# aligirayhanozbay/poisson_CNN

Hardware: AMD Instinct MI355X
Metric: grids/sec (fwd+bwd) at 1024^2 (higher is better)
Workload: dtype f32; 1 GPU; c4: Homogeneous_Poisson_NN_Legacy(hpnn.json) full train step (fwd+bwd+loss+Adam), 8 x 1024x1024 Dirichlet grids per GPU; global_batch=8, parallelism=dp1, math=fp32, ranks_seen=1

## Files before the change

include/pcnn.h:

```cpp
#ifndef PCNN_H
#define PCNN_H
#include <stddef.h>
#include <stdint.h>
#ifdef __cplusplus
extern "C" {
#endif

typedef struct pcnn_handle_s* pcnn_handle;

enum { PCNN_PAD_CONSTANT = 0, PCNN_PAD_SYMMETRIC = 1, PCNN_PAD_REFLECT = 2 };
enum { PCNN_ACT_LINEAR = 0, PCNN_ACT_LEAKY_RELU = 1, PCNN_ACT_TANH = 2, PCNN_ACT_RELU = 3 };
enum { PCNN_POOL_AVERAGE = 0, PCNN_POOL_MAX = 1 };
enum { PCNN_RESIZE_NEAREST = 0, PCNN_RESIZE_BILINEAR = 1, PCNN_RESIZE_BICUBIC = 2,
       PCNN_RESIZE_BICUBIC_LEGACY_ALIGN_CORNERS = 3  };

int pcnn_create(int device, void* hip_stream, pcnn_handle* out);
int pcnn_destroy(pcnn_handle h);
int pcnn_set_stream(pcnn_handle h, void* hip_stream);
int pcnn_sync(pcnn_handle h);
const char* pcnn_last_error(pcnn_handle h);
int pcnn_version(void);
uint32_t pcnn_crc32c(const void* data, size_t n, uint32_t crc);

#define PCNN_UNIQUE_ID_BYTES 128
int pcnn_collective_available(char* why, size_t why_bytes);
int pcnn_comm_unique_id(pcnn_handle h, void* id_out);
int pcnn_comm_init(pcnn_handle h, const void* id, int rank, int world_size);
int pcnn_comm_destroy(pcnn_handle h);
int pcnn_allreduce(pcnn_handle h, float* buf, size_t count);
int pcnn_broadcast(pcnn_handle h, float* buf, size_t count, int root);

enum { PCNN_MATH_FP32 = 0, PCNN_MATH_SPLIT_F16 = 1 };
int pcnn_set_math_mode(pcnn_handle h, int mode);
int pcnn_get_math_mode(pcnn_handle h);

enum { PCNN_SPECTRAL_AUTO = -1, PCNN_SPECTRAL_OFF = 0, PCNN_SPECTRAL_FORCE = 1 };
int pcnn_set_spectral_mode(pcnn_handle h, int mode);
int pcnn_get_spectral_mode(pcnn_handle h);
int pcnn_set_spectral_tile(pcnn_handle h, int tile);
int pcnn_get_spectral_tile(pcnn_handle h);
enum { PCNN_XFORM_MFMA = 0, PCNN_XFORM_FFT = 1 };
int pcnn_set_spectral_transform(pcnn_handle h, int xform);
int pcnn_get_spectral_transform(pcnn_handle h);
int pcnn_set_filter_version(pcnn_handle h, uint64_t version);
int pcnn_filter_cache_clear(pcnn_handle h);
int pcnn_filter_cache_stats(pcnn_handle h, long long* entries, long long* bytes, long long* hits, long long* fills, long long* refreshes);
int pcnn_set_workspace_limit(pcnn_handle h, size_t bytes);
int pcnn_set_workspace_retain(pcnn_handle h, int retain);

typedef struct {
  int N, H, W, Cin, ldx;
  int Ho, Wo, Cout, ldy;
  int kh, kw, pad_top, pad_left;
  int pad_mode; float pad_value;
  int act; float act_alpha;
  int ld_res;
  int ld_act_out;
} pcnn_conv_desc;

int pcnn_conv2d_fwd(pcnn_handle h, const pcnn_conv_desc* d, const float* x, const float* w, const float* bias,
                    const float* bn_scale, const float* bn_shift, const float* residual, float* y, float* act_out);
int pcnn_conv2d_fwd_absmax(pcnn_handle h, const pcnn_conv_desc* d, const float* x, const float* w, const float* bias,
                           const float* bn_scale, const float* bn_shift, const float* residual, float* y, float* act_out, float* y_absmax);

int pcnn_conv2d_flip_transpose_weights(pcnn_handle h, const float* w, float* wt, int kh, int kw, int Cin, int Cout);
typedef struct pcnn_flip_item { const float* w; float* wt; int kh, kw, Cin, Cout; int64_t start; } pcnn_flip_item;
int pcnn_conv2d_flip_transpose_table(pcnn_handle h, const pcnn_flip_item* table_dev, int n, int64_t total);

size_t pcnn_conv2d_wgrad_workspace(const pcnn_conv_desc* d);
int pcnn_conv2d_wgrad(pcnn_handle h, const pcnn_conv_desc* d, const float* x, const float* dz, float* dw,
                      void* workspace, size_t workspace_bytes);
int pcnn_conv2d_wgrad_hint(pcnn_handle h, const pcnn_conv_desc* d, const float* x, const float* dz, float* dw,
                           void* workspace, size_t workspace_bytes, const float* x_absmax, const float* dz_absmax);

int pcnn_resnet3_fwd_eligible(pcnn_handle h, int C, int act);
int pcnn_resnet3_fwd(pcnn_handle h, int N, int H, int W, int C, int act, float act_alpha, const float* x, const float* w0, const float* b0,
                     const float* w1, const float* b1, const float* w2, const float* b2, float* o0, float* a1, float* o1, float* y);

int pcnn_conv2d_bwd_spectral_eligible(pcnn_handle h, const pcnn_conv_desc* d, const pcnn_conv_desc* dg);
int pcnn_conv2d_bwd_spectral(pcnn_handle h, const pcnn_conv_desc* d, const pcnn_conv_desc* dg, const float* x, const float* dz, const float* w_flipped,
                             const float* residual, float* dx, float* dw);
typedef struct pcnn_post_desc {
  const float* act_out; int ld_act_out; int act; float act_alpha;
  float* dbias; float* raw_out; int ld_raw;
} pcnn_post_desc;
int pcnn_conv2d_bwd_spectral_post_eligible(pcnn_handle h, const pcnn_conv_desc* d, const pcnn_conv_desc* dg);
int pcnn_conv2d_bwd_spectral_post(pcnn_handle h, const pcnn_conv_desc* d, const pcnn_conv_desc* dg, const float* x, const float* dz, const float* w_flipped,
                                  const float* residual, float* dx, float* dw, const pcnn_post_desc* post);

int pcnn_conv2d_dgrad_post_eligible(pcnn_handle h, const pcnn_conv_desc* dg, const float* dz, const float* residual, const float* dx, const pcnn_post_desc* post);
int pcnn_conv2d_dgrad_post(pcnn_handle h, const pcnn_conv_desc* dg, const float* dz, const float* w_flipped, const float* residual, float* dx,
                           const pcnn_post_desc* post);

int pcnn_debug_forward_spectrum32(pcnn_handle h, int H, int W, int C, const float* x, int Vy, int Vx, int oy, int ox, int pad_mode, float pad_value,
                                  int ylim, int xlim, int pack, float* out, size_t out_floats);
int pcnn_debug_tile_spectrum64(pcnn_handle h, int H, int W, int C, const float* x, int ylim, int xlim, float* out);

size_t pcnn_colsum_workspace(int C);
int pcnn_conv2d_epilogue_bwd(pcnn_handle h, int64_t npix, int C, const float* dy, int lddy, const float* a, int lda,
                             const float* bn_scale, int act, float act_alpha, float* dz, int lddz,
                             float* dbias, float* dsum_dy_a, float* dsum_dy, void* workspace, size_t workspace_bytes);
int pcnn_conv2d_epilogue_bwd_absmax(pcnn_handle h, int64_t npix, int C, const float* dy, int lddy, const float* a, int lda,
                                    const float* bn_scale, int act, float act_alpha, float* dz, int lddz, float* dbias,
                                    float* dsum_dy_a, float* dsum_dy, float* dz_absmax, void* workspace, size_t workspace_bytes);

int pcnn_pad_fold_bwd(pcnn_handle h, int N, int H, int W, int C, int pt, int pb, int pl, int pr, int pad_mode,
                      const float* gp, int ldgp, float* gx, int ldgx, int accumulate);
int pcnn_pad_fold_bwd_post_eligible(int C, int ldgp, int ld_add, const void* gp, const void* add_to, const pcnn_post_desc* post, int lddz, const void* dz);
int pcnn_pad_fold_bwd_post(pcnn_handle h, int N, int H, int W, int C, int pt, int pb, int pl, int pr, int pad_mode, const float* gp, int ldgp,
                           const float* add_to, int ld_add, const pcnn_post_desc* post, const float* bn_scale, float* dsum_dy_a, float* dsum_dy,
                           float* dz, int lddz, void* workspace, size_t workspace_bytes);

int pcnn_bn_fold(pcnn_handle h, int n, const float* gamma, const float* beta, const float* mean, const float* var, float eps,
                 float* scale, float* shift);
int pcnn_bn_fold_bwd(pcnn_handle h, int n, const float* s_dy_a, const float* s_dy, const float* mean, const float* var, float eps,
                     float* dgamma, float* dbeta);

int pcnn_channel_affine(pcnn_handle h, int64_t npix, int C, const float* x, int ldx, const float* scale, const float* shift,
                        const float* residual, int ld_res, float* y, int ldy);
int pcnn_bn_train_fwd(pcnn_handle h, int64_t npix, int C, const float* a, int lda, const float* gamma, const float* beta, float eps,
                      float momentum, float* moving_mean, float* moving_var, float* mean, float* inv_std, float* scale, float* scratch_2C,
                      const float* residual, int ld_res, float* y, int ldy, void* workspace, size_t workspace_bytes);
int pcnn_bn_train_bwd(pcnn_handle h, int64_t npix, int C, const float* dy, int lddy, const float* a, int lda, const float* scale,
                      const float* mean, const float* inv_std, float* dgamma, float* dbeta, float* scratch_4C, float* da, int ldda,
                      void* workspace, size_t workspace_bytes);

int pcnn_pool2d_fwd(pcnn_handle h, int kind, int N, int H, int W, int C, int f, const float* x, int ldx, float* y, int ldy);
int pcnn_pool2d_bwd(pcnn_handle h, int kind, int N, int H, int W, int C, int f, const float* x, int ldx,
                    const float* y, int ldy, const float* dy, int lddy, float* dx, int lddx, int accumulate);

int pcnn_deconv_fwd(pcnn_handle h, int N, int hc, int wc, int Cin, int H, int W, int Cout, int f, const float* x, int ldx,
                    const float* k, const float* bias, float alpha, float beta, float* y, int ldy);
int pcnn_deconv_bwd_data(pcnn_handle h, int N, int hc, int wc, int Cin, int H, int W, int Cout, int f, const float* dy, int lddy,
                         const float* k, float alpha, float* dx, int lddx);
size_t pcnn_deconv_wgrad_workspace(int N, int hc, int wc, int Cin, int Cout, int f);
int pcnn_deconv_bwd_filter(pcnn_handle h, int N, int hc, int wc, int Cin, int H, int W, int Cout, int f, const float* x, int ldx,
                           const float* dy, int lddy, float alpha, float* dk, float* dbias, void* workspace, size_t workspace_bytes);

typedef struct {
  int N, H, W, Cin, ldx;
  int Ho, Wo, Cout, ldy;
  int k;
  int act; float act_alpha;
  float dropout_rate; uint32_t dropout_seed; uint32_t dropout_layer;
  int ld_act_out;
  int accumulate;
} pcnn_wide_desc;
int pcnn_wide_conv2d_fwd(pcnn_handle h, const pcnn_wide_desc* d, const float* x, const float* w, const float* bias, float* y);
int pcnn_wide_conv2d_dgrad(pcnn_handle h, const pcnn_wide_desc* d, const float* dz, const float* wf, const float* act_out, float* dx);
size_t pcnn_wide_conv2d_wgrad_workspace(const pcnn_wide_desc* d);
int pcnn_wide_conv2d_wgrad(pcnn_handle h, const pcnn_wide_desc* d, const float* x, const float* dz, float* dw, float* dbias, void* workspace,
                           size_t workspace_bytes);
int pcnn_wide_deconv_fwd(pcnn_handle h, const pcnn_wide_desc* d, const float* x, const float* k, const float* bias, float* y);
int pcnn_wide_deconv_bwd_data(pcnn_handle h, const pcnn_wide_desc* d, const float* dz, const float* k, const float* act_out, float* dx);
size_t pcnn_wide_deconv_bwd_filter_workspace(const pcnn_wide_desc* d);
int pcnn_wide_deconv_bwd_filter(pcnn_handle h, const pcnn_wide_desc* d, const float* x, const float* dz, float* dk, void* workspace,
                                size_t workspace_bytes);

int pcnn_resize_tables(int method, int n_in, int n_out, int32_t* idx , float* wt );
int pcnn_resize_fwd(pcnn_handle h, int N, int hc, int wc, int C, int Ho, int Wo, const float* x, int ldx,
                    const int32_t* idx_y, const float* wt_y, const int32_t* idx_x, const float* wt_x,
                    float alpha, float beta, float* y, int ldy);
typedef struct pcnn_resize_src {
  const float* x; int hc, wc, ldx;
  const int32_t* idx_y; const float* wt_y; const int32_t* idx_x; const float* wt_x;
} pcnn_resize_src;
int pcnn_resize_fwd_multi_eligible(int N, int C, int Ho, int Wo, int nsrc, const pcnn_resize_src* src, const float* y, int ldy);
int pcnn_resize_fwd_multi(pcnn_handle h, int N, int C, int Ho, int Wo, int nsrc, const pcnn_resize_src* src, float alpha, float beta, float* y, int ldy);
int pcnn_resize_bwd(pcnn_handle h, int N, int hc, int wc, int C, int Ho, int Wo, const float* dy, int lddy,
                    const int32_t* idx_y, const float* wt_y, const int32_t* idx_x, const float* wt_x,
                    float alpha, float* tmp, float* dx, int lddx);

size_t pcnn_grouped_conv2d_wgrad_workspace(const pcnn_conv_desc* d);
int pcnn_grouped_conv2d_uses_mfma(const pcnn_conv_desc* d, int what);
int pcnn_grouped_conv2d_fwd(pcnn_handle h, const pcnn_conv_desc* d, const float* x, const float* w, long long w_sample_stride, const float* bias,
                            long long bias_sample_stride, int flip_transpose, float* y);
int pcnn_grouped_conv2d_wgrad(pcnn_handle h, const pcnn_conv_desc* d, const float* x, const float* dz, float* dw, long long dw_sample_stride, void* workspace);
int pcnn_grouped_bias_grad(pcnn_handle h, int N, long long HW, int C, const float* dz, int lddz, float* dbias, long long bias_sample_stride);
int pcnn_grouped_deconv_fwd(pcnn_handle h, int N, int H, int W, int Cin, int Ho, int Wo, int Cout, int f, const float* x, const float* k,
                            long long k_sample_stride, const float* bias, long long bias_sample_stride, float* y);
int pcnn_grouped_deconv_bwd_data(pcnn_handle h, int N, int H, int W, int Cin, int Ho, int Wo, int Cout, int f, const float* dy, const float* k,
                                 long long k_sample_stride, float* dx);
int pcnn_grouped_deconv_bwd_filter(pcnn_handle h, int N, int H, int W, int Cin, int Ho, int Wo, int Cout, int f, const float* x, const float* dy,
                                   float* dk, long long k_sample_stride, float* dbias, long long bias_sample_stride);

int pcnn_dense_fwd(pcnn_handle h, int N, int In, int Out, const float* x, const float* w, const float* b, int act, float alpha, float* y);
int pcnn_dense_bwd(pcnn_handle h, int N, int In, int Out, const float* x, const float* w, const float* y, const float* dy,
                   int act, float alpha, float* dx, float* dw, float* db);

int pcnn_assemble_input(pcnn_handle h, int N, int H, int W, const float* rhs, int use_pos, float* out, int ldo);
int pcnn_subsample(pcnn_handle h, int N, int H, int W, int C, int stride, const float* x, int ldx, float* y, int ldy, int adjoint);
int pcnn_axpby(pcnn_handle h, int64_t npix, int C, float alpha, const float* x, int ldx, float beta, float* y, int ldy);
int pcnn_channel_scale_fwd(pcnn_handle h, int N, int64_t hw, int C, const float* x, int ldx, const float* s, float* y, int ldy);
int pcnn_channel_scale_bwd(pcnn_handle h, int N, int64_t hw, int C, const float* x, int ldx, const float* s, const float* dy, int lddy,
                           float* dx, int lddx, float* ds, void* workspace, size_t workspace_bytes);
size_t pcnn_channel_scale_workspace(int N, int64_t hw, int C);
int pcnn_channel_scale_bwd_post(pcnn_handle h, int N, int64_t hw, int C, const float* x, int ldx, const float* s, const float* dy, int lddy,
                                float* dz, int lddz, float* ds, int act, float act_alpha, float* dbias, void* workspace, size_t workspace_bytes);
int pcnn_sample_scale_fwd(pcnn_handle h, int N, int64_t per, const float* x, const float* g, float* y);
int pcnn_sample_scale_bwd(pcnn_handle h, int N, int64_t per, const float* x, const float* g, const float* dy, float* dx, float* dg);
int pcnn_bc_ring_fwd(pcnn_handle h, int N, int H, int W, int neumann, const float* x, float* y);
int pcnn_bc_ring_bwd(pcnn_handle h, int N, int H, int W, int neumann, const float* dy, float* dx);
int pcnn_bc_ring_edges_fwd(pcnn_handle h, int N, int H, int W, int neumann_mask, const float* x, float* y);
int pcnn_bc_ring_edges_bwd(pcnn_handle h, int N, int H, int W, int neumann_mask, const float* dy, float* dx);
int pcnn_spp_max_fwd(pcnn_handle h, int N, int H, int W, int C, int nb, const int32_t* bins, const float* x, float* out, int32_t* argmax);
int pcnn_spp_max_bwd(pcnn_handle h, int N, int H, int W, int C, int nb, const int32_t* argmax, const float* dout, float* dx);
int pcnn_jacobi_sweep(pcnn_handle h, int N, int H, int W, const float* u, const float* rhs, const float* dx , float* out);
int pcnn_jacobi_sweep_bwd(pcnn_handle h, int N, int H, int W, const float* dout, const float* dx , float* du);
int pcnn_jacobi_fused_fwd(pcnn_handle h, int N, int H, int W, int sy, int sx, const float* coef , const float* u, const float* rhs,
                          int n_sweeps, float* out);
int pcnn_jacobi_fused_bwd(pcnn_handle h, int N, int H, int W, int sy, int sx, const float* coef , const float* dout, int n_sweeps,
                          float* du);
int pcnn_jacobi_fused_tile(void);
int pcnn_jacobi_fused_max_sweeps(int sy, int sx);
int pcnn_jacobi_fused_bc_fwd(pcnn_handle h, int N, int H, int W, int sy, int sx, const float* coef , const float* u, const float* rhs,
                             int n_sweeps, int neumann_mask, float* out);
int pcnn_jacobi_fused_bc_bwd(pcnn_handle h, int N, int H, int W, int sy, int sx, const float* coef , const float* dout, int n_sweeps,
                             int neumann_mask, float* du);

int pcnn_loss_partials(pcnn_handle h, int N, int64_t hw, const float* pred, const float* target, const float* G, float* out );
int pcnn_loss_bwd(pcnn_handle h, int N, int64_t hw, const float* pred, const float* target, const float* G,
                  const float* c_mae, const float* c_mse, const float* c_int, float* dpred);
int pcnn_loss_coefficients(pcnn_handle h, int N, int64_t hw, const float* partials, float w_mae, float w_mse, float w_int,
                           int scale_by_peak, int global_batch_size, const float* extra, float* loss, float* c_mae, float* c_mse,
                           float* c_int, float* mse);
int pcnn_loss_partials_p(pcnn_handle h, int N, int64_t hw, const float* pred, const float* target, const float* G, float lp_power, float* partials);
int pcnn_loss_bwd_p(pcnn_handle h, int N, int64_t hw, const float* pred, const float* target, const float* G, const float* c_mae,
                    const float* c_mse, const float* c_int, float lp_power, float* dpred);
int pcnn_loss_coefficients_p(pcnn_handle h, int N, int64_t hw, const float* partials, float w_mae, float w_mse, float w_int, float lp_power,
                             int scale_by_peak, int global_batch_size, const float* extra, float* loss, float* c_mae, float* c_mse,
                             float* c_int, float* mse);
int pcnn_pi_loss_partials(pcnn_handle h, int N, int H, int W, int s, const float* pred, const float* rhs, const float* kern, float* out );
int pcnn_pi_loss_bwd(pcnn_handle h, int N, int H, int W, int s, const float* pred, const float* rhs, const float* kern,
                     const float* coef , float* dpred);
int pcnn_pi_loss_partials_rect(pcnn_handle h, int N, int H, int W, int sy, int sx, const float* pred, const float* rhs, const float* kern,
                               float* out );
int pcnn_pi_loss_bwd_rect(pcnn_handle h, int N, int H, int W, int sy, int sx, const float* pred, const float* rhs, const float* kern,
                          const float* coef , float* dpred);
int pcnn_error_stats(pcnn_handle h, int N, int H, int W, const float* pred, const float* target ,
                     const float* rhs , const float* dx , float* out );

// ... 83 lines not shown
```

poisson_cnn_amd/csrc/pcnn_internal.h:

```cpp
#pragma once
#include <hip/hip_runtime.h>
#include "pcnn_host.h"

void pcnn_comm_release(pcnn_handle_s* h);
void pcnn_filter_cache_free(pcnn_handle_s* h);

typedef float f32x16 __attribute__((ext_vector_type(16)));
typedef float f32x4 __attribute__((ext_vector_type(4)));

__device__ __forceinline__ float pcnn_act(float v, int act, float alpha) {
  switch (act) {
    case PCNN_ACT_LEAKY_RELU: return v > 0.f ? v : alpha * v;
    case PCNN_ACT_TANH: return tanhf(v);
    case PCNN_ACT_RELU: return v > 0.f ? v : 0.f;
    default: return v;
  }
}
__device__ __forceinline__ float pcnn_act_grad_from_out(float a, int act, float alpha) {
  switch (act) {
    case PCNN_ACT_LEAKY_RELU: return a > 0.f ? 1.f : alpha;
    case PCNN_ACT_TANH: return 1.f - a * a;
    case PCNN_ACT_RELU: return a > 0.f ? 1.f : 0.f;
    default: return 1.f;
  }
}

__device__ __forceinline__ int pcnn_pad_index(int i, int n, int mode) {
  if (i >= 0 && i < n) return i;
  if (mode == PCNN_PAD_CONSTANT) return -1;
  int r;
  if (mode == PCNN_PAD_SYMMETRIC) r = i < 0 ? -i - 1 : 2 * n - 1 - i;
  else r = i < 0 ? -i : 2 * n - 2 - i;
  return r < 0 ? 0 : (r >= n ? n - 1 : r);
}
```

poisson_cnn_amd/csrc/pointwise.hip:

```cpp
#include "pcnn_internal.h"

namespace {

constexpr int CS_BLOCK = 256;
constexpr int CS_MAXBLK = 1024;

static int pow2_ge(int c) { int p = 1; while (p < c) p <<= 1; return p; }

__global__ __launch_bounds__(CS_BLOCK) void epilogue_bwd_kernel(int64_t npix, int C, int CP, const float* __restrict__ dy, int lddy,
                                                                const float* __restrict__ a, int lda, const float* __restrict__ bn_scale,
                                                                int act, float alpha, float* __restrict__ dz, int lddz,
                                                                float* __restrict__ partial , unsigned* __restrict__ absmax) {
  __shared__ float red[3][CS_BLOCK];
  const int tid = threadIdx.x, c = tid % CP, r = tid / CP, R = CS_BLOCK / CP;
  float s0 = 0.f, s1 = 0.f, s2 = 0.f, zmax = 0.f;
  if (c < C) {
    const float sc = bn_scale ? bn_scale[c] : 1.f;
    for (int64_t pix = (int64_t)blockIdx.x * R + r; pix < npix; pix += (int64_t)gridDim.x * R) {
      const float g = dy[pix * lddy + c];
      const float av = a ? a[pix * lda + c] : 0.f;
      const float z = g * sc * pcnn_act_grad_from_out(av, act, alpha);
      if (dz) dz[pix * lddz + c] = z;
      s0 += z; s1 += g * av; s2 += g; zmax = fmaxf(zmax, fabsf(z));
    }
  }
  if (absmax) {
#pragma unroll
    for (int o = 32; o > 0; o >>= 1) zmax = fmaxf(zmax, __shfl_xor(zmax, o));
    if ((tid & 63) == 0) atomicMax(absmax, __float_as_uint(zmax <= 3.0e38f ? zmax : 3.0e38f));
  }
  red[0][tid] = s0; red[1][tid] = s1; red[2][tid] = s2;
  __syncthreads();
  if (r == 0 && c < C) {
    for (int k = 0; k < 3; ++k) {
      float s = 0.f;
      for (int q = 0; q < R; ++q) s += red[k][q * CP + c];
      partial[((int64_t)blockIdx.x * 3 + k) * C + c] = s;
    }
  }
}

__global__ __launch_bounds__(CS_BLOCK) void epilogue_bwd_vec4_kernel(int64_t npix, int C, const float* __restrict__ dy, int lddy,
                                                                     const float* __restrict__ a, int lda, const float* __restrict__ bn_scale,
                                                                     int act, float alpha, float* __restrict__ dz, int lddz,
                                                                     float* __restrict__ partial , unsigned* __restrict__ absmax) {
  __shared__ float red[3][CS_BLOCK * 4];
  float zmax = 0.f;
  const int GQ = C >> 2, R = CS_BLOCK / GQ;
  const int tid = threadIdx.x, r = tid / GQ, q = tid - r * GQ, c = q << 2;
  float s0[4] = {0.f, 0.f, 0.f, 0.f}, s1[4] = {0.f, 0.f, 0.f, 0.f}, s2[4] = {0.f, 0.f, 0.f, 0.f};
  if (r < R) {
    float sc[4];
#pragma unroll
    for (int j = 0; j < 4; ++j) sc[j] = bn_scale ? bn_scale[c + j] : 1.f;
    for (int64_t pix = (int64_t)blockIdx.x * R + r; pix < npix; pix += (int64_t)gridDim.x * R) {
      const float4 g4 = *reinterpret_cast<const float4*>(dy + pix * lddy + c);
      const float4 a4 = a ? *reinterpret_cast<const float4*>(a + pix * lda + c) : make_float4(0.f, 0.f, 0.f, 0.f);
      const float g[4] = {g4.x, g4.y, g4.z, g4.w}, av[4] = {a4.x, a4.y, a4.z, a4.w};
      float z[4];
#pragma unroll
      for (int j = 0; j < 4; ++j) {
        z[j] = g[j] * sc[j] * pcnn_act_grad_from_out(av[j], act, alpha);
        s0[j] += z[j]; s1[j] += g[j] * av[j]; s2[j] += g[j]; zmax = fmaxf(zmax, fabsf(z[j]));
      }
      if (dz) *reinterpret_cast<float4*>(dz + pix * lddz + c) = make_float4(z[0], z[1], z[2], z[3]);
    }
  }
  if (absmax) {
#pragma unroll
    for (int o = 32; o > 0; o >>= 1) zmax = fmaxf(zmax, __shfl_xor(zmax, o));
    if ((tid & 63) == 0) atomicMax(absmax, __float_as_uint(zmax <= 3.0e38f ? zmax : 3.0e38f));
  }
#pragma unroll
  for (int j = 0; j < 4; ++j) { red[0][tid * 4 + j] = s0[j]; red[1][tid * 4 + j] = s1[j]; red[2][tid * 4 + j] = s2[j]; }
  __syncthreads();
  if (tid < C) {
    for (int k = 0; k < 3; ++k) {
      float s = 0.f;
      for (int rr = 0; rr < R; ++rr) s += red[k][rr * C + tid];
      partial[((int64_t)blockIdx.x * 3 + k) * C + tid] = s;
    }
  }
}

__global__ __launch_bounds__(256) void colsum_final_kernel(const float* __restrict__ partial, int nblk, int C, float* o0, float* o1, float* o2) {
  __shared__ float red[3][256];
  const int c = blockIdx.x, t = threadIdx.x;
  float s[3] = {0.f, 0.f, 0.f};
  for (int b = t; b < nblk; b += 256)
    for (int k = 0; k < 3; ++k) s[k] += partial[((int64_t)b * 3 + k) * C + c];
  for (int k = 0; k < 3; ++k) red[k][t] = s[k];
  __syncthreads();
  for (int st = 128; st > 0; st >>= 1) {
    if (t < st)
      for (int k = 0; k < 3; ++k) red[k][t] += red[k][t + st];
    __syncthreads();
  }
  if (t == 0) {
    if (o0) o0[c] = red[0][0];
    if (o1) o1[c] = red[1][0];
    if (o2) o2[c] = red[2][0];
  }
}

static int colsum_blocks(int64_t npix, int CP) {
  const int R = CS_BLOCK / CP;
  int64_t nb = pcnn_cdiv64(npix, (int64_t)R * 16);
  if (nb > CS_MAXBLK) nb = CS_MAXBLK;
  if (nb < 1) nb = 1;
  return (int)nb;
}

__global__ void pad_fold_kernel(int N, int H, int W, int C, int pt, int pb, int pl, int pr, int mode, const float* __restrict__ gp, int ldgp,
                                float* __restrict__ gx, int ldgx, int accumulate) {
  const int Hp = H + pt + pb, Wp = W + pl + pr;
  const int64_t total = (int64_t)N * H * W * C;
  for (int64_t i = (int64_t)blockIdx.x * blockDim.x + threadIdx.x; i < total; i += (int64_t)gridDim.x * blockDim.x) {
    const int c = i % C; int64_t r = i / C; const int x = r % W; r /= W; const int y = r % H; const int n = r / H;
    int ys[3], xs[3], ny = 0, nx = 0;
    ys[ny++] = y + pt;
    xs[nx++] = x + pl;
    if (mode == PCNN_PAD_SYMMETRIC) {
      if (y < pt) ys[ny++] = pt - 1 - y;
      if (H - 1 - y < pb) ys[ny++] = pt + H + (H - 1 - y);
      if (x < pl) xs[nx++] = pl - 1 - x;
      if (W - 1 - x < pr) xs[nx++] = pl + W + (W - 1 - x);
    } else if (mode == PCNN_PAD_REFLECT) {
      if (y >= 1 && y <= pt) ys[ny++] = pt - y;
      if (H - 2 - y >= 0 && H - 2 - y < pb) ys[ny++] = pt + H + (H - 2 - y);
      if (x >= 1 && x <= pl) xs[nx++] = pl - x;
      if (W - 2 - x >= 0 && W - 2 - x < pr) xs[nx++] = pl + W + (W - 2 - x);
    }
    float s = 0.f;
    for (int a = 0; a < ny; ++a)
      for (int b = 0; b < nx; ++b) s += gp[(((int64_t)n * Hp + ys[a]) * Wp + xs[b]) * ldgp + c];
    float* dst = &gx[(((int64_t)n * H + y) * W + x) * ldgx + c];
    *dst = accumulate ? *dst + s : s;
  }
}

__global__ void pad_fold_vec4_kernel(int N, int H, int W, int C, int pt, int pb, int pl, int pr, int mode, const float* __restrict__ gp, int ldgp,
                                     float* __restrict__ gx, int ldgx, int accumulate) {
  const int Hp = H + pt + pb, Wp = W + pl + pr, CV = C >> 2;
  const int64_t total = (int64_t)N * H * W * CV;
  for (int64_t i = (int64_t)blockIdx.x * blockDim.x + threadIdx.x; i < total; i += (int64_t)gridDim.x * blockDim.x) {
    const int c = (int)(i % CV) << 2; int64_t r = i / CV; const int x = r % W; r /= W; const int y = r % H; const int n = r / H;
    int ys[3], xs[3], ny = 0, nx = 0;
    ys[ny++] = y + pt;
    xs[nx++] = x + pl;
    if (mode == PCNN_PAD_SYMMETRIC) {
      if (y < pt) ys[ny++] = pt - 1 - y;
      if (H - 1 - y < pb) ys[ny++] = pt + H + (H - 1 - y);
      if (x < pl) xs[nx++] = pl - 1 - x;
      if (W - 1 - x < pr) xs[nx++] = pl + W + (W - 1 - x);
    } else if (mode == PCNN_PAD_REFLECT) {
      if (y >= 1 && y <= pt) ys[ny++] = pt - y;
      if (H - 2 - y >= 0 && H - 2 - y < pb) ys[ny++] = pt + H + (H - 2 - y);
      if (x >= 1 && x <= pl) xs[nx++] = pl - x;
      if (W - 2 - x >= 0 && W - 2 - x < pr) xs[nx++] = pl + W + (W - 2 - x);
    }
    float4 s = make_float4(0.f, 0.f, 0.f, 0.f);
    for (int a = 0; a < ny; ++a)
      for (int b = 0; b < nx; ++b) {
        const float4 q = *reinterpret_cast<const float4*>(gp + (((int64_t)n * Hp + ys[a]) * Wp + xs[b]) * ldgp + c);
        s.x += q.x; s.y += q.y; s.z += q.z; s.w += q.w;
      }
    float4* dst = reinterpret_cast<float4*>(gx + (((int64_t)n * H + y) * W + x) * ldgx + c);
    if (accumulate) { const float4 o = *dst; s.x += o.x; s.y += o.y; s.z += o.z; s.w += o.w; }
    *dst = s;
  }
}

__global__ __launch_bounds__(CS_BLOCK) void pad_fold_post_vec4_kernel(int N, int H, int W, int C, int pt, int pb, int pl, int pr, int mode,
                                                                      const float* __restrict__ gp, int ldgp, const float* __restrict__ add_to, int ldadd,
                                                                      const float* __restrict__ a, int lda, const float* __restrict__ bn_scale, int act, float alpha,
                                                                      float* __restrict__ raw, int ldraw, float* __restrict__ dz, int lddz,
                                                                      float* __restrict__ partial ) {
  __shared__ float red[3][CS_BLOCK * 4];
  const int Hp = H + pt + pb, Wp = W + pl + pr;
  const int64_t npix = (int64_t)N * H * W;
  const int GQ = C >> 2, R = CS_BLOCK / GQ;
  const int tid = threadIdx.x, r = tid / GQ, q = tid - r * GQ, c = q << 2;
  float s0[4] = {0.f, 0.f, 0.f, 0.f}, s1[4] = {0.f, 0.f, 0.f, 0.f}, s2[4] = {0.f, 0.f, 0.f, 0.f};
  if (r < R) {
    float sc[4];
#pragma unroll
    for (int j = 0; j < 4; ++j) sc[j] = bn_scale ? bn_scale[c + j] : 1.f;
    for (int64_t pix = (int64_t)blockIdx.x * R + r; pix < npix; pix += (int64_t)gridDim.x * R) {
      int64_t t = pix; const int x = t % W; t /= W; const int y = t % H; const int n = t / H;
      int ys[3], xs[3], ny = 0, nx = 0;
      ys[ny++] = y + pt;
      xs[nx++] = x + pl;
      if (mode == PCNN_PAD_SYMMETRIC) {
        if (y < pt) ys[ny++] = pt - 1 - y;
        if (H - 1 - y < pb) ys[ny++] = pt + H + (H - 1 - y);
        if (x < pl) xs[nx++] = pl - 1 - x;
        if (W - 1 - x < pr) xs[nx++] = pl + W + (W - 1 - x);
      } else if (mode == PCNN_PAD_REFLECT) {
        if (y >= 1 && y <= pt) ys[ny++] = pt - y;
        if (H - 2 - y >= 0 && H - 2 - y < pb) ys[ny++] = pt + H + (H - 2 - y);
        if (x >= 1 && x <= pl) xs[nx++] = pl - x;
        if (W - 2 - x >= 0 && W - 2 - x < pr) xs[nx++] = pl + W + (W - 2 - x);
      }
      float4 g = make_float4(0.f, 0.f, 0.f, 0.f);
      for (int ia = 0; ia < ny; ++ia)
        for (int ib = 0; ib < nx; ++ib) {
          const float4 v = *reinterpret_cast<const float4*>(gp + (((int64_t)n * Hp + ys[ia]) * Wp + xs[ib]) * ldgp + c);
          g.x += v.x; g.y += v.y; g.z += v.z; g.w += v.w;
        }
      if (add_to) { const float4 o = *reinterpret_cast<const float4*>(add_to + pix * ldadd + c); g.x += o.x; g.y += o.y; g.z += o.z; g.w += o.w; }
      if (raw) *reinterpret_cast<float4*>(raw + pix * ldraw + c) = g;
      const float4 a4 = *reinterpret_cast<const float4*>(a + pix * lda + c);
      const float gv[4] = {g.x, g.y, g.z, g.w}, av[4] = {a4.x, a4.y, a4.z, a4.w};
      float z[4];
#pragma unroll
      for (int j = 0; j < 4; ++j) {
        z[j] = gv[j] * sc[j] * pcnn_act_grad_from_out(av[j], act, alpha);
        s0[j] += z[j]; s1[j] += gv[j] * av[j]; s2[j] += gv[j];
      }
      *reinterpret_cast<float4*>(dz + pix * lddz + c) = make_float4(z[0], z[1], z[2], z[3]);
    }
  }
#pragma unroll
  for (int j = 0; j < 4; ++j) { red[0][tid * 4 + j] = s0[j]; red[1][tid * 4 + j] = s1[j]; red[2][tid * 4 + j] = s2[j]; }
  __syncthreads();
  if (tid < C) {
    for (int k = 0; k < 3; ++k) {
      float s = 0.f;
      for (int rr = 0; rr < R; ++rr) s += red[k][rr * C + tid];
      partial[((int64_t)blockIdx.x * 3 + k) * C + tid] = s;
    }
  }
}

__global__ void axpby_kernel(int64_t npix, int C, float alpha, const float* __restrict__ x, int ldx, float beta, float* __restrict__ y, int ldy) {
  const int64_t total = npix * C;
  for (int64_t i = (int64_t)blockIdx.x * blockDim.x + threadIdx.x; i < total; i += (int64_t)gridDim.x * blockDim.x) {
    const int c = i % C; const int64_t pix = i / C;
    float* dst = &y[pix * ldy + c];
    const float v = alpha * x[pix * ldx + c];
    *dst = beta == 0.f ? v : v + beta * *dst;
  }
}

__global__ void assemble_input_kernel(int N, int H, int W, const float* __restrict__ rhs, int use_pos, float* __restrict__ out, int ldo) {
  const int64_t total = (int64_t)N * H * W;
  const float pi = 3.14159265358979323846f;
  for (int64_t i = (int64_t)blockIdx.x * blockDim.x + threadIdx.x; i < total; i += (int64_t)gridDim.x * blockDim.x) {
    const int x = i % W; const int y = (i / W) % H;
    out[i * ldo] = rhs[i];
    if (use_pos) {
      const float ly = H > 1 ? (float)y * (1.0f / (float)(H - 1)) : 0.f;
      const float lx = W > 1 ? (float)x * (1.0f / (float)(W - 1)) : 0.f;
      out[i * ldo + 1] = cosf(pi * ly);
      out[i * ldo + 2] = cosf(pi * lx);
    }
  }
}

__global__ void channel_scale_fwd_kernel(int N, int64_t hw, int C, const float* __restrict__ x, int ldx, const float* __restrict__ s,
                                         float* __restrict__ y, int ldy) {
  const int64_t total = (int64_t)N * hw * C;
  for (int64_t i = (int64_t)blockIdx.x * blockDim.x + threadIdx.x; i < total; i += (int64_t)gridDim.x * blockDim.x) {
    const int c = i % C; const int64_t pix = i / C; const int n = pix / hw;
    y[pix * ldy + c] = x[pix * ldx + c] * s[n * C + c];
  }
}

__global__ __launch_bounds__(CS_BLOCK) void channel_scale_bwd_kernel(int64_t hw, int C, int CP, const float* __restrict__ x, int ldx,
                                                                     const float* __restrict__ s, const float* __restrict__ dy, int lddy,
                                                                     float* __restrict__ dx, int lddx, float* __restrict__ partial,
                                                                     int gmode, float galpha, float* __restrict__ bpartial) {
  __shared__ float red[CS_BLOCK];
  const int n = blockIdx.y, tid = threadIdx.x, c = tid % CP, r = tid / CP, R = CS_BLOCK / CP;
  float acc = 0.f, bacc = 0.f;
  if (c < C) {
    const float sv = s[n * C + c];
    for (int64_t q = (int64_t)blockIdx.x * R + r; q < hw; q += (int64_t)gridDim.x * R) {
      const int64_t pix = (int64_t)n * hw + q;
      const float g = dy[pix * lddy + c], xv = x[pix * ldx + c];
      acc += g * xv;
      float v = g * sv;
      if (bpartial) {
        v *= gmode == PCNN_ACT_TANH ? 1.f - xv * xv : (xv > 0.f ? 1.f : galpha);
        bacc += v;
      }
      dx[pix * lddx + c] = v;
    }
  }
  red[tid] = acc;
  __syncthreads();
  if (r == 0 && c < C) {
    float t = 0.f;
    for (int q = 0; q < R; ++q) t += red[q * CP + c];
    partial[((int64_t)n * gridDim.x + blockIdx.x) * C + c] = t;
  }
  if (bpartial) {
    __syncthreads();
    red[tid] = bacc;
    __syncthreads();
    if (r == 0 && c < C) {
      float t = 0.f;
      for (int q = 0; q < R; ++q) t += red[q * CP + c];
      bpartial[((int64_t)n * gridDim.x + blockIdx.x) * C + c] = t;
    }
  }
}

__global__ void channel_scale_bias_final_kernel(const float* __restrict__ bpartial, int N, int nb, int C, float* __restrict__ dbias) {
  const int c = blockIdx.x * blockDim.x + threadIdx.x;
  if (c >= C) return;
  float t = 0.f;
  for (int i = 0; i < N * nb; ++i) t += bpartial[(int64_t)i * C + c];
  dbias[c] = t;
}

__global__ void channel_scale_final_kernel(const float* __restrict__ partial, int N, int nblk, int C, float* __restrict__ ds) {
  const int i = blockIdx.x * blockDim.x + threadIdx.x;
  if (i >= N * C) return;
  const int n = i / C, c = i % C;
  float t = 0.f;
  for (int b = 0; b < nblk; ++b) t += partial[((int64_t)n * nblk + b) * C + c];
  ds[i] = t;
}

__global__ void sample_scale_fwd_kernel(int N, int64_t per, const float* __restrict__ x, const float* __restrict__ g, float* __restrict__ y) {
  const int64_t total = (int64_t)N * per;
  for (int64_t i = (int64_t)blockIdx.x * blockDim.x + threadIdx.x; i < total; i += (int64_t)gridDim.x * blockDim.x)
    y[i] = x[i] * (1.0f + g[i / per]);
}

constexpr int SS_SPLIT = 64;
__global__ __launch_bounds__(256) void sample_scale_bwd_kernel(int64_t per, const float* __restrict__ x, const float* __restrict__ g,
                                                               const float* __restrict__ dy, float* __restrict__ dx, float* __restrict__ part) {
  __shared__ float red[256];
  const int n = blockIdx.y, sp = blockIdx.x;
  const float gv = 1.0f + g[n];
  const int64_t piece = (per + SS_SPLIT - 1) / SS_SPLIT, q0 = (int64_t)sp * piece, q1 = q0 + piece < per ? q0 + piece : per;
  float acc = 0.f;
  for (int64_t q = q0 + threadIdx.x; q < q1; q += blockDim.x) {
    const int64_t i = (int64_t)n * per + q;
    const float d = dy[i];
    acc += d * x[i];
    dx[i] = d * gv;
  }
  red[threadIdx.x] = acc;
  __syncthreads();
  for (int s = blockDim.x / 2; s > 0; s >>= 1) {
    if ((int)threadIdx.x < s) red[threadIdx.x] += red[threadIdx.x + s];
    __syncthreads();
  }
  if (threadIdx.x == 0) part[n * SS_SPLIT + sp] = red[0];
}
__global__ void sample_scale_final_kernel(int N, const float* __restrict__ part, float* __restrict__ dg) {
  const int n = blockIdx.x * blockDim.x + threadIdx.x;
  if (n >= N) return;
// ... 638 lines not shown
```

poisson_cnn_amd/csrc/spectral_common.h:

```cpp
#pragma once
#include "pcnn_internal.h"
#include <type_traits>

namespace pcnn_spec {

constexpr int RS = 32;
constexpr int SP_PAD = 32;
__host__ __device__ __forceinline__ int64_t sp_item(int64_t item, int rows) { return item * ((int64_t)rows * RS + SP_PAD); }
__host__ __device__ __forceinline__ size_t sp_bytes(size_t items, int rows) { return items * ((size_t)rows * RS + SP_PAD) * sizeof(float); }

constexpr int SP_P = 1;
__host__ __device__ constexpr int sp_blk(int P, int k, int part) { return 2 * P * (k / P) + P * part + (k % P); }
__host__ __device__ constexpr int sp_pc(int T, int P) { return P < T ? P : T; }
__host__ __device__ constexpr int sp_pr(int T, int P) { return P < T / 2 ? P : T / 2; }
__host__ __device__ constexpr int sp_row_c(int T, int fy, int part, int P = SP_P) { return sp_blk(sp_pc(T, P), fy, part); }
__host__ __device__ constexpr int sp_row_r(int T, int s, int P = SP_P) {
  return s == T / 2 ? sp_blk(sp_pr(T, P), 0, 1) : (s < T / 2 ? sp_blk(sp_pr(T, P), s, 0) : sp_blk(sp_pr(T, P), s - T / 2, 1));
}
__host__ __device__ constexpr int sp_row_from_canonical(int T, int r, int P = SP_P) {
  return r < 2 * T ? (r / T) * T + sp_row_r(T, r % T, P) : 2 * T + ((r - 2 * T) / (2 * T)) * 2 * T + sp_row_c(T, (r - 2 * T) % T, ((r - 2 * T) % (2 * T)) / T, P);
}
static_assert(sp_row_from_canonical(32, 5, 64) == 5 && sp_row_from_canonical(32, 16, 64) == 16 && sp_row_from_canonical(32, 64 + 37, 64) == 64 + 37 && sp_row_from_canonical(64, 128 + 64 + 9, 64) == 128 + 64 + 9, "P >= T is the canonical order");
static_assert(sp_row_from_canonical(32, 16, 1) == 1 && sp_row_from_canonical(32, 3, 1) == 6 && sp_row_from_canonical(32, 16 + 3, 1) == 7 && sp_row_from_canonical(32, 64 + 32 + 5, 1) == 64 + 11, "P = 1: Re | Im adjacent");
inline void sp_build_slots(int T, int P, int* slots) {
  int n = 0;
  auto put = [&](int rr, int ri, int kind) { slots[4 * n] = rr; slots[4 * n + 1] = ri; slots[4 * n + 2] = kind; slots[4 * n + 3] = 0; ++n; };
  for (int b = 0; b < 2; ++b) {
    put(b * T + sp_row_r(T, 0, P), b * T + sp_row_r(T, T / 2, P), 1);
    for (int fy = 1; fy < T / 2; ++fy) put(b * T + sp_row_r(T, fy, P), b * T + sp_row_r(T, T / 2 + fy, P), 0);
  }
  for (int fx = 1; fx < T / 2; ++fx)
    for (int fy = 0; fy < T; ++fy) put(2 * T + 2 * T * (fx - 1) + sp_row_c(T, fy, 0, P), 2 * T + 2 * T * (fx - 1) + sp_row_c(T, fy, 1, P), 0);
}

__device__ __forceinline__ f32x16 mfma(float a, float b, f32x16 c) { return __builtin_amdgcn_mfma_f32_32x32x2f32(a, b, c, 0, 0, 0); }
__device__ __forceinline__ f32x4 mfma16(float a, float b, f32x4 c) { return __builtin_amdgcn_mfma_f32_16x16x4f32(a, b, c, 0, 0, 0); }
__device__ __forceinline__ f32x16 zero16() {
  f32x16 z;
#pragma unroll
  for (int i = 0; i < 16; ++i) z[i] = 0.f;
  return z;
}
__device__ __forceinline__ f32x4 zero4() { f32x4 z = {0.f, 0.f, 0.f, 0.f}; return z; }
__device__ __forceinline__ void lds_barrier() { asm volatile("s_waitcnt lgkmcnt(0)\n\ts_barrier" ::: "memory"); }
__device__ __forceinline__ int acc_row(int r, int half) { return 8 * (r >> 2) + 4 * half + (r & 3); }

__device__ __forceinline__ float dpp_quad_swap1(float v) { return __int_as_float(__builtin_amdgcn_mov_dpp(__float_as_int(v), 0xB1, 0xf, 0xf, true)); }
__device__ __forceinline__ float dpp_quad_swap2(float v) { return __int_as_float(__builtin_amdgcn_mov_dpp(__float_as_int(v), 0x4E, 0xf, 0xf, true)); }
__device__ __forceinline__ void quad_transpose(float& r0, float& r1, float& r2, float& r3, bool odd, bool upper) {
  { const float t = dpp_quad_swap1(odd ? r0 : r1); if (odd) r0 = t; else r1 = t; }
  { const float t = dpp_quad_swap1(odd ? r2 : r3); if (odd) r2 = t; else r3 = t; }
  { const float t = dpp_quad_swap2(upper ? r0 : r2); if (upper) r0 = t; else r2 = t; }
  { const float t = dpp_quad_swap2(upper ? r1 : r3); if (upper) r1 = t; else r3 = t; }
}

struct FwdParams {
  const float* x = nullptr; float* sp = nullptr; const float* tab = nullptr;
  int H = 0, W = 0, C = 0, ld = 0, groups = 1, cstride = 32, cvalid = 32;
  int tiles_x = 1, tiles_y = 1, tile0 = 0, ntile = 1;
  int Vy = 0, Vx = 0, oy = 0, ox = 0, pad_mode = PCNN_PAD_CONSTANT; float pad_value = 0.f;
  int ylim = 0, xlim = 0;
  int ext_y = 1 << 30, ext_x = 1 << 30;
  int pack = 1, cpt = 32, tgx = 1;
};

struct InvParams {
  const float* sp = nullptr; const float* tab = nullptr;
  float* y = nullptr; const float* bias = nullptr; const float* bn_scale = nullptr; const float* bn_shift = nullptr; const float* res = nullptr;
  float* act_out = nullptr; unsigned* absmax = nullptr;
  int Ho = 0, Wo = 0, C = 0, ldy = 0, ld_res = 0, ld_act = 0, groups = 1, cstride = 32, cvalid = 32, act = PCNN_ACT_LINEAR; float alpha = 0.f;
  int tiles_x = 1, tiles_y = 1, tile0 = 0, ntile = 1, Vy = 0, Vx = 0;
  int flip = 0;
  int pack = 1, cpt = 32, tgx = 1;
  const float* gact = nullptr; float* y2 = nullptr; float* bsum = nullptr;
  int ld_gact = 0, ld_y2 = 0, gmode = 0; float galpha = 1.f;
};

constexpr int TAB32_FLOATS = 7168, TAB64_FLOATS = 32768;
constexpr size_t O_TAB32 = 0, O_SLOTS32 = O_TAB32 + ((TAB32_FLOATS * 4 + 255) & ~255), O_TAB64 = O_SLOTS32 + 512 * 16,
                 O_SLOTS64 = O_TAB64 + TAB64_FLOATS * 4, O_SLOTS32F = O_SLOTS64 + 2048 * 16, O_SLOTS64F = O_SLOTS32F + 512 * 16, O_REST = O_SLOTS64F + 2048 * 16;
static_assert(O_REST % 256 == 0, "workspace header alignment");
void build_tables64(float* tab, int* slots);

constexpr int POST_BLOCKS = 256, POST_SLOTS_MAX = POST_BLOCKS * 8 * 4;

struct Xform {
  int family;
  int T, rows, nslot;
  int P;
  size_t tab_off, slots_off;
  void (*fwd)(pcnn_handle h, FwdParams p, int ntile);
  void (*inv)(pcnn_handle h, InvParams p, int ntile);
  void (*post_bias)(pcnn_handle h, const float* bsum, int pack, int cpt, int C, float* dbias);
  void (*fwd_multi)(pcnn_handle h, const FwdParams* tab, int count, int max_items);
  int post_slots;
  const float* tab; const int4* slots;
};
extern const Xform XFORM_MFMA32, XFORM_MFMA64, XFORM_FFT32, XFORM_FFT64;

template <bool B> using flag = std::integral_constant<bool, B>;
template <typename Launch>
void dispatch_epilogue(InvParams p, Launch launch) {
  auto slope = [](int act, float alpha) { return act == PCNN_ACT_LINEAR ? 1.f : (act == PCNN_ACT_RELU ? 0.f : alpha); };
  if (p.gact) {
    p.alpha = 1.f; p.galpha = slope(p.gmode, p.galpha);
    if (p.res) launch(flag<false>{}, flag<true>{}, flag<true>{}, p); else launch(flag<false>{}, flag<false>{}, flag<true>{}, p);
  } else if (p.act == PCNN_ACT_TANH) {
    if (p.res) launch(flag<true>{}, flag<true>{}, flag<false>{}, p); else launch(flag<true>{}, flag<false>{}, flag<false>{}, p);
  } else {
    p.alpha = slope(p.act, p.alpha);
    if (p.res) launch(flag<false>{}, flag<true>{}, flag<false>{}, p); else launch(flag<false>{}, flag<false>{}, flag<false>{}, p);
  }
}

}
```

poisson_cnn_amd/csrc/spectral_conv.hip:

```cpp
#include "spectral_common.h"
#include <math.h>
#include <stdlib.h>
#include <array>
#include <vector>

int pcnn_spectral_conv_fwd(pcnn_handle h, const pcnn_conv_desc* d, const float* x, const float* w, const float* bias, const float* bn_scale,
                           const float* bn_shift, const float* residual, float* y, float* act_out);
int pcnn_spectral_conv_wgrad(pcnn_handle h, const pcnn_conv_desc* d, const float* x, const float* dz, float* dw);
bool pcnn_spectral_eligible(pcnn_handle h, const pcnn_conv_desc* d, bool wgrad);
bool pcnn_conv_small_fwd_eligible(const pcnn_conv_desc* d);
bool pcnn_conv_fwd_takes_narrow_route(pcnn_handle h, const pcnn_conv_desc* d);

using namespace pcnn_spec;


namespace {

constexpr int T = 32, ROWS = 1024, NSLOT = 512;
constexpr int TAB_G = 0, TAB_GI = 1024, TAB_F2 = 2048, TAB_FI2 = 4096, TAB_GI2 = 6144, TAB_FLOATS = TAB32_FLOATS;
static_assert(TAB_GI2 + 1024 == TAB_FLOATS, "table block");
constexpr size_t LDS_U = (size_t)T * T * 32 * sizeof(float);
constexpr size_t LDS_INV = LDS_U + 1024 * sizeof(float);
__host__ __device__ __forceinline__ int64_t sp_item(int64_t item) { return pcnn_spec::sp_item(item, ROWS); }

// ... 928 lines not shown
  for (FilterEntry& en : fc->e) pcnn_release(h, en.buf);
  for (int ti = 0; ti < 2; ++ti) if (fc->dev[ti]) pcnn_release(h, fc->dev[ti]);
  delete fc;
  h->filter_cache = nullptr;
}

extern "C" int pcnn_set_filter_version(pcnn_handle h, uint64_t version) {
  if (!h) return 1;
  h->filter_version = version;
  return 0;
}

extern "C" int pcnn_filter_cache_clear(pcnn_handle h) {
  if (!h) return 1;
  pcnn_filter_cache_free(h);
  return 0;
}

extern "C" int pcnn_filter_cache_stats(pcnn_handle h, long long* entries, long long* bytes, long long* hits, long long* fills, long long* refreshes) {
  if (!h) return 1;
  const FilterCache* fc = static_cast<const FilterCache*>(h->filter_cache);
  if (entries) *entries = fc ? (long long)fc->e.size() : 0;
  if (bytes) *bytes = fc ? (long long)fc->bytes : 0;
  if (hits) *hits = h->fc_hits;
  if (fills) *fills = h->fc_fills;
  if (refreshes) *refreshes = h->fc_refreshes;
  return 0;
}

int pcnn_spectral_conv_fwd(pcnn_handle h, const pcnn_conv_desc* d, const float* x, const float* w, const float* bias, const float* bn_scale,
                           const float* bn_shift, const float* residual, float* y, float* act_out) {
  TileGrid g;
  if (int rc = tile_grid(h, d, d->kh, d->kw, d->N, d->Ho, d->Wo, d->Cin, d->Cout, &g)) return rc;
  const int gin = pcnn_cdiv(d->Cin, 32), gout = pcnn_cdiv(d->Cout, 32);
  int chunk = std::min(chunk_tiles(g.T) / (gin > gout ? gin : gout), g.ntile);
  float* ws[3];
  if (int rc = carve_workspace(h, &chunk, [&](int ch) {
        return std::array<size_t, 3>{sp_region((size_t)d->Cin * gout, g.rows), sp_region((size_t)ch * gin, g.rows), sp_region((size_t)pad32(ch) * gout, g.rows)};
      }, ws)) return rc;
  float *wsp = ws[0], *xs = ws[1], *ys = ws[2];
  const Xform xf = xform_of(h, g.T);
  const float* fsp = filter_spectrum(h, xf, w, wsp, d->kh, d->kw, d->Cin, d->Cout, gout);
  PCNN_CHECK_LAUNCH(h, "spectral convolution (filter spectrum)");
  FwdParams fx = image_fwd_params(g, x, xs, d->H, d->W, d->Cin, d->ldx, gin, d->pad_top, d->pad_left, d->pad_mode, d->pad_value);
  InvParams iv = image_inv_params(g, ys, y, d->Ho, d->Wo, d->Cout, d->ldy, gout, residual, d->ld_res);
  iv.bias = bias; iv.bn_scale = bn_scale; iv.bn_shift = bn_shift; iv.act_out = act_out; iv.ld_act = d->ld_act_out;
  iv.absmax = reinterpret_cast<unsigned*>(h->y_absmax); iv.act = d->act; iv.alpha = d->act_alpha;
  MixParams mx;
  mx.xs = xs; mx.ys = ys; mx.wsp = fsp; mx.gin = gin; mx.gout = gout; mx.Cin = d->Cin; mx.cpt = g.cpt;
  for (int t0 = 0; t0 < g.ntile; t0 += chunk) {
    const int nt = std::min(chunk, g.ntile - t0);
    fx.tile0 = t0; iv.tile0 = t0;
    launch_fwd(h, xf, fx, nt);
    launch_mix(h, xf, mx, gin, gout, nt);
    launch_inv(h, xf, iv, nt);
  }
  PCNN_CHECK_LAUNCH(h, "spectral convolution");
  return 0;
}

int pcnn_spectral_conv_wgrad(pcnn_handle h, const pcnn_conv_desc* d, const float* x, const float* dz, float* dw) {
  TileGrid g;
  if (int rc = tile_grid(h, d, d->kh, d->kw, d->N, d->Ho, d->Wo, d->Cin, d->Cout, &g)) return rc;
  const int gin = pcnn_cdiv(d->Cin, 32), S = wgrad_splits(g.T);
  int chunk = std::min(chunk_tiles(g.T) / gin, g.ntile);
  float* ws[4];
  if (int rc = carve_workspace(h, &chunk, [&](int ch) {
        return std::array<size_t, 4>{sp_region((size_t)d->Cin, g.rows), sp_region((size_t)ch * gin, g.rows), sp_region((size_t)ch, g.rows), align256((size_t)S * g.nslot * gin * 4 * 1024 * 4)};
      }, ws)) return rc;
  float *csp = ws[0], *xs = ws[1], *zs = ws[2], *part = ws[3];
  const Xform xf = xform_of(h, g.T);
  FwdParams fx = image_fwd_params(g, x, xs, d->H, d->W, d->Cin, d->ldx, gin, d->pad_top, d->pad_left, d->pad_mode, d->pad_value);
  FwdParams fz = image_fwd_params(g, dz, zs, d->Ho, d->Wo, d->Cout, d->ldy, 1, 0, 0, PCNN_PAD_CONSTANT, 0.f);
  fz.ylim = g.Vy; fz.xlim = g.Vx;
  WMixParams wm;
  wm.xs = xs; wm.ds = zs; wm.part = part; wm.slots = xf.slots; wm.gin = gin; wm.S = S / 4; wm.rows = g.rows; wm.nslot = g.nslot;
  for (int t0 = 0; t0 < g.ntile; t0 += chunk) {
    const int nt = std::min(chunk, g.ntile - t0);
    fx.tile0 = t0; fz.tile0 = t0; wm.ntile = nt; wm.accumulate = t0 > 0;
    launch_fwd(h, xf, fx, nt);
    launch_fwd(h, xf, fz, nt);
    hipLaunchKernelGGL(spec_wmix_kernel, dim3(g.nslot, S / 4, gin), dim3(256), 0, h->stream, wm);
  }
  hipLaunchKernelGGL(spec_wcombine_kernel, dim3(g.nslot, gin), dim3(256), 0, h->stream, part, xf.slots, csp, S, gin, d->Cin, 1.0f, g.cpt, g.rows);
  launch_inv(h, xf, taps_params(xf, csp, dw, d->kh, d->kw, d->Cin, d->Cout, 0), 1);
  PCNN_CHECK_LAUNCH(h, "spectral weight gradient");
  return 0;
}

__global__ __launch_bounds__(256) void spec_canonical_rows_kernel(const float* __restrict__ sp, float* __restrict__ out, int T, int rows, int P) {
  const int item = blockIdx.y;
  for (int e = blockIdx.x * 256 + threadIdx.x; e < rows * 32; e += gridDim.x * 256) {
    const int r = e >> 5, c = e & 31;
    out[(size_t)item * rows * 32 + e] = sp[pcnn_spec::sp_item(item, rows) + pcnn_spec::sp_row_from_canonical(T, r, P) * RS + c];
  }
}
static int canonical_copy(pcnn_handle h, const Xform& xf, const float* sp, float* out, int items) {
  hipLaunchKernelGGL(spec_canonical_rows_kernel, dim3(16, items), dim3(256), 0, h->stream, sp, out, xf.T, xf.rows, xf.P);
  return hipGetLastError() == hipSuccess ? 0 : 1;
}

extern "C" int pcnn_debug_tile_spectrum64(pcnn_handle h, int H, int W, int C, const float* x, int ylim, int xlim, float* out) {
  PCNN_REQUIRE(h, h && x && out && H >= 1 && W >= 1 && C >= 1 && C <= 64, "pcnn_debug_tile_spectrum64: bad argument");
  TileGrid g;
  if (int rc = tile_grid_given(h, 64, 64, 64, 1, 1, 64, 64, &g)) return rc;
  const int groups = pcnn_cdiv(C, 32);
  char* r;
  if (int rc = ensure_workspace(h, sp_region((size_t)groups, g.rows), &r)) return rc;
  const Xform xf = xform_of(h, g.T);
  FwdParams f = image_fwd_params(g, x, reinterpret_cast<float*>(r), H, W, C, C, groups, 0, 0, PCNN_PAD_CONSTANT, 0.f);
  f.ylim = ylim; f.xlim = xlim;
  launch_fwd(h, xf, f, 1);
  PCNN_CHECK_LAUNCH(h, "pcnn_debug_tile_spectrum64");
  if (canonical_copy(h, xf, f.sp, out, groups)) PCNN_FAIL(h, "pcnn_debug_tile_spectrum64: copy failed");
  return 0;
}

extern "C" int pcnn_debug_forward_spectrum32(pcnn_handle h, int H, int W, int C, const float* x, int Vy, int Vx, int oy, int ox, int pad_mode, float pad_value,
                                             int ylim, int xlim, int pack, float* out, size_t out_floats) {
  PCNN_REQUIRE(h, h && x && out && H >= 1 && W >= 1 && C >= 1 && C <= 64 && Vy >= 1 && Vy <= 32 && Vx >= 1 && Vx <= 32, "pcnn_debug_forward_spectrum32: bad argument");
  PCNN_REQUIRE(h, pack == 1 || ((pack == 2 || pack == 4 || pack == 8) && C <= 32 / pack), "pcnn_debug_forward_spectrum32: pack = %d with %d channels", pack, C);
  TileGrid g;
  if (int rc = tile_grid_given(h, 32, Vy, Vx, pack, 1, H, W, &g)) return rc;
  const int groups = pack > 1 ? 1 : pcnn_cdiv(C, 32);
  PCNN_REQUIRE(h, out_floats >= (size_t)g.ntile * groups * 1024 * 32, "pcnn_debug_forward_spectrum32: output holds %zu floats, %zu needed", out_floats, (size_t)g.ntile * groups * 1024 * 32);
  char* r;
  if (int rc = ensure_workspace(h, sp_region((size_t)g.ntile * groups, g.rows), &r)) return rc;
  const Xform xf = xform_of(h, g.T);
  FwdParams f = image_fwd_params(g, x, reinterpret_cast<float*>(r), H, W, C, C, groups, oy, ox, pad_mode, pad_value);
  f.ylim = ylim; f.xlim = xlim;
  launch_fwd(h, xf, f, g.ntile);
  PCNN_CHECK_LAUNCH(h, "pcnn_debug_forward_spectrum32");
  if (canonical_copy(h, xf, f.sp, out, g.ntile * groups)) PCNN_FAIL(h, "pcnn_debug_forward_spectrum32: copy failed");
  return 0;
}

extern "C" int pcnn_conv2d_bwd_spectral_eligible(pcnn_handle h, const pcnn_conv_desc* d, const pcnn_conv_desc* dg) {
  if (!h || !d || !dg) return 0;
  if (d->Cout > 32 || d->Cin > 64) return 0;
  if (d->pad_mode == PCNN_PAD_CONSTANT && d->pad_value != 0.f) return 0;
  if (pcnn_conv_fwd_takes_narrow_route(h, dg)) return 0;
  if (pcnn_spectral_eligible(h, dg, false) && pcnn_spectral_eligible(h, d, true)) return 1;
  double ts_g = 0.0, ta_g = 0.0, ts_w = 0.0, ta_w = 0.0;
  if (spectral_costs(h, dg, false, &ts_g, &ta_g) != 2 || spectral_costs(h, d, true, &ts_w, &ta_w) != 2) return 0;
  return 1.75 * std::max(ts_g, ts_w) < 0.9 * (ta_g + ta_w) ? 1 : 0;
}

extern "C" int pcnn_conv2d_bwd_spectral_post_eligible(pcnn_handle h, const pcnn_conv_desc* d, const pcnn_conv_desc* dg) {
  if (!pcnn_conv2d_bwd_spectral_eligible(h, d, dg)) return 0;
  if (d->pad_mode != PCNN_PAD_CONSTANT) return 0;
  return d->Cin <= 32 ? 1 : 0;
}

static int bwd_spectral_impl(pcnn_handle h, const pcnn_conv_desc* d, const pcnn_conv_desc* dg, const float* x, const float* dz, const float* w_flipped,
                             const float* residual, float* dx, float* dw, const pcnn_post_desc* post);

extern "C" int pcnn_conv2d_bwd_spectral(pcnn_handle h, const pcnn_conv_desc* d, const pcnn_conv_desc* dg, const float* x, const float* dz, const float* w_flipped,
                                        const float* residual, float* dx, float* dw) {
  return bwd_spectral_impl(h, d, dg, x, dz, w_flipped, residual, dx, dw, nullptr);
}

extern "C" int pcnn_conv2d_bwd_spectral_post(pcnn_handle h, const pcnn_conv_desc* d, const pcnn_conv_desc* dg, const float* x, const float* dz, const float* w_flipped,
                                             const float* residual, float* dx, float* dw, const pcnn_post_desc* post) {
  PCNN_REQUIRE(h, h && post && post->act_out, "pcnn_conv2d_bwd_spectral_post: null argument");
  PCNN_REQUIRE(h, pcnn_conv2d_bwd_spectral_post_eligible(h, d, dg), "pcnn_conv2d_bwd_spectral_post: layer is not eligible (ask pcnn_conv2d_bwd_spectral_post_eligible first)");
  return bwd_spectral_impl(h, d, dg, x, dz, w_flipped, residual, dx, dw, post);
}

static int bwd_spectral_impl(pcnn_handle h, const pcnn_conv_desc* d, const pcnn_conv_desc* dg, const float* x, const float* dz, const float* w_flipped,
                             const float* residual, float* dx, float* dw, const pcnn_post_desc* post) {
  PCNN_REQUIRE(h, h && d && dg && x && dz && w_flipped && dx && dw, "pcnn_conv2d_bwd_spectral: null argument");
  if (pcnn_check_conv_desc(h, "pcnn_conv2d_bwd_spectral", d, 64, 32, PCNN_ANY) || pcnn_check_conv_desc(h, "pcnn_conv2d_bwd_spectral (dg)", dg, 32, 64, PCNN_ANY)) return 1;
  PCNN_REQUIRE(h, pcnn_conv2d_bwd_spectral_eligible(h, d, dg), "pcnn_conv2d_bwd_spectral: layer is not eligible (ask pcnn_conv2d_bwd_spectral_eligible first)");
  PCNN_REQUIRE(h, dg->Cin == d->Cout && dg->Cout == d->Cin && dg->kh == d->kh && dg->kw == d->kw && dg->N == d->N, "pcnn_conv2d_bwd_spectral: descriptors do not match");
  TileGrid g;
  if (int rc = tile_grid(h, dg, d->kh, d->kw, d->N, dg->Ho, dg->Wo, d->Cin, d->Cout, &g)) return rc;
  const int gz = 1, gx = pcnn_cdiv(d->Cin, 32), S = wgrad_splits(g.T);
  const size_t bs_b = post ? (size_t)POST_SLOTS_MAX * 64 * sizeof(float) : 0;
  int chunk = std::min(chunk_tiles(g.T) / gx, g.ntile);
  float* ws[7];
  if (int rc = carve_workspace(h, &chunk, [&](int ch) {
        const size_t ys_b = sp_region((size_t)pad32(ch) * gx, g.rows);
        return std::array<size_t, 7>{sp_region((size_t)std::max(dg->Cin * gx, d->Cin), g.rows), sp_region((size_t)ch * gz, g.rows), ys_b, ys_b,
                                     align256((size_t)S * g.nslot * gx * 4 * 1024 * 4), bs_b, 4096};
      }, ws)) return rc;
  float *wsp = ws[0], *zs = ws[1], *ys = ws[2], *xs = ws[3], *part = ws[4], *bsum = ws[5];
  const Xform xf = xform_of(h, g.T);
  PCNN_REQUIRE(h, gx == 1 || dg->Cout == 64, "pcnn_conv2d_bwd_spectral: %d input channels unsupported (<= 32 or 64)", d->Cin);
  const float* fsp = filter_spectrum(h, xf, w_flipped, wsp, d->kh, d->kw, dg->Cin, dg->Cout, gx);
  PCNN_CHECK_LAUNCH(h, "pcnn_conv2d_bwd_spectral (filter spectrum)");
  FwdParams fz = image_fwd_params(g, dz, zs, dg->H, dg->W, dg->Cin, dg->ldx, gz, dg->pad_top, dg->pad_left, dg->pad_mode, dg->pad_value);
  const bool padded_domain = d->pad_mode != PCNN_PAD_CONSTANT;
  FwdParams fxm = image_fwd_params(g, x, xs, d->H, d->W, d->Cin, d->ldx, gx, padded_domain ? d->pad_top : 0, padded_domain ? d->pad_left : 0, d->pad_mode, 0.f);
  fxm.ylim = g.Vy; fxm.xlim = g.Vx; fxm.ext_y = dg->Ho; fxm.ext_x = dg->Wo;
  InvParams iv = image_inv_params(g, ys, dx, dg->Ho, dg->Wo, dg->Cout, dg->ldy, gx, residual, dg->ld_res);
  if (post) {
    iv.gact = post->act_out; iv.ld_gact = post->ld_act_out; iv.gmode = post->act; iv.galpha = post->act_alpha;
    iv.y2 = post->raw_out; iv.ld_y2 = post->ld_raw; iv.bsum = post->dbias ? bsum : nullptr;
    if (iv.bsum && hipMemsetAsync(bsum, 0, bs_b, h->stream) != hipSuccess) PCNN_FAIL(h, "pcnn_conv2d_bwd_spectral_post: memset failed");
  }
  MixWParams mw;
  mw.zs = zs; mw.xs = xs; mw.ys = ys; mw.part = part; mw.wsp = fsp; mw.slots = xf.slots; mw.gx = gx; mw.rows = g.rows; mw.nslot = g.nslot;
  mw.Cz = dg->Cin; mw.cpt = g.cpt;
  for (int t0 = 0; t0 < g.ntile; t0 += chunk) {
    const int nt = std::min(chunk, g.ntile - t0);
    fz.tile0 = t0; fxm.tile0 = t0; iv.tile0 = t0; mw.ntile = nt; mw.accumulate = t0 > 0;
    launch_fwd(h, xf, fz, nt);
    launch_fwd(h, xf, fxm, nt);
    hipLaunchKernelGGL(spec_mixw_kernel, dim3(g.nslot, S / 4, gx), dim3(256), 0, h->stream, mw);
    launch_inv(h, xf, iv, nt);
  }
  if (post && post->dbias) xf.post_bias(h, bsum, g.pack, g.cpt, dg->Cout, post->dbias);
  float* csp = wsp;
  hipLaunchKernelGGL(spec_wcombine_kernel, dim3(g.nslot, gx), dim3(256), 0, h->stream, part, xf.slots, csp, S, gx, d->Cin, -1.0f, g.cpt, g.rows);
  launch_inv(h, xf, taps_params(xf, csp, dw, d->kh, d->kw, d->Cin, d->Cout, 1), 1);
  PCNN_CHECK_LAUNCH(h, "pcnn_conv2d_bwd_spectral");
  return 0;
}
```

poisson_cnn_amd/csrc/spectral_fft.hip:

```cpp
#include "spectral_common.h"
#include "fft_regs.h"
#include <algorithm>

namespace pcnn_spec {

namespace {
using namespace pcnn_fft;

constexpr int T = 32, ROWS = 1024;
constexpr int EO = 16 * 32 * 32;
constexpr size_t LDS_BYTES = (size_t)T * T * 32 * sizeof(float);
__host__ __device__ __forceinline__ int64_t sp_item32(int64_t item) { return pcnn_spec::sp_item(item, ROWS); }

__device__ __forceinline__ int pad_sel(int i, int n, int mode) {
  const int refl = mode == PCNN_PAD_SYMMETRIC ? (i < 0 ? -i - 1 : 2 * n - 1 - i) : (i < 0 ? -i : 2 * n - 2 - i);
  const int rc = min(max(refl, 0), n - 1);
  return (unsigned)i < (unsigned)n ? i : (mode == PCNN_PAD_CONSTANT ? 0 : rc);
}

struct FwdRow {
  float fill;
  int cl, cr;
  int xlim;
  bool use_fill;
// ... 5 lines not shown
  int t = p.tile0 + item / p.groups;
  const int txg = t % p.tgx; t /= p.tgx;
  const int ty = t % p.tiles_y;
  const int n = t / p.tiles_y;
  const int sub = p.pack > 1 ? c / p.cpt : 0, cc = c - sub * p.cpt;
  const int tx = txg * p.pack + sub;
  const int chan = g * p.cstride + cc;
  const bool cok = cc < p.cvalid && chan < p.C && tx < p.tiles_x;
  const float* img = p.x + (int64_t)n * p.H * p.W * p.ld;
  const int wy0 = ty * p.Vy - p.oy, wx0 = tx * p.Vx - p.ox;
  const int ylim = min(p.ylim, p.ext_y - ty * p.Vy);
  it.xlim = min(p.xlim, p.ext_x - tx * p.Vx);
  const int gy = wy0 + y;
  const bool rowconst = p.pad_mode == PCNN_PAD_CONSTANT && (unsigned)gy >= (unsigned)p.H;
  const bool rowzero = !cok || y >= ylim;
  it.use_fill = rowzero || rowconst;
  it.fill = rowzero ? 0.f : p.pad_value;
  it.cl = 0; it.cr = T;
  const int wx_first = txg * p.pack * p.Vx - p.ox, wx_last = wx_first + (p.pack - 1) * p.Vx;
  it.fast = wx_first >= 0 && wx_last + T <= p.W;
  if (2 * wave >= ylim) return;
  const int sy = pad_sel(gy, p.H, p.pad_mode);
  const unsigned ch = (unsigned)(cok ? chan : 0);
  if (it.fast) {
    const unsigned lo = (unsigned)((sy * p.W + wx0) * p.ld) + ch;
    const float* rp = img;
#pragma unroll
    for (int x = 0; x < T; ++x) { R[x] = rp[lo]; rp += p.ld; }
  } else {
    const unsigned rowoff = (unsigned)(sy * p.W * p.ld) + ch;
    if (p.pad_mode == PCNN_PAD_CONSTANT) { it.cl = -wx0; it.cr = p.W - wx0; }
#pragma unroll
    for (int x = 0; x < T; ++x) R[x] = img[rowoff + (unsigned)(pad_sel(wx0 + x, p.W, p.pad_mode) * p.ld)];
  }
}

template <bool MASKED>
__device__ __forceinline__ void fwd_consume(const FwdParams& p, const FwdRow& it, float (&R)[32]) {
#pragma unroll
  for (int x = 0; x < T; ++x) {
    float v = R[x];
    if (!it.fast && (x < it.cl || x >= it.cr)) v = p.pad_value;
    if (it.use_fill) v = it.fill;
    if (MASKED && x >= it.xlim) v = 0.f;
    R[x] = v;
  }
}

template <int N> __device__ __forceinline__ void pin(float* a) {
#pragma unroll
  for (int i = 0; i < N; ++i) asm volatile("" : "+v"(a[i]));
}

__device__ __forceinline__ float hc_get(const float (&R)[32], int s) {
  bool neg = false;
  const int pos = s <= 16 ? rfft_pos(32, s, false, neg) : rfft_pos(32, s - 16, true, neg);
  return neg ? -R[pos] : R[pos];
}
__device__ __forceinline__ void hc_put(float (&R)[32], int s, float v) {
  bool neg = false;
  const int pos = s <= 16 ? rfft_pos(32, s, false, neg) : rfft_pos(32, s - 16, true, neg);
  R[pos] = neg ? -v : v;
}

template <bool MASKED>
__device__ __forceinline__ void fft32_fwd_body(const FwdParams& p, float* U, const int bid, const int gdim) {
  const int tid = threadIdx.x, lane = tid & 63, half = lane >> 5, c = lane & 31;
  const int wave = __builtin_amdgcn_readfirstlane(tid >> 6);
  const int total = p.ntile * p.groups;
  int item = bid;
  if (item >= total) return;
  const int y = 2 * wave + half;
  float R[32];
  FwdRow cur;
  fwd_request(p, item, wave, y, c, cur, R);
  auto x_phase = [&]() {
    fwd_consume<MASKED>(p, cur, R);
    rfft_fwd<32>(R);
    float* u = U + (y * 32) * 32 + c;
#pragma unroll
    for (int s = 0; s < T; ++s) u[s * 32] = hc_get(R, s);
  };
  x_phase();
  for (;;) {
    const int next = item + gdim;
    if (next < total) fwd_request(p, next, wave, y, c, cur, R);
    lds_barrier();
    float* out = p.sp + sp_item32(item);
    float V[32];
    if (wave == 0) {
      const float* u = U + (half ? 16 : 0) * 32 + c;
#pragma unroll
      for (int yy = 0; yy < T; ++yy) V[yy] = u[yy * 1024];
      rfft_fwd<32>(V);
      const unsigned lo = (unsigned)((half ? 32 : 0) * RS + c);
#pragma unroll
      for (int s = 0; s < T; ++s) __builtin_nontemporal_store(hc_get(V, s), &(out + (sp_row_r(T, s) * RS))[lo]);
    } else {
      const float* ur = U + wave * 32 + c, *ui = U + (16 + wave) * 32 + c;
      float* vr = V, *vi = V + 16;
      int par = half;
      asm volatile("" : "+v"(par));
      const float osign = par ? -1.f : 1.f;
#pragma unroll
      for (int yy = 0; yy < 16; ++yy) {
        const float lr = ur[yy * 1024], hr = ur[(yy + 16) * 1024], li = ui[yy * 1024], hi = ui[(yy + 16) * 1024];
        const float ar = fma_(osign, hr, lr), ai = fma_(osign, hi, li);
        if (yy == 0) { vr[yy] = ar; vi[yy] = ai; }
        else {
          const float wr = par ? tw_re<32>(yy) : 1.f, wi = par ? tw_im<32>(yy) : 0.f;
          vr[yy] = fma_(ar, wr, -(ai * wi));
          vi[yy] = fma_(ar, wi, ai * wr);
        }
      }
      cfft_dif<16, -1>(vr, vi);
      float* o = out + (64 + 64 * (wave - 1)) * RS;
      const unsigned lo = (unsigned)(half * (sp_row_c(T, 1, 0) - sp_row_c(T, 0, 0)) * RS + c);
#pragma unroll
      for (int m = 0; m < 16; ++m) {
        __builtin_nontemporal_store(vr[bitrev(m, 16)], &(o + (sp_row_c(T, 2 * m, 0) * RS))[lo]);
        __builtin_nontemporal_store(vi[bitrev(m, 16)], &(o + (sp_row_c(T, 2 * m, 1) * RS))[lo]);
      }
    }
    if (next >= total) break;
    item = __builtin_amdgcn_readfirstlane(next);
    lds_barrier();
    x_phase();
  }
}

template <bool MASKED>
__global__ __launch_bounds__(1024) void fft32_fwd_kernel(FwdParams p) {
  extern __shared__ __attribute__((aligned(16))) float U[];
  fft32_fwd_body<MASKED>(p, U, blockIdx.x, gridDim.x);
}

__device__ __forceinline__ FwdParams load_fwd_params(const FwdParams* q) {
  static_assert(sizeof(FwdParams) % 4 == 0, "FwdParams is copied word by word");
  FwdParams p;
  const int* s = reinterpret_cast<const int*>(q);
  int* d = reinterpret_cast<int*>(&p);
#pragma unroll
  for (int i = 0; i < (int)(sizeof(FwdParams) / 4); ++i) d[i] = __builtin_amdgcn_readfirstlane(s[i]);
  return p;
}

__global__ __launch_bounds__(1024) void fft32_fwd_multi_kernel(const FwdParams* __restrict__ tab) {
  extern __shared__ __attribute__((aligned(16))) float U[];
  const FwdParams p = load_fwd_params(tab + blockIdx.y);
  fft32_fwd_body<true>(p, U, blockIdx.x, gridDim.x);
}

struct NoBetween { __device__ __forceinline__ void operator()(int) const {} };
template <bool TANH, bool RES, bool POST, int NPIX, int BURST, bool NT, typename Between = NoBetween>
__device__ __forceinline__ void epilogue_row(const InvParams& p, const float* X, float scale, int vx, unsigned pix0, int sgn, unsigned chv, float bias, float sc, float sh,
                                             float* yimg, float* aimg, const float* rimg, const float* gimg, float* y2img, float& ymax, float& bsum, Between between = Between(),
                                             int vx_uniform = NPIX) {
  auto st = [](float v, float* q) { if (NT) __builtin_nontemporal_store(v, q); else *q = v; };
  float first_y = 0.f, first_a = 0.f, first_y2 = 0.f;
#pragma unroll
  for (int x0b = 0; x0b < NPIX; x0b += BURST) {
    if (x0b >= vx_uniform) { between(x0b / BURST); continue; }
    float rv[BURST], gv[BURST], oy[BURST], oa[BURST], oy2[BURST];
    if (RES) {
#pragma unroll
      for (int r = 0; r < BURST; ++r) rv[r] = rimg[(pix0 + (unsigned)(x0b + r < vx ? sgn * (x0b + r) : 0)) * (unsigned)p.ld_res + chv];
    }
    if (POST) {
#pragma unroll
      for (int r = 0; r < BURST; ++r) gv[r] = gimg[(pix0 + (unsigned)(x0b + r < vx ? sgn * (x0b + r) : 0)) * (unsigned)p.ld_gact + chv];
    }
#pragma unroll
    for (int r = 0; r < BURST; ++r) {
      const bool ok = x0b + r < vx;
      float v = X[x0b + r] * scale;
      if (!POST) {
        v += bias;
        v = TANH ? tanhf(v) : (v > 0.f ? v : v * p.alpha);
        oa[r] = v;
        v = v * sc + sh;
      }
      if (RES) v += rv[r];
      if (POST) {
        oy2[r] = v;
        const float gq = gv[r];
        v *= p.gmode == PCNN_ACT_TANH ? 1.f - gq * gq : (gq > 0.f ? 1.f : p.galpha);
        bsum += ok ? v : 0.f;
      }
      oy[r] = v;
      ymax = fmaxf(ymax, ok ? fabsf(v) : 0.f);
      if (x0b + r == 0) { first_y = v; if (!POST) first_a = oa[0]; if (POST) first_y2 = oy2[0]; }
    }
    __builtin_amdgcn_sched_barrier(0);
    float* const second = POST ? y2img : aimg;
    const unsigned ld2 = (unsigned)(POST ? p.ld_y2 : p.ld_act);
    if (second) {
#pragma unroll
      for (int r = 0; r < BURST; ++r) {
        const bool ok = x0b + r < vx;
        const unsigned pix = pix0 + (unsigned)(ok ? sgn * (x0b + r) : 0);
        st(ok ? (POST ? oy2[r] : oa[r]) : (POST ? first_y2 : first_a), &second[pix * ld2 + chv]);
        st(ok ? oy[r] : first_y, &yimg[pix * (unsigned)p.ldy + chv]);
      }
    } else {
#pragma unroll
      for (int r = 0; r < BURST; ++r) {
        const bool ok = x0b + r < vx;
        const unsigned pix = pix0 + (unsigned)(ok ? sgn * (x0b + r) : 0);
        st(ok ? oy[r] : first_y, &yimg[pix * (unsigned)p.ldy + chv]);
      }
    }
    __builtin_amdgcn_sched_barrier(0);
    between(x0b / BURST);
  }
}

__device__ __forceinline__ void inv_request(const float* in, int wave, int half, int c, float (&B)[32]) {
  const float* sp = in + (wave == 0 ? 0 : (64 + 64 * (wave - 1)) * RS);
  const unsigned lo = (unsigned)((wave == 0 ? 32 : sp_row_c(T, 1, 0) - sp_row_c(T, 0, 0)) * RS * half + c);
  static_assert(sp_row_r(T, 17, 1) == 3 && sp_row_r(T, 16, 1) == 1 && sp_row_c(T, 6, 1, 1) == 13, "row order the stepping form assumes");
  const int step = (wave == 0 ? 2 : 4) * RS;
#pragma unroll
  for (int part = 0; part < 2; ++part) {
    const float* q = sp + part * RS;
#pragma unroll
    for (int m = 0; m < 16; ++m) { B[16 * part + m] = q[lo]; q += step; }
  }
}

template <int J0, int NJ>
__device__ __forceinline__ void inv_request_slice(const float* in, int wave, int half, int c, float (&B)[32]) {
  const float* sp = in + (wave == 0 ? 0 : (64 + 64 * (wave - 1)) * RS);
  const unsigned lo = (unsigned)((wave == 0 ? 32 : 2) * RS * half + c);
  const int step = (wave == 0 ? 2 : 4) * RS;
#pragma unroll
  for (int j = J0; j < J0 + NJ; ++j) B[j] = (sp + (j >> 4) * RS + (j & 15) * step)[lo];
}

template <bool RES, bool POST> constexpr bool inv32_pipe() { return RES == POST; }

template <bool TANH, bool RES, bool POST>
__global__ __launch_bounds__(1024) void fft32_inv_kernel(InvParams p) {
  extern __shared__ __attribute__((aligned(16))) float U[];
  const int tid = threadIdx.x, lane = tid & 63, half = lane >> 5, c = lane & 31;
  const int wave = __builtin_amdgcn_readfirstlane(tid >> 6);
  const int total = p.ntile * p.groups;
  int item = blockIdx.x;
  if (item >= total) return;
  constexpr bool INV32_PIPE = inv32_pipe<RES, POST>();
  float B[32];
  if (INV32_PIPE) inv_request(p.sp + sp_item32(item), wave, half, c, B);
  float ymax = 0.f, bsum = 0.f;
  constexpr int BURST = (RES == POST) ? 4 : 8;
  for (;;) {
    const int next = item + gridDim.x;
    {
      float V[32];
      if (!INV32_PIPE) inv_request(p.sp + sp_item32(item), wave, half, c, B);
#pragma unroll
      for (int i = 0; i < 32; ++i) V[i] = B[i];
      if (wave == 0) {
        float W[32];
#pragma unroll
        for (int s = 0; s < T; ++s) hc_put(W, s, V[s]);
        rfft_inv<32>(W);
        float* e = U + (half ? 16 : 0) * 32 + c;
#pragma unroll
        for (int yy = 0; yy < 16; ++yy) {
          e[yy * 1024] = 0.5f * (W[yy] + W[yy + 16]);
          e[EO + yy * 1024] = 0.5f * (W[yy] - W[yy + 16]);
        }
      } else {
        float* vr = V, *vi = V + 16;
        cfft_dif<16, +1>(vr, vi);
        float* er = U + (half ? EO : 0) + wave * 32 + c, *ei = er + 16 * 32;
        int par = half;
        asm volatile("" : "+v"(par));
#pragma unroll
        for (int yy = 0; yy < 16; ++yy) {
          const float ar = vr[bitrev(yy, 16)], ai = vi[bitrev(yy, 16)];
          if (yy == 0) { er[0] = ar; ei[0] = ai; }
          else {
            const float wr = par ? tw_re<32>(yy) : 1.f, wi = par ? -tw_im<32>(yy) : 0.f;
            er[yy * 1024] = fma_(ar, wr, -(ai * wi));
            ei[yy * 1024] = fma_(ar, wi, ai * wr);
          }
        }
      }
    }
    lds_barrier();
    {
      const int g = item % p.groups;
      int t = p.tile0 + item / p.groups;
      const int txg = t % p.tgx; t /= p.tgx;
      const int ty = t % p.tiles_y;
      const int n = t / p.tiles_y;
      const int sub = p.pack > 1 ? c / p.cpt : 0, cc = c - sub * p.cpt;
      const int subx = sub * p.Vx;
      const int y0 = ty * p.Vy, x0 = txg * p.pack * p.Vx;
      const int vy = min(p.Vy, p.Ho - y0), vx = min(p.Vx, p.Wo - x0 - subx);
      const int chan = g * p.cstride + cc;
      const bool cok = cc < p.cvalid && chan < p.C;
      const float* nin = p.sp + sp_item32(next < total ? next : item);
      bool piped = false;
      if (2 * wave < vy) {
        const int yy = 2 * wave + half;
        const bool rowok = cok && yy < vy && vx > 0;
        float X[32];
        {
          const float* e = U + ((yy & 15) * 32) * 32 + c;
          const float osign = wave < 8 ? 1.f : -1.f;
#pragma unroll
          for (int s0 = 0; s0 < T; s0 += 8) {
#pragma unroll
            for (int s = s0; s < s0 + 8; ++s) hc_put(X, s, fma_(osign, e[EO + s * 32], e[s * 32]));
            __builtin_amdgcn_sched_barrier(0);
          }
        }
        rfft_inv<32>(X);
        const float bias = (p.bias && cok) ? p.bias[chan] : 0.f;
        const float sc = (p.bn_scale && cok) ? p.bn_scale[chan] : 1.f, sh = (p.bn_scale && cok) ? p.bn_shift[chan] : 0.f;
        const int sgn = p.flip ? -1 : 1;
        const int prow = p.flip ? p.Ho - 1 - y0 - yy : y0 + yy, pcol = p.flip ? p.Wo - 1 - x0 - subx : x0 + subx;
        unsigned pix0 = (unsigned)(prow * p.Wo + pcol);
        asm volatile("" : "+v"(pix0));
        const int64_t ipix = (int64_t)n * p.Ho * p.Wo;
        float* yimg = p.y + ipix * p.ldy;
        float* aimg = (!POST && p.act_out) ? p.act_out + ipix * p.ld_act : nullptr;
        const float* rimg = RES ? p.res + ipix * p.ld_res : nullptr;
        const float* gimg = POST ? p.gact + ipix * p.ld_gact : nullptr;
        float* y2img = (POST && p.y2) ? p.y2 + ipix * p.ld_y2 : nullptr;
        const unsigned chv = (unsigned)chan;
        if (INV32_PIPE) {
          auto between = [&](int b) {
            if constexpr (BURST == 8) {
              if (b == 0) inv_request_slice<0, 8>(nin, wave, half, c, B); else if (b == 1) inv_request_slice<8, 8>(nin, wave, half, c, B);
              else if (b == 2) inv_request_slice<16, 8>(nin, wave, half, c, B); else inv_request_slice<24, 8>(nin, wave, half, c, B);
            } else {
              if (b == 0) inv_request_slice<0, 4>(nin, wave, half, c, B); else if (b == 1) inv_request_slice<4, 4>(nin, wave, half, c, B);
              else if (b == 2) inv_request_slice<8, 4>(nin, wave, half, c, B); else if (b == 3) inv_request_slice<12, 4>(nin, wave, half, c, B);
              else if (b == 4) inv_request_slice<16, 4>(nin, wave, half, c, B); else if (b == 5) inv_request_slice<20, 4>(nin, wave, half, c, B);
              else if (b == 6) inv_request_slice<24, 4>(nin, wave, half, c, B); else inv_request_slice<28, 4>(nin, wave, half, c, B);
            }
          };
          if (rowok) {
            epilogue_row<TANH, RES, POST, T, BURST, false>(p, X, 1.f / 1024.f, vx, pix0, sgn, chv, bias, sc, sh, yimg, aimg, rimg, gimg, y2img, ymax, bsum, between,
                                                           p.pack > 1 ? T : __builtin_amdgcn_readfirstlane(min(p.Vx, p.Wo - x0)));
          } else {
            inv_request(nin, wave, half, c, B);
          }
          piped = true;
        } else
        if (rowok)
          epilogue_row<TANH, RES, POST, T, BURST, false>(p, X, 1.f / 1024.f, vx, pix0, sgn, chv, bias, sc, sh, yimg, aimg, rimg, gimg, y2img, ymax, bsum, NoBetween(),
                                                         p.pack > 1 ? T : __builtin_amdgcn_readfirstlane(min(p.Vx, p.Wo - x0)));
      }
      if (INV32_PIPE && !piped) inv_request(nin, wave, half, c, B);
    }
    if (next >= total) break;
    item = __builtin_amdgcn_readfirstlane(next);
    lds_barrier();
  }
  if (POST && p.bsum) p.bsum[(blockIdx.x * 16 + wave) * 64 + lane] += bsum;
  if (p.absmax) {
#pragma unroll
    for (int o = 32; o > 0; o >>= 1) ymax = fmaxf(ymax, __shfl_xor(ymax, o));
    if (lane == 0) {
      const unsigned bits = __float_as_uint(ymax <= 3.0e38f ? ymax : 3.0e38f);
      if (bits > __atomic_load_n(p.absmax, __ATOMIC_RELAXED)) atomicMax(p.absmax, bits);
    }
  }
}


__global__ __launch_bounds__(256) void fft32_post_bias_kernel(const float* __restrict__ bsum, int nslots, int pack, int cpt, float* __restrict__ dbias) {
  __shared__ float red[256];
  const int ch = blockIdx.x, t = threadIdx.x;
  float a = 0.f;
  for (int sl = t; sl < nslots; sl += 256)
    for (int sub = 0; sub < pack; ++sub) {
      const int c = sub * cpt + ch;
      a += bsum[sl * 64 + c];
      a += bsum[sl * 64 + 32 + c];
    }
  red[t] = a;
  __syncthreads();
  for (int st = 128; st > 0; st >>= 1) { if (t < st) red[t] += red[t + st]; __syncthreads(); }
  if (t == 0) dbias[ch] = red[0];
}

constexpr int T64 = 64, ROWS64 = 4096;
__device__ __forceinline__ void item64(int v, int& tg, int& hf) { tg = (v >> 4) * 8 + (v & 7); hf = (v >> 3) & 1; }

__host__ __device__ __forceinline__ int64_t sp_item64(int64_t item) { return pcnn_spec::sp_item(item, ROWS64); }


struct FwdItem64 {
  const float* img;
  int cl, cr;
  int xlim;
  unsigned voff;
};
struct FwdRow64 {
  float fill;
  unsigned lo;
  bool use_fill;
  bool fetch;
};

__device__ __forceinline__ void fwd64_describe(const FwdParams& p, int v, int lane, int c16, FwdItem64& it, FwdRow64 (&row)[2], int unit0) {
  int tg, hf;
  item64(v, tg, hf);
  const int g = tg % p.groups;
  int t = p.tile0 + tg / p.groups;
  const int tx = t % p.tiles_x; t /= p.tiles_x;
  const int ty = t % p.tiles_y;
  const int n = t / p.tiles_y;
  const int cc = 16 * hf + c16, chan = g * p.cstride + cc;
  const bool cok = cc < p.cvalid && chan < p.C;
  it.img = p.x + (int64_t)n * p.H * p.W * p.ld;
  const int wy0 = ty * p.Vy - p.oy, wx0 = tx * p.Vx - p.ox;
  const int ylim = min(p.ylim, p.ext_y - ty * p.Vy);
  it.xlim = min(p.xlim, p.ext_x - tx * p.Vx);
  it.cl = 0; it.cr = T64;
  if (p.pad_mode == PCNN_PAD_CONSTANT) { it.cl = -wx0; it.cr = p.W - wx0; }
  it.voff = (unsigned)(pad_sel(wx0 + lane, p.W, p.pad_mode) * p.ld);
#pragma unroll
  for (int u = 0; u < 2; ++u) {
    const int y = 4 * (unit0 + u) + (lane >> 4);
    const int gy = wy0 + y;
    const bool rowconst = p.pad_mode == PCNN_PAD_CONSTANT && (unsigned)gy >= (unsigned)p.H;
    const bool rowzero = !cok || y >= ylim;
    row[u].use_fill = rowzero || rowconst;
    row[u].fill = rowzero ? 0.f : p.pad_value;
    row[u].fetch = 4 * (unit0 + u) < ylim;
    row[u].lo = (unsigned)(pad_sel(gy, p.H, p.pad_mode) * p.W * p.ld) + (unsigned)(cok ? chan : 0);
  }
}

template <int Un>
__device__ __forceinline__ void fwd64_request(const FwdItem64& it, const FwdRow64 (&row)[2], float (&R)[2][64]) {
#pragma unroll
  for (int x = 0; x < T64; ++x) {
    const float* rp = it.img + (unsigned)__builtin_amdgcn_readlane((int)it.voff, x);
    R[Un][x] = row[Un].fetch ? rp[row[Un].lo] : 0.f;
  }
}

template <bool MASKED>
__device__ __forceinline__ void fwd64_consume(const FwdParams& p, const FwdItem64& it, const FwdRow64& row, float (&R)[64]) {
#pragma unroll
  for (int x = 0; x < T64; ++x) {
    float v = R[x];
    if (x < it.cl || x >= it.cr) v = p.pad_value;
    if (row.use_fill) v = row.fill;
    if (MASKED && x >= it.xlim) v = 0.f;
    R[x] = v;
  }
}

__device__ __forceinline__ void y64_gather(const float* U, int offr, int offi, int cl, float isign, const float* tw, float* vr, float* vi) {
  asm volatile("" : "+v"(offr), "+v"(offi));
  const float* ur = U + offr, *ui = U + offi;
  const bool odd = cl & 1;
  const float sg2 = odd ? -1.f : 1.f;
  const float s = (cl & 2) ? -1.f : 1.f;
#pragma unroll
  for (int y = 0; y < 16; ++y) {
    const float u0r = ur[y * 512], u1r = ur[(y + 16) * 512], u2r = ur[(y + 32) * 512], u3r = ur[(y + 48) * 512];
    const float u0i = isign * ui[y * 512], u1i = isign * ui[(y + 16) * 512], u2i = isign * ui[(y + 32) * 512], u3i = isign * ui[(y + 48) * 512];
    const float ar = fma_(sg2, u2r, u0r), ai = fma_(sg2, u2i, u0i);
    const float wr_ = fma_(sg2, u3r, u1r), wi_ = fma_(sg2, u3i, u1i);
    const float br = odd ? wi_ : wr_, bi = odd ? -wr_ : wi_;
    const float xr = fma_(s, br, ar), xi = fma_(s, bi, ai);
    if (y == 0) { vr[0] = xr; vi[0] = xi; }
    else {
      const float tr = tw[2 * y], ti = tw[2 * y + 1];
      vr[y] = fma_(xr, tr, -(xi * ti));
      vi[y] = fma_(xr, ti, xi * tr);
    }
    if (y & 1) __builtin_amdgcn_sched_barrier(0);
  }
}

template <bool MASKED>
__device__ __forceinline__ void fft64_fwd_body(const FwdParams& p, const int nvirt, float* U, const int bid, const int gdim) {
  const int tid = threadIdx.x, lane = tid & 63, lg = lane >> 4, c16 = lane & 15;
  const int wave = __builtin_amdgcn_readfirstlane(tid >> 6);
  const int ntg = p.ntile * p.groups;
  int v = bid;
  if (v >= nvirt) return;
  float* const TW = U + 64 * 32 * 16;
  if (tid < 64) { TW[2 * tid] = cos64(((tid >> 4) * (tid & 15)) & 63); TW[2 * tid + 1] = -sin64(((tid >> 4) * (tid & 15)) & 63); }
  const float* const tw = TW + lg * 32;
  float R[2][64];
  FwdItem64 cur;
  FwdRow64 row[2];
  auto safe = [&](int vv) { int tg, hf; item64(vv, tg, hf); return tg < ntg ? vv : (vv & 8); };
  fwd64_describe(p, safe(v), lane, c16, cur, row, 2 * wave);
  for (;;) {
    const int next = v + gdim;
    const bool more = next < nvirt;
    fwd64_request<0>(cur, row, R);
    fwd64_request<1>(cur, row, R);
#pragma unroll
    for (int u = 0; u < 2; ++u) {
      __builtin_amdgcn_sched_barrier(0);
      fwd64_consume<MASKED>(p, cur, row[u], R[u]);
      rfft_fwd<64>(R[u]);
      pin<32>(R[u]);
      int uoff = ((4 * (2 * wave + u) + lg) * 32) * 16 + c16;
      asm volatile("" : "+v"(uoff));
      float* urow = U + uoff;
#pragma unroll
      for (int m = 0; m < 16; ++m) {
        urow[m * 16] = R[u][32 + bitrev(m, 16)];
        urow[(16 + m) * 16] = R[u][48 + bitrev(m, 16)];
      }
    }
    lds_barrier();
    int tg, hf;
    item64(v, tg, hf);
    const bool store = tg < ntg;
    float* out = p.sp + sp_item64(store ? tg : 0) + 16 * hf;
    int cl = lg;
    asm volatile("" : "+v"(cl));
#pragma unroll
    for (int u = 0; u < 2; ++u) {
      __builtin_amdgcn_sched_barrier(0);
      const int q = 2 * wave + u;
      const int mcol = (q & 1) ? 15 - (q >> 1) : (q >> 1);
      float V[32];
      float* vr = V, *vi = V + 16;
      y64_gather(U, mcol * 16 + c16, (16 + mcol) * 16 + c16, cl, (q & 1) ? -1.f : 1.f, tw, vr, vi);
      cfft_dif<16, -1>(vr, vi);
      if (store) {
        float* o = out + (128 + 128 * (2 * q)) * RS;
        const unsigned lo = (unsigned)(sp_row_c(64, cl, 0) * RS + c16);
#pragma unroll
        for (int m = 0; m < 16; ++m) {
          __builtin_nontemporal_store(vr[bitrev(m, 16)], &(o + (sp_row_c(64, 4 * m, 0) * RS))[lo]);
          __builtin_nontemporal_store(vi[bitrev(m, 16)], &(o + (sp_row_c(64, 4 * m, 1) * RS))[lo]);
        }
      }
    }
    lds_barrier();
#pragma unroll
    for (int u = 0; u < 2; ++u) {
      int uoff = ((4 * (2 * wave + u) + lg) * 32) * 16 + c16;
      asm volatile("" : "+v"(uoff));
      float* urow = U + uoff;
      float (&E)[32] = *reinterpret_cast<float (*)[32]>(&R[u][0]);
#pragma unroll
      for (int s2 = 0; s2 < 32; ++s2) urow[s2 * 16] = hc_get(E, s2);
    }
    if (more) fwd64_describe(p, safe(next), lane, c16, cur, row, 2 * wave);
    lds_barrier();
    asm volatile("" : "+v"(cl));
#pragma unroll
    for (int u = 0; u < 2; ++u) {
      __builtin_amdgcn_sched_barrier(0);
      const int q = 2 * wave + u;
      float V[32];
      float* vr = V, *vi = V + 16;
      if (q < 15) {
        y64_gather(U, (q + 1) * 16 + c16, (17 + q) * 16 + c16, cl, 1.f, tw, vr, vi);
        cfft_dif<16, -1>(vr, vi);
        if (store) {
          float* o = out + (128 + 128 * (2 * (q + 1) - 1)) * RS;
          const unsigned lo = (unsigned)(sp_row_c(64, cl, 0) * RS + c16);
#pragma unroll
          for (int m = 0; m < 16; ++m) {
            __builtin_nontemporal_store(vr[bitrev(m, 16)], &(o + (sp_row_c(64, 4 * m, 0) * RS))[lo]);
            __builtin_nontemporal_store(vi[bitrev(m, 16)], &(o + (sp_row_c(64, 4 * m, 1) * RS))[lo]);
          }
        }
      } else {
        int uuoff = ((cl & 2) ? 16 : 0) * 16 + c16;
        asm volatile("" : "+v"(uuoff));
        const float* uu = U + uuoff;
        float* o = out;
        const unsigned lo = (unsigned)(((cl & 2) ? 64 : 0) * RS + c16);
        if ((cl & 1) == 0) {
#pragma unroll
          for (int yy = 0; yy < 32; ++yy) V[yy] = uu[yy * 512] + uu[(yy + 32) * 512];
          rfft_fwd<32>(V);
          if (store) {
#pragma unroll
            for (int k = 0; k <= 16; ++k) __builtin_nontemporal_store(hc_get(V, k), &(o + (sp_row_r(64, 2 * k) * RS))[lo]);
#pragma unroll
            for (int k = 1; k < 16; ++k) __builtin_nontemporal_store(hc_get(V, 16 + k), &(o + (sp_row_r(64, 32 + 2 * k) * RS))[lo]);
          }
        } else {
#pragma unroll
          for (int n2 = 0; n2 < 16; ++n2) {
            const float dr = uu[n2 * 512] - uu[(n2 + 32) * 512], di = uu[(n2 + 48) * 512] - uu[(n2 + 16) * 512];
            mul_tw<64, -1>(n2, dr, di, vr[n2], vi[n2]);
          }
          cfft_dif<16, -1>(vr, vi);
          if (store) {
#pragma unroll
            for (int m = 0; m < 8; ++m) {
              __builtin_nontemporal_store(vr[bitrev(m, 16)], &(o + (sp_row_r(64, 4 * m + 1) * RS))[lo]);
              __builtin_nontemporal_store(vi[bitrev(m, 16)], &(o + (sp_row_r(64, 32 + 4 * m + 1) * RS))[lo]);
              __builtin_nontemporal_store(vr[bitrev(15 - m, 16)], &(o + (sp_row_r(64, 4 * m + 3) * RS))[lo]);
              __builtin_nontemporal_store(-vi[bitrev(15 - m, 16)], &(o + (sp_row_r(64, 32 + 4 * m + 3) * RS))[lo]);
            }
          }
        }
      }
    }
    if (!more) break;
    v = __builtin_amdgcn_readfirstlane(next);
    lds_barrier();
  }
}

template <bool MASKED>
__global__ __launch_bounds__(512) void fft64_fwd_kernel(FwdParams p, int nvirt) {
  extern __shared__ __attribute__((aligned(16))) float U[];
  fft64_fwd_body<MASKED>(p, nvirt, U, blockIdx.x, gridDim.x);
}

__global__ __launch_bounds__(512) void fft64_fwd_multi_kernel(const FwdParams* __restrict__ tab) {
  extern __shared__ __attribute__((aligned(16))) float U[];
  const FwdParams p = load_fwd_params(tab + blockIdx.y);
  const int ntg = p.ntile * p.groups;
  fft64_fwd_body<true>(p, 2 * ((ntg + 7) & ~7), U, blockIdx.x, gridDim.x);
}

constexpr int G_YS = 528, G_CS = 16 * G_YS + 16;
constexpr size_t LDS64I_BYTES = (4 * G_CS + 128) * sizeof(float);

template <bool TANH, bool RES, bool POST>
__global__ __launch_bounds__(512) void fft64_inv_kernel(InvParams p, int nvirt) {
  extern __shared__ __attribute__((aligned(16))) float G[];
  const int tid = threadIdx.x, lane = tid & 63, lg = lane >> 4, c16 = lane & 15;
  const int wave = __builtin_amdgcn_readfirstlane(tid >> 6);
  const int ntg = p.ntile * p.groups;
  int v = blockIdx.x;
  if (v >= nvirt) return;
  float* const TW = G + 4 * G_CS;
  if (tid < 64) { TW[2 * tid] = cos64(((tid >> 4) * (tid & 15)) & 63); TW[2 * tid + 1] = -sin64(((tid >> 4) * (tid & 15)) & 63); }
  const float* const tw = TW + lg * 32;
  float ymax = 0.f, bsum = 0.f;
  constexpr int BURST = 8;
  for (;;) {
    const int next = v + gridDim.x;
    int tg, hf;
    item64(v, tg, hf);
    const bool live = tg < ntg;
    const float* in = p.sp + sp_item64(live ? tg : 0) + 16 * hf;
    float R[2][64];
    int cl = lg;
#pragma unroll
    for (int phase = 0; phase < 2; ++phase) {
      lds_barrier();
      asm volatile("" : "+v"(cl));
#pragma unroll
      for (int u = 0; u < 2; ++u) {
        __builtin_amdgcn_sched_barrier(0);
        const int q = 2 * wave + u;
        float V[32];
        float* vr = V, *vi = V + 16;
        int sre;
        if (phase == 1 && q == 15) {
          sre = 0;
          const unsigned lo = (unsigned)c16;
#pragma unroll
          for (int m = 0; m < 16; ++m) {
            const int fy = 4 * m + cl, fp = fy <= 32 ? fy : 64 - fy;
            const float sg = fy <= 32 ? 1.f : -1.f;
            const bool hasim = fp != 0 && fp != 32;
            const unsigned rr = (unsigned)(sp_row_r(64, fp) * RS), ri = (unsigned)(sp_row_r(64, 32 + (hasim ? fp : 1)) * RS);
            const float ar = in[lo + rr], br = (in + 64 * RS)[lo + rr];
            float ai = in[lo + ri], bi = (in + 64 * RS)[lo + ri];
            ai = hasim ? sg * ai : 0.f; bi = hasim ? sg * bi : 0.f;
            vr[m] = ar - bi; vi[m] = ai + br;
          }
        } else {
          int fx;
          if (phase == 0) {
            fx = 2 * q + 1;
            sre = (q & 1) ? 15 - (q >> 1) : (q >> 1);
          } else { fx = 2 * (q + 1); sre = q + 1; }
          const float* src = in + (128 + 128 * (fx - 1)) * RS;
          const unsigned lo = (unsigned)(sp_row_c(64, cl, 0) * RS + c16);
#pragma unroll
          for (int m = 0; m < 16; ++m) {
            vr[m] = (src + sp_row_c(64, 4 * m, 0) * RS)[lo];
            vi[m] = (src + sp_row_c(64, 4 * m, 1) * RS)[lo];
          }
        }
        cfft_dif<16, +1>(vr, vi);
        int goff = cl * G_CS + sre * 16 + c16;
        asm volatile("" : "+v"(goff));
        float* g = G + goff;
#pragma unroll
        for (int y = 0; y < 16; ++y) {
          const float ar = vr[bitrev(y, 16)], ai = vi[bitrev(y, 16)];
          float gr, gi;
          if (y == 0) { gr = ar; gi = ai; }
          else {
            const float tr = tw[2 * y], ti = -tw[2 * y + 1];
            gr = fma_(ar, tr, -(ai * ti));
            gi = fma_(ar, ti, ai * tr);
          }
          g[y * G_YS] = gr;
          g[y * G_YS + 256] = gi;
        }
      }
      lds_barrier();
#pragma unroll
      for (int u = 0; u < 2; ++u) {
        __builtin_amdgcn_sched_barrier(0);
        const int unit = 2 * wave + u, j = unit >> 2;
        const int y = (4 * unit + lg) & 15;
        int goff = y * G_YS + c16;
        asm volatile("" : "+v"(goff));
        const float* g0 = G + goff;
        const bool swp = j & 1;
        const float s2 = (j & 1) ? -1.f : 1.f;
        const float s1r = (j == 0) ? 1.f : (j == 1 ? -1.f : (j == 2 ? -1.f : 1.f)), s1i = (j == 0) ? 1.f : (j == 1 ? 1.f : (j == 2 ? -1.f : -1.f));
        const float s3r = (j == 0) ? 1.f : (j == 1 ? 1.f : (j == 2 ? -1.f : -1.f)), s3i = (j == 0) ? 1.f : (j == 1 ? -1.f : (j == 2 ? -1.f : 1.f));
#pragma unroll
        for (int k = 0; k < 16; ++k) {
          const float a0 = g0[k * 16], b0 = g0[k * 16 + 256];
          const float a1 = g0[G_CS + k * 16], b1 = g0[G_CS + k * 16 + 256];
          const float a2 = g0[2 * G_CS + k * 16], b2 = g0[2 * G_CS + k * 16 + 256];
          const float a3 = g0[3 * G_CS + k * 16], b3 = g0[3 * G_CS + k * 16 + 256];
          const float p1 = swp ? b1 : a1, q1 = swp ? a1 : b1, p3 = swp ? b3 : a3, q3 = swp ? a3 : b3;
          float re = fma_(s2, a2, a0), im = fma_(s2, b2, b0);
          re = fma_(s1r, p1, re); im = fma_(s1i, q1, im);
          re = fma_(s3r, p3, re); im = fma_(s3i, q3, im);
          asm volatile("" : "+v"(re), "+v"(im));
          if (phase == 0) {
            R[u][32 + bitrev(k, 16)] = re;
            R[u][48 + bitrev(k, 16)] = k >= 8 ? -im : im;
          } else {
            float (&E)[32] = *reinterpret_cast<float (*)[32]>(&R[u][0]);
            if (k == 0) { hc_put(E, 0, re); hc_put(E, 16, im); }
            else { hc_put(E, k, re); hc_put(E, 16 + k, im); }
          }
          if ((k & 3) == 3) __builtin_amdgcn_sched_barrier(0);
        }
      }
    }
    {
      const int g = tg % p.groups;
      int t = p.tile0 + (live ? tg : 0) / p.groups;
      const int tx = t % p.tiles_x; t /= p.tiles_x;
      const int ty = t % p.tiles_y;
      const int n = t / p.tiles_y;
      const int y0 = ty * p.Vy, x0 = tx * p.Vx;
      const int vy = min(p.Vy, p.Ho - y0), vx = min(p.Vx, p.Wo - x0);
      const int cc = 16 * hf + c16, chan = g * p.cstride + cc;
      const bool cok = live && cc < p.cvalid && chan < p.C;
      const float bias = (p.bias && cok) ? p.bias[chan] : 0.f;
      const float sc = (p.bn_scale && cok) ? p.bn_scale[chan] : 1.f, sh = (p.bn_scale && cok) ? p.bn_shift[chan] : 0.f;
      const int sgn = p.flip ? -1 : 1;
      const int64_t ipix = (int64_t)n * p.Ho * p.Wo;
      float* yimg = p.y + ipix * p.ldy;
      float* aimg = (!POST && p.act_out) ? p.act_out + ipix * p.ld_act : nullptr;
      const float* rimg = RES ? p.res + ipix * p.ld_res : nullptr;
      const float* gimg = POST ? p.gact + ipix * p.ld_gact : nullptr;
      float* y2img = (POST && p.y2) ? p.y2 + ipix * p.ld_y2 : nullptr;
      const unsigned chv = (unsigned)chan;
#pragma unroll
      for (int u = 0; u < 2; ++u) {
        __builtin_amdgcn_sched_barrier(0);
        const int unit = 2 * wave + u;
        if (4 * unit >= vy) continue;
        const int yy = 4 * unit + lg;
        rfft_inv<64>(R[u]);
        const int prow = p.flip ? p.Ho - 1 - y0 - yy : y0 + yy, pcol = p.flip ? p.Wo - 1 - x0 : x0;
        unsigned pix0 = (unsigned)(prow * p.Wo + pcol);
        asm volatile("" : "+v"(pix0));
        if (cok && yy < vy)
          epilogue_row<TANH, RES, POST, T64, BURST, true>(p, R[u], 1.f / 4096.f, vx, pix0, sgn, chv, bias, sc, sh, yimg, aimg, rimg, gimg, y2img, ymax, bsum, NoBetween(),
                                                          __builtin_amdgcn_readfirstlane(vx));
      }
    }
    if (next >= nvirt) break;
    v = __builtin_amdgcn_readfirstlane(next);
  }
  if (POST && p.bsum) p.bsum[(blockIdx.x * 8 + wave) * 64 + lane] += bsum;
  if (p.absmax) {
#pragma unroll
    for (int o = 32; o > 0; o >>= 1) ymax = fmaxf(ymax, __shfl_xor(ymax, o));
    if (lane == 0) {
      const unsigned bits = __float_as_uint(ymax <= 3.0e38f ? ymax : 3.0e38f);
      if (bits > __atomic_load_n(p.absmax, __ATOMIC_RELAXED)) atomicMax(p.absmax, bits);
    }
  }
}

__global__ __launch_bounds__(256) void fft64_post_bias_kernel(const float* __restrict__ bsum, int nblocks, float* __restrict__ dbias) {
  __shared__ float red[256];
  const int ch = blockIdx.x, t = threadIdx.x, hf = ch >> 4, c16 = ch & 15;
  float a = 0.f;
  for (int sl = t; sl < nblocks * 8 * 4; sl += 256) {
    const int lgq = sl & 3, bw = sl >> 2, block = bw >> 3;
    if (((block >> 3) & 1) == hf) a += bsum[(size_t)bw * 64 + lgq * 16 + c16];
  }
  red[t] = a;
  __syncthreads();
  for (int st = 128; st > 0; st >>= 1) { if (t < st) red[t] += red[t + st]; __syncthreads(); }
  if (t == 0) dbias[ch] = red[0];
}

constexpr size_t LDS64_BYTES = LDS_BYTES + 128 * sizeof(float);

void launch_fwd_fft32(pcnn_handle h, FwdParams p, int ntile) {
  p.ntile = ntile;
  const dim3 grid((unsigned)std::min(ntile * p.groups, 256));
  if (p.ylim < T || p.xlim < T) {
    set_lds(fft32_fwd_kernel<true>, LDS_BYTES);
    hipLaunchKernelGGL((fft32_fwd_kernel<true>), grid, dim3(1024), LDS_BYTES, h->stream, p);
  } else {
    set_lds(fft32_fwd_kernel<false>, LDS_BYTES);
    hipLaunchKernelGGL((fft32_fwd_kernel<false>), grid, dim3(1024), LDS_BYTES, h->stream, p);
  }
}

void launch_fwd_fft32_multi(pcnn_handle h, const FwdParams* tab, int count, int max_items) {
  set_lds(fft32_fwd_multi_kernel, LDS_BYTES);
  hipLaunchKernelGGL(fft32_fwd_multi_kernel, dim3((unsigned)std::min(max_items, 64), (unsigned)count), dim3(1024), LDS_BYTES, h->stream, tab);
}
void launch_fwd_fft64_multi(pcnn_handle h, const FwdParams* tab, int count, int max_items) {
  set_lds(fft64_fwd_multi_kernel, LDS64_BYTES);
  const int nvirt = 2 * ((max_items + 7) & ~7);
  hipLaunchKernelGGL(fft64_fwd_multi_kernel, dim3((unsigned)std::min((nvirt + 15) & ~15, 64), (unsigned)count), dim3(512), LDS64_BYTES, h->stream, tab);
}

void launch_post_bias_fft32(pcnn_handle h, const float* bsum, int pack, int cpt, int C, float* dbias) {
  hipLaunchKernelGGL(fft32_post_bias_kernel, dim3((unsigned)C), dim3(256), 0, h->stream, bsum, XFORM_FFT32.post_slots, pack, cpt, dbias);
}
void launch_post_bias_fft64(pcnn_handle h, const float* bsum, int, int, int C, float* dbias) {
  hipLaunchKernelGGL(fft64_post_bias_kernel, dim3((unsigned)C), dim3(256), 0, h->stream, bsum, POST_BLOCKS, dbias);
}

void launch_fwd_fft64(pcnn_handle h, FwdParams p, int ntile) {
  p.ntile = ntile;
  const int ntg = ntile * p.groups;
  const int nvirt = 2 * ((ntg + 7) & ~7);
  const dim3 grid((unsigned)std::min((nvirt + 15) & ~15, 256));
  const bool masked = p.ylim < T64 || p.xlim < T64 || p.ext_y < (1 << 29) || p.ext_x < (1 << 29);
  if (masked) {
    set_lds(fft64_fwd_kernel<true>, LDS64_BYTES);
    hipLaunchKernelGGL((fft64_fwd_kernel<true>), grid, dim3(512), LDS64_BYTES, h->stream, p, nvirt);
  } else {
    set_lds(fft64_fwd_kernel<false>, LDS64_BYTES);
    hipLaunchKernelGGL((fft64_fwd_kernel<false>), grid, dim3(512), LDS64_BYTES, h->stream, p, nvirt);
  }
}

void launch_inv_fft64(pcnn_handle h, InvParams p, int ntile) {
  p.ntile = ntile;
  const int ntg = ntile * p.groups;
  const int nvirt = 2 * ((ntg + 7) & ~7);
  const dim3 grid((unsigned)std::min((nvirt + 15) & ~15, 256));
  dispatch_epilogue(p, [&](auto TANH, auto RES, auto POST, const InvParams& q) {
    constexpr auto kernel = fft64_inv_kernel<TANH.value, RES.value, POST.value>;
    set_lds(kernel, LDS64I_BYTES);
    hipLaunchKernelGGL(kernel, grid, dim3(512), LDS64I_BYTES, h->stream, q, nvirt);
  });
}

void launch_inv_fft32(pcnn_handle h, InvParams p, int ntile) {
  p.ntile = ntile;
  const dim3 grid((unsigned)std::min(ntile * p.groups, 256));
  dispatch_epilogue(p, [&](auto TANH, auto RES, auto POST, const InvParams& q) {
    constexpr auto kernel = fft32_inv_kernel<TANH.value, RES.value, POST.value>;
    set_lds(kernel, LDS_BYTES);
    hipLaunchKernelGGL(kernel, grid, dim3(1024), LDS_BYTES, h->stream, q);
  });
}

}

#ifndef __HIP_DEVICE_COMPILE__
const Xform XFORM_FFT32 = {PCNN_XFORM_FFT, T, ROWS, ROWS / 2, SP_P, O_TAB32, O_SLOTS32F, launch_fwd_fft32, launch_inv_fft32, launch_post_bias_fft32,
                           launch_fwd_fft32_multi, POST_BLOCKS * 16, nullptr, nullptr};
const Xform XFORM_FFT64 = {PCNN_XFORM_FFT, T64, ROWS64, ROWS64 / 2, SP_P, O_TAB64, O_SLOTS64F, launch_fwd_fft64, launch_inv_fft64, launch_post_bias_fft64,
                           launch_fwd_fft64_multi, POST_BLOCKS * 8, nullptr, nullptr};
#endif

}
```

poisson_cnn_amd/layers.py:

```python
import numpy as np
import torch

from . import ops
from .utils import advanced_pad_amounts, canonical_activation, glorot_limit, same_pad_amounts, split_indices


class ParamStore:

    def __init__(self):
        self.specs = []
        self.bn_layers = []
        self.finalized = False

    def add(self, name, shape, init, kind='w'):
        assert not self.finalized
        self.specs.append((name, tuple(int(s) for s in shape), init, kind))
        return name

    def add_bn(self, name, c):
        off = sum(ch for _, ch in self.bn_layers)
        self.bn_layers.append((name, c))
        for suffix, init, kind in (('gamma', 'ones', 'bn_gamma'), ('beta', 'zeros', 'bn_beta'), ('moving_mean', 'zeros', 'bn_mean'),
                                   ('moving_variance', 'ones', 'bn_var')):
            self.add('%s/%s' % (name, suffix), (c,), init, kind)
# ... 129 lines not shown
        if self.side is not None:
            torch.cuda.current_stream().wait_stream(self.side)
        self.side_reads.clear()

    def before_inplace_write(self, t):
        ev = self.side_reads.pop(t.data_ptr(), None)
        if ev is not None:
            torch.cuda.current_stream().wait_event(ev)

    def wflip(self, shape, device):
        n = int(np.prod(shape))
        key = self._stream_key()
        buf = self._wflips.get(key)
        if buf is None or buf.numel() < n:
            buf = self._wflips[key] = torch.empty(n, dtype=torch.float32, device=device)
        return buf[:n].view(shape)


class ConvUnit:

    def __init__(self, store, ctx, name, k, cin, cout, *, pad='advanced', padding_mode='CONSTANT', pad_value=0.0, activation='linear',
                 use_bias=True, bn_name=None, stride=1):
        self.store, self.ctx, self.name = store, ctx, name
        self.stride = int(stride)
        if self.stride > 1 and pad != 'advanced':
            raise NotImplementedError('strided convolutions are implemented for the advanced-padding form (the only strided use in the reference)')
        self.kh, self.kw = (int(k), int(k)) if np.isscalar(k) else (int(k[0]), int(k[1]))
        self.k = self.kw
        self.cin, self.cout = int(cin), int(cout)
        amounts = advanced_pad_amounts if pad == 'advanced' else same_pad_amounts
        self.pads_y, self.pads_x = amounts(self.kh), amounts(self.kw)
        self.pads = self.pads_x
        self.mode = padding_mode.upper() if pad == 'advanced' else 'CONSTANT'
        if self.mode not in ops.PAD_MODES:
            raise ValueError('unknown padding mode ' + padding_mode)
        self.pad_value = float(pad_value) if pad == 'advanced' else 0.0
        self.act = canonical_activation(activation)
        self.use_bias = use_bias
        store.add(name + '/kernel', (self.kh, self.kw, self.cin, self.cout), 'glorot')
        if use_bias:
            store.add(name + '/bias', (self.cout,), 'zeros')
        self.bn_name = bn_name
        if bn_name is not None:
            self.bn_off = store.add_bn(bn_name, self.cout)
        self.saved = None

    def _bn(self):
        if self.bn_name is None:
            return None, None
        s = self.store
        return s.bn_scale[self.bn_off:self.bn_off + self.cout], s.bn_shift[self.bn_off:self.bn_off + self.cout]

    def forward(self, x, residual=None, out=None, training=True, x_absmax=None):
        if self.stride > 1:
            assert residual is None and out is None
            full = self._forward(x, training=training, x_absmax=x_absmax)
            self.out_absmax = None
            self._full_hw = (full.shape[1], full.shape[2])
            return ops.subsample(full, self.stride)
        return self._forward(x, residual=residual, out=out, training=training, x_absmax=x_absmax)

    def _forward(self, x, residual=None, out=None, training=True, x_absmax=None):
        self.out_absmax = None
        ops.sync_flipped_filters(self.store.filter_version())
        w = self.store.w[self.name + '/kernel']
        b = self.store.w[self.name + '/bias'] if self.use_bias else None
        sc, sh = self._bn()
        N, H, W, _ = x.shape
        if out is None:
            out = ops.empty((N, H, W, self.cout), x.device)
        if self.bn_name is not None and training and getattr(self.store, 'bn_training', False):
            a = ops.empty((N, H, W, self.cout), x.device)
            ops.conv2d_fwd(x, w, b, pad_top=self.pads_y[0], pad_left=self.pads_x[0], pad_mode=self.mode, pad_value=self.pad_value, act=self.act, out=a,
                           w_version=self.store.filter_version())
            sw = self.store.w
            _, stats = ops.bn_train_forward(a, sw[self.bn_name + '/gamma'], sw[self.bn_name + '/beta'], sw[self.bn_name + '/moving_mean'],
                                            sw[self.bn_name + '/moving_variance'], residual=residual, out=out, ws=self.ctx.ws)
            self.saved = (x, a, stats, x_absmax)
            return out
        need_a = training and (sc is not None or residual is not None)
        a = ops.empty((N, H, W, self.cout), x.device) if need_a else None
        if training and ops.get_math_mode() == 'split_f16':
            self.out_absmax = ops.empty((1,), x.device)
        ops.conv2d_fwd(x, w, b, pad_top=self.pads_y[0], pad_left=self.pads_x[0], pad_mode=self.mode, pad_value=self.pad_value, act=self.act,
                       bn_scale=sc, bn_shift=sh, residual=residual, out=out, act_out=a, y_absmax=self.out_absmax, w_version=self.store.filter_version())
        if training:
            self.saved = (x, a if a is not None else out, None, x_absmax)
        return out

    def _flipped(self, w):
        ver = self.store.filter_version()
        wf = getattr(self, '_wf', None)
        if wf is None or wf.device != w.device:
            self._wf = torch.empty((self.kh, self.kw, self.cout, self.cin), dtype=torch.float32, device=w.device)
            self._wf_ver = None
            ops.register_flipped(self)
        if ver and self._wf_ver is not None and self._wf_ver != ver:
            ops.sync_flipped_filters(ver)
        if not ver or self._wf_ver != ver:
            self._reflip(ver)
        return self._wf, ver

    def _reflip(self, ver):
        ops.flip_transpose_weights(self.store.w[self.name + '/kernel'], out=self._wf)
        self._wf_ver = ver

    def post_spec(self, want_raw=False):
        if self.saved is None or self.stride > 1 or self.saved[2] is not None:
            return None
        sc, _ = self._bn()
        if sc is None and self.act == 'linear':
            return None
        s = self.store
        s1 = s.bn_s1[self.bn_off:self.bn_off + self.cout] if sc is not None else None
        s2 = s.bn_s2[self.bn_off:self.bn_off + self.cout] if sc is not None else None
        return ops.Post(self.saved[1], self.act, s.g[self.name + '/bias'] if self.use_bias else None, want_raw, bn_scale=sc, s_dy_a=s1, s_dy=s2)

    def backward(self, dy, need_dx=True, inplace=False, add_to=None, dz_ready=False, post=None):
        if self.stride > 1:
            dy, inplace = ops.subsample_bwd(dy, self._full_hw, self.stride), True
        x, a, bn_stats, x_absmax = self.saved
        self.saved = None
        s, g = self.store, self.store.g
        N, H, W, _ = x.shape
        sc, _ = self._bn()
        if bn_stats is not None:
            dy = ops.bn_train_backward(dy, a, bn_stats, g[self.bn_name + '/gamma'], g[self.bn_name + '/beta'], ws=self.ctx.ws)
            sc, inplace = None, True
        dense = ops._ld(dy) == self.cout
        dz = dy if (inplace and dense) else ops.empty((N, H, W, self.cout), dy.device)
        s1 = s.bn_s1[self.bn_off:self.bn_off + self.cout] if sc is not None else None
        s2 = s.bn_s2[self.bn_off:self.bn_off + self.cout] if sc is not None else None
        trivial = self.act == 'linear' and sc is None
        amax = None
        if dz_ready:
            assert bn_stats is None
            dz = dy
        elif trivial and not self.use_bias:
            dz = dy
        else:
            if not trivial and ops.get_math_mode() == 'split_f16':
                amax = ops.empty((1,), dy.device)
            ops.epilogue_bwd(dy, a if (self.act != 'linear' or sc is not None) else None, act=self.act, bn_scale=sc, dz=None if trivial else dz,
                             dbias=g[self.name + '/bias'] if self.use_bias else None, s_dy_a=s1, s_dy=s2, ws=self.ctx.ws, dz_absmax=amax)
            if trivial:
                dz = dy
        w = s.w[self.name + '/kernel']
        kh, kw = self.kh, self.kw
        wf, wver = None, 0
        if need_dx:
            wf, wver = self._flipped(w)
            res = add_to if (self.mode == 'CONSTANT') else None
            out = ops.conv2d_bwd_fused(x, dz, w.shape, wf, pad_top=self.pads_y[0], pad_left=self.pads_x[0], pad_mode=self.mode, pad_value=self.pad_value,
                                       dw=g[self.name + '/kernel'], residual=res, post=post, w_version=wver)
            if out is not None:
                if self.mode == 'CONSTANT':
                    return out
                if post is not None and not post.applied:
                    dzp = ops.pad_fold_bwd_post(out, (H, W), (self.pads_y, self.pads_x), self.mode, post, add_to=add_to, ws=self.ctx.ws)
                    if dzp is not None:
                        return dzp
                if add_to is not None and add_to.is_contiguous():
                    self.ctx.before_inplace_write(add_to)
                    return ops.pad_fold_bwd(out, (H, W), (self.pads_y, self.pads_x), self.mode, out=add_to, accumulate=True)
                dx = ops.pad_fold_bwd(out, (H, W), (self.pads_y, self.pads_x), self.mode)
                return dx if add_to is None else ops.axpby(1.0, add_to, 1.0, dx)
        side = self.ctx.side_stream()
        if side is None:
            ops.conv2d_wgrad(x, dz, w.shape, pad_top=self.pads_y[0], pad_left=self.pads_x[0], pad_mode=self.mode, pad_value=self.pad_value,
                             out=g[self.name + '/kernel'], ws=self.ctx.ws, x_absmax=x_absmax, dz_absmax=amax)
        else:
            ev = torch.cuda.Event()
            ev.record()
            with torch.cuda.stream(side):
                side.wait_event(ev)
                for t in (x, dz, x_absmax, amax):
                    if t is not None:
                        t.record_stream(side)
                ops.conv2d_wgrad(x, dz, w.shape, pad_top=self.pads_y[0], pad_left=self.pads_x[0], pad_mode=self.mode, pad_value=self.pad_value,
                                 out=g[self.name + '/kernel'], ws=self.ctx.ws_side, x_absmax=x_absmax, dz_absmax=amax)
                done = torch.cuda.Event()
                done.record()
            self.ctx.side_reads[dz.data_ptr()] = done
        if not need_dx:
            return None
        if self.mode == 'CONSTANT':
            if post is not None and not post.applied:
                dxp = ops.conv2d_dgrad_post(dz, wf, pad_top=kh - 1 - self.pads_y[0], pad_left=kw - 1 - self.pads_x[0], out_hw=(H, W), residual=add_to, post=post)
                if dxp is not None:
                    return dxp
            return ops.conv2d_fwd(dz, wf, None, pad_top=kh - 1 - self.pads_y[0], pad_left=kw - 1 - self.pads_x[0], residual=add_to, w_version=wver)
        gp = ops.conv2d_fwd(dz, wf, None, pad_top=kh - 1, pad_left=kw - 1, out_hw=(H + kh - 1, W + kw - 1), w_version=wver)
        if post is not None and not post.applied:
            dzp = ops.pad_fold_bwd_post(gp, (H, W), (self.pads_y, self.pads_x), self.mode, post, add_to=add_to, ws=self.ctx.ws)
            if dzp is not None:
                return dzp
        if add_to is not None and add_to.is_contiguous():
            self.ctx.before_inplace_write(add_to)
            return ops.pad_fold_bwd(gp, (H, W), (self.pads_y, self.pads_x), self.mode, out=add_to, accumulate=True)
        dx = ops.pad_fold_bwd(gp, (H, W), (self.pads_y, self.pads_x), self.mode)
        return dx if add_to is None else ops.axpby(1.0, add_to, 1.0, dx)


class resnet:

    def __init__(self, store, ctx, name, filters, kernel_size, *, use_batchnorm=False, padding_mode='constant', constant_padding_value=0.0,
                 activation='linear', use_bias=True):
        kw = dict(padding_mode=padding_mode, pad_value=constant_padding_value, activation=activation, use_bias=use_bias)
        self.c0 = ConvUnit(store, ctx, name + '/conv0', kernel_size, filters, filters, **kw)
        self.c1 = ConvUnit(store, ctx, name + '/conv1', kernel_size, filters, filters, **kw)
        self.c2 = ConvUnit(store, ctx, name + '/conv2', kernel_size, filters, filters, **kw)
        if use_batchnorm:
            for i, c in enumerate((self.c0, self.c1)):
                c.bn_name = '%s/bn%d' % (name, i)
                c.bn_off = store.add_bn(c.bn_name, filters)

    def _fusable(self, x, out):
        cs = (self.c0, self.c1, self.c2)
        c = self.c0
        return (all(u.kh == 3 and u.kw == 3 and u.cin == c.cin and u.cout == c.cin and u.mode == 'CONSTANT' and u.pad_value == 0.0 and u.stride == 1
                    and u.bn_name is None and u.act == c.act and u.pads_y == (1, 1) and u.pads_x == (1, 1) for u in cs)
                and x.is_contiguous() and x.shape[3] == c.cin and (out is None or out.is_contiguous())
                and ops.get_math_mode() == 'fp32' and ops.resnet3_eligible(c.cin, c.act))

    def forward(self, x, out=None, training=True, x_absmax=None):
        if self._fusable(x, out):
            w = self.c0.store.w
            wb = [(w[u.name + '/kernel'], w[u.name + '/bias'] if u.use_bias else None) for u in (self.c0, self.c1, self.c2)]
            y, o0, a1, o1 = ops.resnet3_fwd(x, wb[0][0], wb[0][1], wb[1][0], wb[1][1], wb[2][0], wb[2][1], act=self.c0.act, training=training, out=out)
            if training:
                self.c0.saved, self.c1.saved, self.c2.saved = (x, o0, None, None), (o0, a1, None, None), (o1, y, None, None)
            self.c0.out_absmax = self.c1.out_absmax = self.c2.out_absmax = self.out_absmax = None
            return y
        o = self.c0.forward(x, training=training, x_absmax=x_absmax)
        o = self.c1.forward(o, residual=x, training=training, x_absmax=self.c0.out_absmax)
        o = self.c2.forward(o, out=out, training=training, x_absmax=self.c1.out_absmax)
        self.out_absmax = self.c2.out_absmax
        return o

    def post_spec(self, want_raw=False):
        return self.c2.post_spec(want_raw)

    def backward(self, dy, inplace=False, dz_ready=False, post=None):
        p1 = self.c1.post_spec(want_raw=True)
        d1 = self.c2.backward(dy, inplace=inplace, dz_ready=dz_ready, post=p1)
        ready1 = p1 is not None and p1.applied
        d1raw = p1.raw if ready1 else d1
        p0 = self.c0.post_spec()
        d0 = self.c1.backward(d1, inplace=ready1, dz_ready=ready1, post=p0)
        ready0 = p0 is not None and p0.applied
        return self.c0.backward(d0, inplace=True, add_to=d1raw, dz_ready=ready0, post=post)


class _bottleneck_base:

    def __init__(self, store, ctx, name, cin, *, downsampling_factor, filters, conv_kernel_size, n_convs=1, upsampling_factor=None,
                 padding_mode='constant', constant_padding_value=0.0, conv_activation='linear', conv_use_bias=True, use_resnet=False,
                 downsampling_method='conv', conv_downsampling_kernel_size=None, pool_downsampling_method='max', use_batchnorm=False, **unused):
        self.name, self.f = name, int(downsampling_factor)
        self.up = int(upsampling_factor) if upsampling_factor is not None else self.f
        self.downsampling_factor = self.f
        self.filters = filters
        self.method = downsampling_method.lower()
        self.pool = pool_downsampling_method.lower()
        kw = dict(padding_mode=padding_mode, pad_value=constant_padding_value, activation=conv_activation, use_bias=conv_use_bias)
        self.down_conv = None
        self.stages = []
        n_layers = 0
        if self.method == 'conv':
            if conv_downsampling_kernel_size is None:
                raise ValueError('conv_downsampling_kernel_size is required for downsampling_method="conv"')
            self.down_conv = ConvUnit(store, ctx, name + '/downsample', conv_downsampling_kernel_size, cin, filters, stride=self.f, **kw)
            c = filters
        elif self.method == 'pool':
            c = cin
            if use_resnet:
                self.stages.append(ConvUnit(store, ctx, name + '/conv0', conv_kernel_size, cin, filters, **kw))
                n_layers, c = 1, filters
        else:
            raise ValueError('Downsampling method can only be conv or pool')
        i = 0
        while n_layers < n_convs:
            if use_resnet:
                self.stages.append(resnet(store, ctx, '%s/res%d' % (name, i), filters, conv_kernel_size, use_batchnorm=use_batchnorm, padding_mode=padding_mode,
                                          constant_padding_value=constant_padding_value, activation=conv_activation, use_bias=conv_use_bias))
                n_layers += 1
            else:
                self.stages.append(ConvUnit(store, ctx, '%s/conv%d' % (name, i), conv_kernel_size, c, filters,
                                            bn_name=('%s/bn%d' % (name, i)) if use_batchnorm else None, **kw))
                n_layers += 2 if use_batchnorm else 1
                c = filters
            i += 1
        self.conv0 = self.stages[0] if (self.method == 'pool' and use_resnet) else None
        self.res = [st for st in self.stages if isinstance(st, resnet)]

    def _down_and_convs(self, x, training, pooled=None):
        self.x = x if training else None
        self._pooled_given = pooled is not None
        hint = None
        if self.down_conv is not None:
            o = self.down_conv.forward(x, training=training)
        elif pooled is not None:
            o = pooled
        else:
            o = ops.pool2d_fwd(x, self.f, self.pool)
        for st in self.stages:
            o = st.forward(o, training=training, x_absmax=hint)
            hint = st.out_absmax
        return o
# ... 286 lines not shown
```

poisson_cnn_amd/ops.py:

```python
import ctypes
from ctypes import byref, c_float, c_int, c_int64, c_size_t, c_void_p

import numpy as np
import torch

from . import _lib
from ._lib import ConvDesc

PAD_MODES = {'CONSTANT': 0, 'SYMMETRIC': 1, 'REFLECT': 2}
ACTS = {'linear': 0, 'leaky_relu': 1, 'tanh': 2, 'relu': 3}
POOLS = {'average': 0, 'avg': 0, 'max': 1}
RESIZE = {'nearest': 0, 'bilinear': 1, 'bicubic': 2, 'bicubic_legacy': 3}
LEAKY_ALPHA = 0.2
BN_EPS = 1e-3

_handles = {}
MATH_MODES = {'fp32': 0, 'split_f16': 1}
_math_mode = MATH_MODES[__import__('os').environ.get('PCNN_MATH', 'fp32')]


def set_math_mode(mode):
    global _math_mode
    _math_mode = MATH_MODES[mode]
    for h in _handles.values():
# ... 91 lines not shown


_flip_table = (None, None, 0, 0)


def _flip_layer_set():
    layers = sorted((l for l in _flip_layers if getattr(l, '_wf', None) is not None), key=id)
    return layers, tuple((id(l), l._wf.data_ptr()) for l in layers)


def _build_flip_table(layers, key):
    global _flip_table
    arr = np.zeros(len(layers), dtype=[('w', '<u8'), ('wt', '<u8'), ('kh', '<i4'), ('kw', '<i4'), ('ci', '<i4'), ('co', '<i4'), ('start', '<i8')])
    start = 0
    for i, l in enumerate(layers):
        w = l.store.w[l.name + '/kernel']
        arr[i] = (w.data_ptr(), l._wf.data_ptr(), l.kh, l.kw, l.cin, l.cout, start)
        start += w.numel()
    _flip_table = (key, torch.from_numpy(arr.view(np.uint8)).to(layers[0]._wf.device), len(layers), start)


def prepare_flip_table_for_capture():
    layers, key = _flip_layer_set()
    if not layers:
        return []
    if key != _flip_table[0]:
        _build_flip_table(layers, key)
    return [_flip_table[1]] + [l._wf for l in layers]


def sync_flipped_filters(version):
    global _flips_version, _flip_table
    if not version or version == _flips_version:
        return
    layers, key = _flip_layer_set()
    if layers:
        if key != _flip_table[0] and torch.cuda.is_current_stream_capturing():
            for l in layers:
                l._reflip(version)
            _flips_version = version
            return
        if key != _flip_table[0]:
            _build_flip_table(layers, key)
        _, tab, n, total = _flip_table
        handle().call('pcnn_conv2d_flip_transpose_table', _p(tab), c_int(n), c_int64(total))
        for l in layers:
            l._wf_ver = version
    _flips_version = version


class _FilterVersion:
    __slots__ = ('h', 'v')

    def __init__(self, h, v):
        self.h, self.v = h, int(v or 0)

    def __enter__(self):
        if self.v:
            h = self.h
            if getattr(h, '_fepoch', 0) != _filter_epoch:
                if torch.cuda.is_current_stream_capturing():
                    self.v = 0
                    return
                h.call('pcnn_filter_cache_clear')
                h._fepoch = _filter_epoch
            h.call('pcnn_set_filter_version', self.v)

    def __exit__(self, *exc):
        if self.v:
            self.h.call('pcnn_set_filter_version', 0)
        return False


def handle():
    dev = torch.cuda.current_device()
    st = torch.cuda.current_stream().cuda_stream
    h = _handles.get((dev, st))
    if h is None:
        h = _lib.Handle(dev, st)
        h.call('pcnn_set_math_mode', c_int(_math_mode))
        h.call('pcnn_set_spectral_mode', c_int(_spectral_mode))
        h.call('pcnn_set_spectral_tile', c_int(_spectral_tile))
        h.call('pcnn_set_spectral_transform', c_int(_spectral_xform))
        _handles[(dev, st)] = h
    return h


def release_stream_handle(stream_ptr, device=None):
    dev = torch.cuda.current_device() if device is None else device
    h = _handles.pop((dev, int(stream_ptr)), None)
    if h is not None:
        try:
            h.call('pcnn_set_workspace_retain', c_int(0))
        finally:
            del h


def _p(t):
    return c_void_p(t.data_ptr()) if t is not None else c_void_p(0)


def _chk(t, name='tensor'):
    if t.dtype != torch.float32 or not t.is_cuda:
        raise ValueError('%s must be a CUDA float32 tensor' % name)
    if t.dim() > 0 and t.stride(-1) != 1 and t.shape[-1] != 1:
        raise ValueError('%s must have unit channel stride (NHWC)' % name)
    return t


def _ld(t):
    _chk(t)
    N, H, W, C = t.shape
    if W > 1:
        ld = t.stride(2)
    elif H > 1:
        ld = t.stride(1)
    elif N > 1:
        ld = t.stride(0)
    else:
        ld = max(C, 1)
    if (W > 1 and t.stride(2) != ld) or (H > 1 and t.stride(1) != W * ld) or (N > 1 and t.stride(0) != H * W * ld) or ld < C:
        raise ValueError('tensor is not pixel-linear NHWC (strides %s for shape %s)' % (t.stride(), tuple(t.shape)))
    return ld


def empty(shape, device='cuda'):
    return torch.empty(shape, dtype=torch.float32, device=device)


def zeros(shape, device='cuda'):
    return torch.zeros(shape, dtype=torch.float32, device=device)


class Workspace:

    def __init__(self):
        self.buf = None

    def get(self, nbytes, device='cuda'):
        n = (int(nbytes) + 3) // 4 + 16
        if self.buf is None or self.buf.numel() < n:
            self.buf = None
            self.buf = torch.empty(n, dtype=torch.float32, device=device)
        return self.buf


_default_ws = Workspace()
_post_fusion = __import__('os').environ.get('PCNN_POST_FUSION', '1') != '0'


def set_post_fusion(on):
    global _post_fusion
    _post_fusion = bool(on)


_stage_fusion = __import__('os').environ.get('PCNN_STAGE_FUSION', '1') != '0'


def set_stage_fusion(on):
    global _stage_fusion
    _stage_fusion = bool(on)


class KernelTimer:

    def __init__(self):
        self.records = []

    def launch(self, kind, flops, fn, nbytes=0.0):
        s, e = torch.cuda.Event(enable_timing=True), torch.cuda.Event(enable_timing=True)
        s.record()
        fn()
        e.record()
        self.records.append((kind, flops, s, e, nbytes))

    def total_bytes(self, kind):
        return sum(r[4] for r in self.records if r[0] == kind)

    def select(self, pred):
        torch.cuda.synchronize()
        sel = [r for r in self.records if pred(r[0], r[1], r[4])]
        return sum(r[1] for r in sel), sum(r[4] for r in sel), sum(r[2].elapsed_time(r[3]) for r in sel) * 1e-3, len(sel)

    def totals(self, kind):
        torch.cuda.synchronize()
        sel = [r for r in self.records if r[0] == kind]
        return sum(r[1] for r in sel), sum(r[2].elapsed_time(r[3]) for r in sel) * 1e-3, len(sel)


_timer = None


def set_kernel_timer(t):
    global _timer
    _timer = t


def _launch(kind, flops, fn, nbytes=0.0):
    if _timer is None:
        fn()
    else:
        _timer.launch(kind, flops, fn, nbytes)


def conv_desc(x_shape, ldx, w_shape, out_hw, ldy, pad_top, pad_left, pad_mode='CONSTANT', pad_value=0.0, act='linear', ld_res=0, ld_act=0):
    N, H, W, Cin = x_shape
    kh, kw, ci, Cout = w_shape
    assert ci == Cin, (ci, Cin)
    return ConvDesc(N, H, W, Cin, ldx, out_hw[0], out_hw[1], Cout, ldy, kh, kw, pad_top, pad_left, PAD_MODES[pad_mode.upper()],
                    float(pad_value), ACTS[act], LEAKY_ALPHA, ld_res, ld_act)


def conv2d_fwd(x, w, bias=None, *, pad_top, pad_left, out_hw=None, pad_mode='CONSTANT', pad_value=0.0, act='linear',
               bn_scale=None, bn_shift=None, residual=None, out=None, act_out=None, y_absmax=None, w_version=0):
    N, H, W, Cin = x.shape
    kh, kw, ci, Cout = w.shape
    assert w.is_contiguous()
    Ho, Wo = out_hw if out_hw is not None else (H, W)
    if out is None:
        out = empty((N, Ho, Wo, Cout), x.device)
    d = conv_desc(x.shape, _ld(x), w.shape, (Ho, Wo), _ld(out), pad_top, pad_left, pad_mode, pad_value, act,
                  _ld(residual) if residual is not None else 0, _ld(act_out) if act_out is not None else 0)
    def run():
        h = handle()
        with _FilterVersion(h, w_version):
            h.call('pcnn_conv2d_fwd_absmax', byref(d), _p(x), _p(w), _p(bias), _p(bn_scale), _p(bn_shift), _p(residual), _p(out), _p(act_out), _p(y_absmax))
    _launch('conv_fwd', 2.0 * N * Ho * Wo * kh * kw * Cin * Cout, run,
            4.0 * (N * H * W * Cin + N * Ho * Wo * Cout * (1 + (residual is not None) + (act_out is not None)) + kh * kw * Cin * Cout))
    return out


def conv2d_dgrad_post(dz, wf, *, pad_top, pad_left, out_hw, residual, post):
    if post is None or post.bn_scale is not None or not _post_fusion:
        return None
    N, H, W, Cin = dz.shape
    kh, kw, _, Cout = wf.shape
    Ho, Wo = out_hw
    out = empty((N, Ho, Wo, Cout), dz.device)
    dg = conv_desc(dz.shape, _ld(dz), wf.shape, (Ho, Wo), _ld(out), pad_top, pad_left, 'CONSTANT', 0.0, 'linear', _ld(residual) if residual is not None else 0, 0)
    raw = empty((N, Ho, Wo, Cout), dz.device) if post.want_raw else None
    pd = PostDesc(post.a.data_ptr(), _ld(post.a), ACTS[post.act], LEAKY_ALPHA, post.dbias.data_ptr() if post.dbias is not None else None,
                  raw.data_ptr() if raw is not None else None, Cout)
    h = handle()
    if tuple(post.a.shape) != (N, Ho, Wo, Cout) or not h.lib.pcnn_conv2d_dgrad_post_eligible(h._h, byref(dg), _p(dz), _p(residual), _p(out), byref(pd)):
        return None
    _launch('conv_fwd_post', 2.0 * N * Ho * Wo * kh * kw * Cin * Cout,
            lambda: h.call('pcnn_conv2d_dgrad_post', byref(dg), _p(dz), _p(wf), _p(residual), _p(out), byref(pd)),
            4.0 * (N * H * W * Cin + N * Ho * Wo * Cout * (1 + (residual is not None)) + kh * kw * Cin * Cout))
    post.applied, post.raw = True, raw
    return out


def flip_transpose_weights(w, out=None):
    kh, kw, ci, co = w.shape
    wt = out if out is not None else empty((kh, kw, co, ci), w.device)
    handle().call('pcnn_conv2d_flip_transpose_weights', _p(w), _p(wt), c_int(kh), c_int(kw), c_int(ci), c_int(co))
    return wt


def conv2d_wgrad(x, dz, w_shape, *, pad_top, pad_left, pad_mode='CONSTANT', pad_value=0.0, out=None, ws=None, x_absmax=None, dz_absmax=None):
    N, Ho, Wo, Cout = dz.shape
    d = conv_desc(x.shape, _ld(x), w_shape, (Ho, Wo), _ld(dz), pad_top, pad_left, pad_mode, pad_value)
    lib = _lib.load()
    nbytes = lib.pcnn_conv2d_wgrad_workspace(byref(d))
    wsb = (ws or _default_ws).get(nbytes, x.device)
    dw = out if out is not None else empty(tuple(w_shape), x.device)
    assert dw.is_contiguous()
    _launch('conv_wgrad', 2.0 * N * Ho * Wo * w_shape[0] * w_shape[1] * w_shape[2] * w_shape[3],
            lambda: handle().call('pcnn_conv2d_wgrad_hint', byref(d), _p(x), _p(dz), _p(dw), _p(wsb), c_size_t(wsb.numel() * 4), _p(x_absmax), _p(dz_absmax)),
            4.0 * (x.shape[0] * x.shape[1] * x.shape[2] * x.shape[3] + N * Ho * Wo * Cout + w_shape[0] * w_shape[1] * w_shape[2] * w_shape[3]))
    return dw


class PostDesc(ctypes.Structure):
    _fields_ = [('act_out', c_void_p), ('ld_act_out', c_int), ('act', c_int), ('act_alpha', c_float), ('dbias', c_void_p), ('raw_out', c_void_p), ('ld_raw', c_int)]


class Post:

    def __init__(self, a, act, dbias=None, want_raw=False, bn_scale=None, s_dy_a=None, s_dy=None):
        self.a, self.act, self.dbias, self.want_raw = a, act, dbias, want_raw
        self.bn_scale, self.s_dy_a, self.s_dy = bn_scale, s_dy_a, s_dy
        self.applied, self.raw = False, None


def conv2d_bwd_fused(x, dz, w_shape, wf, *, pad_top, pad_left, pad_mode='CONSTANT', pad_value=0.0, dw, residual=None, post=None, w_version=0):
    N, H, W, Cin = x.shape
    kh, kw, _, Cout = w_shape
    mode = pad_mode.upper()
    d = conv_desc(x.shape, _ld(x), w_shape, (dz.shape[1], dz.shape[2]), _ld(dz), pad_top, pad_left, mode, pad_value)
    if mode == 'CONSTANT':
        out_hw, dpt, dpl = (H, W), kh - 1 - pad_top, kw - 1 - pad_left
    else:
        out_hw, dpt, dpl = (dz.shape[1] + kh - 1, dz.shape[2] + kw - 1), kh - 1, kw - 1
        residual = None
    ldo = Cin
    dg = conv_desc(dz.shape, _ld(dz), (kh, kw, Cout, Cin), out_hw, ldo, dpt, dpl, 'CONSTANT', 0.0, 'linear', _ld(residual) if residual is not None else 0, 0)
    h = handle()
    if not h.lib.pcnn_conv2d_bwd_spectral_eligible(h._h, byref(d), byref(dg)):
        return None
    out = empty((N, out_hw[0], out_hw[1], Cin), x.device)
    flops = 2.0 * N * dz.shape[1] * dz.shape[2] * kh * kw * Cin * Cout
    nbytes = 4.0 * (2 * N * H * W * Cin + N * dz.shape[1] * dz.shape[2] * Cout + 2 * kh * kw * Cin * Cout)
    if post is not None and post.bn_scale is None and mode == 'CONSTANT' and _post_fusion and h.lib.pcnn_conv2d_bwd_spectral_post_eligible(h._h, byref(d), byref(dg)):
        post.raw = empty((N, H, W, Cin), x.device) if post.want_raw else None
        pd = PostDesc(post.a.data_ptr(), _ld(post.a), ACTS[post.act], LEAKY_ALPHA, post.dbias.data_ptr() if post.dbias is not None else None,
                      post.raw.data_ptr() if post.raw is not None else None, Cin)
        def run_post():
            with _FilterVersion(h, w_version):
                h.call('pcnn_conv2d_bwd_spectral_post', byref(d), byref(dg), _p(x), _p(dz), _p(wf), _p(residual), _p(out), _p(dw), byref(pd))
        _launch('conv_bwd_fused', 2.0 * flops, run_post, nbytes)
        post.applied = True
        return out
    def run():
        with _FilterVersion(h, w_version):
            h.call('pcnn_conv2d_bwd_spectral', byref(d), byref(dg), _p(x), _p(dz), _p(wf), _p(residual), _p(out), _p(dw))
    _launch('conv_bwd_fused', 2.0 * flops, run, nbytes)
    return out


def resnet3_eligible(C, act):
    h = handle()
    return _stage_fusion and bool(h.lib.pcnn_resnet3_fwd_eligible(h._h, c_int(C), c_int(ACTS[act])))


def resnet3_fwd(x, w0, b0, w1, b1, w2, b2, *, act, training, out=None):
    N, H, W, C = x.shape
    assert x.is_contiguous() and w0.shape == (3, 3, C, C) and w1.shape == (3, 3, C, C) and w2.shape == (3, 3, C, C)
    if out is None:
        out = empty((N, H, W, C), x.device)
    assert out.is_contiguous() and out.shape == x.shape
    o0, a1, o1 = (empty((N, H, W, C), x.device) for _ in range(3)) if training else (None, None, None)
    T = 4.0 * N * H * W * C
    nbytes = (8.0 if training else 7.0) * T + 3 * 4.0 * 9 * C * C
    _launch('conv_stage', 3 * 2.0 * N * H * W * 9 * C * C,
            lambda: handle().call('pcnn_resnet3_fwd', c_int(N), c_int(H), c_int(W), c_int(C), c_int(ACTS[act]), c_float(LEAKY_ALPHA), _p(x), _p(w0), _p(b0),
                                  _p(w1), _p(b1), _p(w2), _p(b2), _p(o0), _p(a1), _p(o1), _p(out)), nbytes)
    return out, o0, a1, o1


def epilogue_bwd(dy, a, *, act='linear', bn_scale=None, dz=None, dbias=None, s_dy_a=None, s_dy=None, ws=None, dz_absmax=None):
    N, H, W, C = dy.shape
    lib = _lib.load()
    wsb = (ws or _default_ws).get(lib.pcnn_colsum_workspace(c_int(C)), dy.device)
    handle().call('pcnn_conv2d_epilogue_bwd_absmax', c_int64(N * H * W), c_int(C), _p(dy), c_int(_ld(dy)), _p(a), c_int(_ld(a) if a is not None else 0),
                  _p(bn_scale), c_int(ACTS[act]), c_float(LEAKY_ALPHA), _p(dz), c_int(_ld(dz) if dz is not None else 0),
                  _p(dbias), _p(s_dy_a), _p(s_dy), _p(dz_absmax), _p(wsb), c_size_t(wsb.numel() * 4))
    return dz


def pad_fold_bwd(gp, out_hw, pads, pad_mode, out=None, accumulate=False):
    N, Hp, Wp, C = gp.shape
    H, W = out_hw
    (pt, pb), (pl, pr) = pads
    assert Hp == H + pt + pb and Wp == W + pl + pr
    gx = out if out is not None else empty((N, H, W, C), gp.device)
    handle().call('pcnn_pad_fold_bwd', c_int(N), c_int(H), c_int(W), c_int(C), c_int(pt), c_int(pb), c_int(pl), c_int(pr),
                  c_int(PAD_MODES[pad_mode.upper()]), _p(gp), c_int(_ld(gp)), _p(gx), c_int(_ld(gx)), c_int(1 if accumulate else 0))
    return gx


def pad_fold_bwd_post(gp, out_hw, pads, pad_mode, post, add_to=None, ws=None):
    if not _post_fusion:
        return None
    N, Hp, Wp, C = gp.shape
    H, W = out_hw
    (pt, pb), (pl, pr) = pads
    assert Hp == H + pt + pb and Wp == W + pl + pr
    lib = _lib.load()
    dz = empty((N, H, W, C), gp.device)
    raw = empty((N, H, W, C), gp.device) if post.want_raw else None
    pd = PostDesc(post.a.data_ptr(), _ld(post.a), ACTS[post.act], LEAKY_ALPHA, post.dbias.data_ptr() if post.dbias is not None else None,
                  raw.data_ptr() if raw is not None else None, C)
    if add_to is not None and not (add_to.dim() == 4 and tuple(add_to.shape) == (N, H, W, C)):
        return None
    ld_add = _ld(add_to) if add_to is not None else 0
    if not lib.pcnn_pad_fold_bwd_post_eligible(c_int(C), c_int(_ld(gp)), c_int(ld_add), _p(gp), _p(add_to), byref(pd), c_int(_ld(dz)), _p(dz)):
        return None
    wsb = (ws or _default_ws).get(lib.pcnn_colsum_workspace(c_int(C)), gp.device)
    handle().call('pcnn_pad_fold_bwd_post', c_int(N), c_int(H), c_int(W), c_int(C), c_int(pt), c_int(pb), c_int(pl), c_int(pr), c_int(PAD_MODES[pad_mode.upper()]),
                  _p(gp), c_int(_ld(gp)), _p(add_to), c_int(ld_add), byref(pd), _p(post.bn_scale), _p(post.s_dy_a), _p(post.s_dy), _p(dz), c_int(_ld(dz)),
                  _p(wsb), c_size_t(wsb.numel() * 4))
    post.raw, post.applied = raw, True
    return dz


def bn_fold(gamma, beta, mean, var, scale, shift, eps=BN_EPS):
    handle().call('pcnn_bn_fold', c_int(gamma.numel()), _p(gamma), _p(beta), _p(mean), _p(var), c_float(eps), _p(scale), _p(shift))


def bn_fold_bwd(s1, s2, mean, var, dgamma, dbeta, eps=BN_EPS):
    handle().call('pcnn_bn_fold_bwd', c_int(s1.numel()), _p(s1), _p(s2), _p(mean), _p(var), c_float(eps), _p(dgamma), _p(dbeta))


def channel_affine(x, scale, shift, residual=None, out=None):
    N, H, W, C = x.shape
    y = out if out is not None else empty((N, H, W, C), x.device)
    handle().call('pcnn_channel_affine', c_int64(N * H * W), c_int(C), _p(x), c_int(_ld(x)), _p(scale), _p(shift), _p(residual),
                  c_int(_ld(residual) if residual is not None else 0), _p(y), c_int(_ld(y)))
    return y


def bn_train_forward(a, gamma, beta, moving_mean, moving_var, residual=None, out=None, momentum=0.99, eps=BN_EPS, ws=None):
    N, H, W, C = a.shape
    lib = _lib.load()
    st = empty((5, C), a.device)
    mean, inv_std, scale = st[0], st[1], st[2]
    y = out if out is not None else empty((N, H, W, C), a.device)
    wsb = (ws or _default_ws).get(lib.pcnn_colsum_workspace(c_int(C)), a.device)
    handle().call('pcnn_bn_train_fwd', c_int64(N * H * W), c_int(C), _p(a), c_int(_ld(a)), _p(gamma), _p(beta), c_float(eps), c_float(momentum),
                  _p(moving_mean), _p(moving_var), _p(mean), _p(inv_std), _p(scale), _p(st[3:]), _p(residual),
                  c_int(_ld(residual) if residual is not None else 0), _p(y), c_int(_ld(y)), _p(wsb), c_size_t(wsb.numel() * 4))
    return y, (mean, inv_std, scale)


def bn_train_backward(dy, a, stats, dgamma, dbeta, ws=None):
    N, H, W, C = dy.shape
    mean, inv_std, scale = stats
    lib = _lib.load()
    tmp = empty((4, C), dy.device)
    wsb = (ws or _default_ws).get(lib.pcnn_colsum_workspace(c_int(C)), dy.device)
    da = empty((N, H, W, C), dy.device)
    handle().call('pcnn_bn_train_bwd', c_int64(N * H * W), c_int(C), _p(dy), c_int(_ld(dy)), _p(a), c_int(_ld(a)), _p(scale), _p(mean), _p(inv_std),
                  _p(dgamma), _p(dbeta), _p(tmp), _p(da), c_int(C), _p(wsb), c_size_t(wsb.numel() * 4))
    return da


def pool_out(n, f):
    return -(-n // f)


def pool2d_fwd(x, f, kind='average', out=None):
    N, H, W, C = x.shape
    y = out if out is not None else empty((N, pool_out(H, f), pool_out(W, f), C), x.device)
    handle().call('pcnn_pool2d_fwd', c_int(POOLS[kind.lower()]), c_int(N), c_int(H), c_int(W), c_int(C), c_int(f), _p(x), c_int(_ld(x)), _p(y), c_int(_ld(y)))
    return y


def pool2d_bwd(x, dy, f, kind='average', dx=None, accumulate=False):
    N, H, W, C = x.shape
    if dx is None:
        dx = empty((N, H, W, C), x.device)
        accumulate = False
    handle().call('pcnn_pool2d_bwd', c_int(POOLS[kind.lower()]), c_int(N), c_int(H), c_int(W), c_int(C), c_int(f), _p(x), c_int(_ld(x)),
                  c_void_p(0), c_int(0), _p(dy), c_int(_ld(dy)), _p(dx), c_int(_ld(dx)), c_int(1 if accumulate else 0))
    return dx


def _deconv_same_pads(k, hc, wc, H, W, f):
    kh, kw = k.shape[0], k.shape[1]
    if hc != -(-H // f) or wc != -(-W // f):
        raise ValueError('SAME transposed convolution needs input = ceil(output / stride): got %s for output %s at stride %d' % ((hc, wc), (H, W), f))
    return max((hc - 1) * f + kh - H, 0) // 2, max((wc - 1) * f + kw - W, 0) // 2


def _deconv_general_fwd(x, k, bias, out_hw, f, alpha, beta, out):
    N, hc, wc, Cin = x.shape
    kh, kw, Cout, _ = k.shape
    H, W = out_hw
    pt, pl = _deconv_same_pads(k, hc, wc, H, W, f)
    x_up = subsample_bwd(x, ((hc - 1) * f + 1, (wc - 1) * f + 1), f)
    y = conv2d_fwd(x_up, flip_transpose_weights(k.contiguous()), bias, pad_top=kh - 1 - pt, pad_left=kw - 1 - pl, out_hw=(H, W))
    if out is None:
        return y if alpha == 1.0 else axpby(alpha, y, 0.0, y)
    return axpby(alpha, y, beta, out)


def deconv_fwd(x, k, bias, out_hw, f, *, alpha=1.0, beta=0.0, out=None):
    N, hc, wc, Cin = x.shape
    Cout = k.shape[2]
    H, W = out_hw
# ... 876 lines not shown
```

Baseline: 43.36 grids/s.

## Fold symmetric/reflect pad gradient into spectral inverse FFT epilogue

For non-constant padded convolutions, the backward spectral dgrad now folds the padded-domain gradient back onto the unpadded image inside the inverse FFT kernels. Pad strips are staged in LDS and summed into interior pixels, and residual add and activation backward happen in the same kernel. This removes the separate full-size padded dx buffer and the pad_fold_bwd pass over it. In exchange it adds a new FOLD template variant, LDS staging and geometry eligibility checks, so ineligible layers fall back to the old path.

```diff
diff --git a/include/pcnn.h b/include/pcnn.h
--- a/include/pcnn.h
+++ b/include/pcnn.h
@@ -87,6 +87,11 @@
 int pcnn_conv2d_bwd_spectral_post_eligible(pcnn_handle h, const pcnn_conv_desc* d, const pcnn_conv_desc* dg);
 int pcnn_conv2d_bwd_spectral_post(pcnn_handle h, const pcnn_conv_desc* d, const pcnn_conv_desc* dg, const float* x, const float* dz, const float* w_flipped,
                                   const float* residual, float* dx, float* dw, const pcnn_post_desc* post);
+
+int pcnn_spectral_fold_geometry_ok(int H, int W, int pt, int pb, int pl, int pr, int pad_mode, int Vy, int Vx);
+int pcnn_conv2d_bwd_spectral_fold_eligible(pcnn_handle h, const pcnn_conv_desc* d, const pcnn_conv_desc* dg);
+int pcnn_conv2d_bwd_spectral_fold(pcnn_handle h, const pcnn_conv_desc* d, const pcnn_conv_desc* dg, const float* x, const float* dz, const float* w_flipped,
+                                  const float* add_to, float* dx, float* dw, const pcnn_post_desc* post);
 
 int pcnn_conv2d_dgrad_post_eligible(pcnn_handle h, const pcnn_conv_desc* dg, const float* dz, const float* residual, const float* dx, const pcnn_post_desc* post);
 int pcnn_conv2d_dgrad_post(pcnn_handle h, const pcnn_conv_desc* dg, const float* dz, const float* w_flipped, const float* residual, float* dx,
diff --git a/poisson_cnn_amd/csrc/pcnn_internal.h b/poisson_cnn_amd/csrc/pcnn_internal.h
--- a/poisson_cnn_amd/csrc/pcnn_internal.h
+++ b/poisson_cnn_amd/csrc/pcnn_internal.h
@@ -33,3 +33,19 @@
   else r = i < 0 ? -i : 2 * n - 2 - i;
   return r < 0 ? 0 : (r >= n ? n - 1 : r);
 }
+
+__host__ __device__ __forceinline__ int pcnn_pad_fold_sources(int i, int n, int pn, int pf, int mode, int (&src)[3]) {
+  bool near = false, far = false;
+  int vn = 0, vf = 0;
+  if (mode == PCNN_PAD_SYMMETRIC) {
+    near = i < pn; vn = pn - 1 - i;
+    far = n - 1 - i < pf; vf = pn + n + (n - 1 - i);
+  } else if (mode == PCNN_PAD_REFLECT) {
+    near = i >= 1 && i <= pn; vn = pn - i;
+    far = n - 2 - i >= 0 && n - 2 - i < pf; vf = pn + n + (n - 2 - i);
+  }
+  src[0] = i + pn;
+  src[1] = near ? vn : vf;
+  src[2] = vf;
+  return 1 + (near ? 1 : 0) + (far ? 1 : 0);
+}
diff --git a/poisson_cnn_amd/csrc/pointwise.hip b/poisson_cnn_amd/csrc/pointwise.hip
--- a/poisson_cnn_amd/csrc/pointwise.hip
+++ b/poisson_cnn_amd/csrc/pointwise.hip
@@ -117,20 +117,8 @@
   const int64_t total = (int64_t)N * H * W * C;
   for (int64_t i = (int64_t)blockIdx.x * blockDim.x + threadIdx.x; i < total; i += (int64_t)gridDim.x * blockDim.x) {
     const int c = i % C; int64_t r = i / C; const int x = r % W; r /= W; const int y = r % H; const int n = r / H;
-    int ys[3], xs[3], ny = 0, nx = 0;
-    ys[ny++] = y + pt;
-    xs[nx++] = x + pl;
-    if (mode == PCNN_PAD_SYMMETRIC) {
-      if (y < pt) ys[ny++] = pt - 1 - y;
-      if (H - 1 - y < pb) ys[ny++] = pt + H + (H - 1 - y);
-      if (x < pl) xs[nx++] = pl - 1 - x;
-      if (W - 1 - x < pr) xs[nx++] = pl + W + (W - 1 - x);
-    } else if (mode == PCNN_PAD_REFLECT) {
-      if (y >= 1 && y <= pt) ys[ny++] = pt - y;
-      if (H - 2 - y >= 0 && H - 2 - y < pb) ys[ny++] = pt + H + (H - 2 - y);
-      if (x >= 1 && x <= pl) xs[nx++] = pl - x;
-      if (W - 2 - x >= 0 && W - 2 - x < pr) xs[nx++] = pl + W + (W - 2 - x);
-    }
+    int ys[3], xs[3];
+    const int ny = pcnn_pad_fold_sources(y, H, pt, pb, mode, ys), nx = pcnn_pad_fold_sources(x, W, pl, pr, mode, xs);
     float s = 0.f;
     for (int a = 0; a < ny; ++a)
       for (int b = 0; b < nx; ++b) s += gp[(((int64_t)n * Hp + ys[a]) * Wp + xs[b]) * ldgp + c];
@@ -145,20 +133,8 @@
   const int64_t total = (int64_t)N * H * W * CV;
   for (int64_t i = (int64_t)blockIdx.x * blockDim.x + threadIdx.x; i < total; i += (int64_t)gridDim.x * blockDim.x) {
     const int c = (int)(i % CV) << 2; int64_t r = i / CV; const int x = r % W; r /= W; const int y = r % H; const int n = r / H;
-    int ys[3], xs[3], ny = 0, nx = 0;
-    ys[ny++] = y + pt;
-    xs[nx++] = x + pl;
-    if (mode == PCNN_PAD_SYMMETRIC) {
-      if (y < pt) ys[ny++] = pt - 1 - y;
-      if (H - 1 - y < pb) ys[ny++] = pt + H + (H - 1 - y);
-      if (x < pl) xs[nx++] = pl - 1 - x;
-      if (W - 1 - x < pr) xs[nx++] = pl + W + (W - 1 - x);
-    } else if (mode == PCNN_PAD_REFLECT) {
-      if (y >= 1 && y <= pt) ys[ny++] = pt - y;
-      if (H - 2 - y >= 0 && H - 2 - y < pb) ys[ny++] = pt + H + (H - 2 - y);
-      if (x >= 1 && x <= pl) xs[nx++] = pl - x;
-      if (W - 2 - x >= 0 && W - 2 - x < pr) xs[nx++] = pl + W + (W - 2 - x);
-    }
+    int ys[3], xs[3];
+    const int ny = pcnn_pad_fold_sources(y, H, pt, pb, mode, ys), nx = pcnn_pad_fold_sources(x, W, pl, pr, mode, xs);
     float4 s = make_float4(0.f, 0.f, 0.f, 0.f);
     for (int a = 0; a < ny; ++a)
       for (int b = 0; b < nx; ++b) {
@@ -188,20 +164,8 @@
     for (int j = 0; j < 4; ++j) sc[j] = bn_scale ? bn_scale[c + j] : 1.f;
     for (int64_t pix = (int64_t)blockIdx.x * R + r; pix < npix; pix += (int64_t)gridDim.x * R) {
       int64_t t = pix; const int x = t % W; t /= W; const int y = t % H; const int n = t / H;
-      int ys[3], xs[3], ny = 0, nx = 0;
-      ys[ny++] = y + pt;
-      xs[nx++] = x + pl;
-      if (mode == PCNN_PAD_SYMMETRIC) {
-        if (y < pt) ys[ny++] = pt - 1 - y;
-        if (H - 1 - y < pb) ys[ny++] = pt + H + (H - 1 - y);
-        if (x < pl) xs[nx++] = pl - 1 - x;
-        if (W - 1 - x < pr) xs[nx++] = pl + W + (W - 1 - x);
-      } else if (mode == PCNN_PAD_REFLECT) {
-        if (y >= 1 && y <= pt) ys[ny++] = pt - y;
-        if (H - 2 - y >= 0 && H - 2 - y < pb) ys[ny++] = pt + H + (H - 2 - y);
-        if (x >= 1 && x <= pl) xs[nx++] = pl - x;
-        if (W - 2 - x >= 0 && W - 2 - x < pr) xs[nx++] = pl + W + (W - 2 - x);
-      }
+      int ys[3], xs[3];
+      const int ny = pcnn_pad_fold_sources(y, H, pt, pb, mode, ys), nx = pcnn_pad_fold_sources(x, W, pl, pr, mode, xs);
       float4 g = make_float4(0.f, 0.f, 0.f, 0.f);
       for (int ia = 0; ia < ny; ++ia)
         for (int ib = 0; ib < nx; ++ib) {
diff --git a/poisson_cnn_amd/csrc/spectral_common.h b/poisson_cnn_amd/csrc/spectral_common.h
--- a/poisson_cnn_amd/csrc/spectral_common.h
+++ b/poisson_cnn_amd/csrc/spectral_common.h
@@ -74,6 +74,7 @@
   int pack = 1, cpt = 32, tgx = 1;
   const float* gact = nullptr; float* y2 = nullptr; float* bsum = nullptr;
   int ld_gact = 0, ld_y2 = 0, gmode = 0; float galpha = 1.f;
+  int fold = 0, fH = 0, fW = 0, fpt = 0, fpb = 0, fpl = 0, fpr = 0;
 };
 
 constexpr int TAB32_FLOATS = 7168, TAB64_FLOATS = 32768;
diff --git a/poisson_cnn_amd/csrc/spectral_conv.hip b/poisson_cnn_amd/csrc/spectral_conv.hip
--- a/poisson_cnn_amd/csrc/spectral_conv.hip
+++ b/poisson_cnn_amd/csrc/spectral_conv.hip
@@ -1104,8 +1104,47 @@
   return d->Cin <= 32 ? 1 : 0;
 }
 
+static bool fold_axis_ok(int n, int pn, int pf, int V, int mode) {
+  const int r = mode == PCNN_PAD_REFLECT ? 1 : 0;
+  if (pn > 0) {
+    const int j = std::min(pn - 1 + r, n - 1);
+    if (j >= r && (pn - 1 + r - j) / V != (pn + j) / V) return false;
+  }
+  if (pf > 0) {
+    const int j = std::min(pf - 1, n - 1 - r);
+    if (j >= 0 && (pn + n - 1 - r - j) / V != (pn + n + j) / V) return false;
+  }
+  return true;
+}
+extern "C" int pcnn_spectral_fold_geometry_ok(int H, int W, int pt, int pb, int pl, int pr, int pad_mode, int Vy, int Vx) {
+  if (pad_mode != PCNN_PAD_SYMMETRIC && pad_mode != PCNN_PAD_REFLECT) return 0;
+  if (H < 1 || W < 1 || pt < 0 || pb < 0 || pl < 0 || pr < 0 || Vy < 1 || Vx < 1) return 0;
+  return fold_axis_ok(H, pt, pb, Vy, pad_mode) && fold_axis_ok(W, pl, pr, Vx, pad_mode) ? 1 : 0;
+}
+
+extern "C" int pcnn_conv2d_bwd_spectral_fold_eligible(pcnn_handle h, const pcnn_conv_desc* d, const pcnn_conv_desc* dg) {
+  if (!pcnn_conv2d_bwd_spectral_eligible(h, d, dg)) return 0;
+  if (d->pad_mode == PCNN_PAD_CONSTANT) return 0;
+  if (h->spectral_xform != PCNN_XFORM_FFT) return 0;
+  const int pt = d->pad_top, pb = d->kh - 1 - pt, pl = d->pad_left, pr = d->kw - 1 - pl;
+  if (pt < 0 || pb < 0 || pl < 0 || pr < 0 || d->Ho != d->H || d->Wo != d->W || dg->Ho != d->H + d->kh - 1 || dg->Wo != d->W + d->kw - 1) return 0;
+  TileGrid g;
+  if (tile_grid(h, dg, d->kh, d->kw, d->N, dg->Ho, dg->Wo, d->Cin, d->Cout, &g)) return 0;
+  if (g.pack != 1) return 0;
+  if ((size_t)(d->kh - 1 + d->kw - 1) * g.T * (g.T == 64 ? 16 : 32) > (g.T == 64 ? (size_t)33856 : (size_t)32768) || pl > 15) return 0;
+  return pcnn_spectral_fold_geometry_ok(d->H, d->W, pt, pb, pl, pr, d->pad_mode, g.Vy, g.Vx);
+}
+
 static int bwd_spectral_impl(pcnn_handle h, const pcnn_conv_desc* d, const pcnn_conv_desc* dg, const float* x, const float* dz, const float* w_flipped,
-                             const float* residual, float* dx, float* dw, const pcnn_post_desc* post);
+                             const float* residual, float* dx, float* dw, const pcnn_post_desc* post, bool fold = false);
+
+extern "C" int pcnn_conv2d_bwd_spectral_fold(pcnn_handle h, const pcnn_conv_desc* d, const pcnn_conv_desc* dg, const float* x, const float* dz, const float* w_flipped,
+                                             const float* add_to, float* dx, float* dw, const pcnn_post_desc* post) {
+  PCNN_REQUIRE(h, h && d && dg, "pcnn_conv2d_bwd_spectral_fold: null argument");
+  PCNN_REQUIRE(h, pcnn_conv2d_bwd_spectral_fold_eligible(h, d, dg), "pcnn_conv2d_bwd_spectral_fold: layer is not eligible (ask pcnn_conv2d_bwd_spectral_fold_eligible first)");
+  PCNN_REQUIRE(h, !post || (post->act_out && d->Cin <= 32), "pcnn_conv2d_bwd_spectral_fold: the fused activation backward needs act_out and <= 32 input channels");
+  return bwd_spectral_impl(h, d, dg, x, dz, w_flipped, add_to, dx, dw, post, true);
+}
 
 extern "C" int pcnn_conv2d_bwd_spectral(pcnn_handle h, const pcnn_conv_desc* d, const pcnn_conv_desc* dg, const float* x, const float* dz, const float* w_flipped,
                                         const float* residual, float* dx, float* dw) {
@@ -1120,7 +1159,7 @@
 }
 
 static int bwd_spectral_impl(pcnn_handle h, const pcnn_conv_desc* d, const pcnn_conv_desc* dg, const float* x, const float* dz, const float* w_flipped,
-                             const float* residual, float* dx, float* dw, const pcnn_post_desc* post) {
+                             const float* residual, float* dx, float* dw, const pcnn_post_desc* post, bool fold) {
   PCNN_REQUIRE(h, h && d && dg && x && dz && w_flipped && dx && dw, "pcnn_conv2d_bwd_spectral: null argument");
   if (pcnn_check_conv_desc(h, "pcnn_conv2d_bwd_spectral", d, 64, 32, PCNN_ANY) || pcnn_check_conv_desc(h, "pcnn_conv2d_bwd_spectral (dg)", dg, 32, 64, PCNN_ANY)) return 1;
   PCNN_REQUIRE(h, pcnn_conv2d_bwd_spectral_eligible(h, d, dg), "pcnn_conv2d_bwd_spectral: layer is not eligible (ask pcnn_conv2d_bwd_spectral_eligible first)");
@@ -1146,6 +1185,9 @@
   FwdParams fxm = image_fwd_params(g, x, xs, d->H, d->W, d->Cin, d->ldx, gx, padded_domain ? d->pad_top : 0, padded_domain ? d->pad_left : 0, d->pad_mode, 0.f);
   fxm.ylim = g.Vy; fxm.xlim = g.Vx; fxm.ext_y = dg->Ho; fxm.ext_x = dg->Wo;
   InvParams iv = image_inv_params(g, ys, dx, dg->Ho, dg->Wo, dg->Cout, dg->ldy, gx, residual, dg->ld_res);
+  if (fold) {
+    iv.fold = d->pad_mode; iv.fH = d->H; iv.fW = d->W; iv.fpt = d->pad_top; iv.fpb = d->kh - 1 - d->pad_top; iv.fpl = d->pad_left; iv.fpr = d->kw - 1 - d->pad_left;
+  }
   if (post) {
     iv.gact = post->act_out; iv.ld_gact = post->ld_act_out; iv.gmode = post->act; iv.galpha = post->act_alpha;
     iv.y2 = post->raw_out; iv.ld_y2 = post->ld_raw; iv.bsum = post->dbias ? bsum : nullptr;
diff --git a/poisson_cnn_amd/csrc/spectral_fft.hip b/poisson_cnn_amd/csrc/spectral_fft.hip
--- a/poisson_cnn_amd/csrc/spectral_fft.hip
+++ b/poisson_cnn_amd/csrc/spectral_fft.hip
@@ -181,7 +181,7 @@
 }
 
 struct NoBetween { __device__ __forceinline__ void operator()(int) const {} };
-template <bool TANH, bool RES, bool POST, int NPIX, int BURST, bool NT, typename Between = NoBetween>
+template <bool TANH, bool RES, bool POST, int NPIX, int BURST, bool NT, bool FOLD = false, typename Between = NoBetween>
 __device__ __forceinline__ void epilogue_row(const InvParams& p, const float* X, float scale, int vx, unsigned pix0, int sgn, unsigned chv, float bias, float sc, float sh,
                                              float* yimg, float* aimg, const float* rimg, const float* gimg, float* y2img, float& ymax, float& bsum, Between between = Between(),
                                              int vx_uniform = NPIX) {
@@ -203,6 +203,7 @@
     for (int r = 0; r < BURST; ++r) {
       const bool ok = x0b + r < vx;
       float v = X[x0b + r] * scale;
+      if (FOLD && POST) v += 0.f;
       if (!POST) {
         v += bias;
         v = TANH ? tanhf(v) : (v > 0.f ? v : v * p.alpha);
@@ -244,6 +245,73 @@
   }
 }
 
+struct FoldTile { int xlo, ncol; bool edge; };
+__device__ __forceinline__ FoldTile fold_tile(const InvParams& p, int y0, int x0, int vy, int vx) {
+  FoldTile f;
+  f.xlo = max(0, p.fpl - x0);
+  f.ncol = min(vx, p.fpl + p.fW - x0) - f.xlo;
+  f.edge = y0 < p.fpt || y0 + vy > p.fpt + p.fH || x0 < p.fpl || x0 + vx > p.fpl + p.fW;
+  return f;
+}
+__device__ __forceinline__ int fold_strip(int i, int pn, int n) { return i < pn ? i : i - n; }
+template <int TT, int CL>
+__device__ __forceinline__ void fold_put(const InvParams& p, float* S, const float (&X)[TT], int yy, int y0, int x0, int vx, int cl) {
+  asm volatile("" : "+v"(x0), "+v"(vx));
+  const int gy = y0 + yy;
+  if (gy < p.fpt || gy >= p.fpt + p.fH) {
+    float* r = S + (fold_strip(gy, p.fpt, p.fH) * TT) * CL + cl;
+#pragma unroll
+    for (int x = 0; x < TT; ++x) r[x * CL] = X[x];
+  }
+  if (x0 < p.fpl || x0 + vx > p.fpl + p.fW) {
+    float* q = S + ((p.fpt + p.fpb) * TT + yy * (p.fpl + p.fpr)) * CL + cl;
+#pragma unroll
+    for (int x = 0; x < TT; ++x) {
+      const int gx = x0 + x;
+      if (x < vx && (gx < p.fpl || gx >= p.fpl + p.fW)) q[fold_strip(gx, p.fpl, p.fW) * CL] = X[x];
+    }
+  }
+}
+template <int TT, int CL>
+__device__ __forceinline__ void fold_add(const InvParams& p, const float* S, float (&X)[TT], int yy, int y0, int x0, int vx, int cl) {
+  asm volatile("" : "+v"(x0), "+v"(vx));
+  int ys[3], xs[3];
+  const int ny = pcnn_pad_fold_sources(y0 + yy - p.fpt, p.fH, p.fpt, p.fpb, p.fold, ys);
+  const float* const q = S + ((p.fpt + p.fpb) * TT + yy * (p.fpl + p.fpr)) * CL + cl;
+#pragma unroll
+  for (int x = 0; x < TT; ++x) {
+    const int ix = x0 + x - p.fpl;
+    if (x < vx && ix >= 0 && ix < p.fW) {
+      const int nx = pcnn_pad_fold_sources(ix, p.fW, p.fpl, p.fpr, p.fold, xs);
+      if (ny + nx > 2) {
+        float s = 0.f;
+        s += X[x];
+#pragma unroll
+        for (int b = 1; b < 3; ++b)
+          if (b < nx) s += q[fold_strip(xs[b], p.fpl, p.fW) * CL];
+#pragma unroll
+        for (int a = 1; a < 3; ++a)
+          if (a < ny) {
+            const float* r = S + (fold_strip(ys[a], p.fpt, p.fH) * TT - x0) * CL + cl;
+#pragma unroll
+            for (int b = 0; b < 3; ++b)
+              if (b < nx) s += r[xs[b] * CL];
+          }
+        X[x] = s;
+      }
+    }
+  }
+}
+template <int TT>
+__device__ __forceinline__ void fold_shift(float (&X)[TT], int sh) {
+#pragma unroll
+  for (int bit = 1; bit < 16; bit <<= 1)
+    if (sh & bit) {
+#pragma unroll
+      for (int i = 0; i + bit < TT; ++i) X[i] = X[i + bit];
+    }
+}
+
 __device__ __forceinline__ void inv_request(const float* in, int wave, int half, int c, float (&B)[32]) {
   const float* sp = in + (wave == 0 ? 0 : (64 + 64 * (wave - 1)) * RS);
   const unsigned lo = (unsigned)((wave == 0 ? 32 : sp_row_c(T, 1, 0) - sp_row_c(T, 0, 0)) * RS * half + c);
@@ -268,7 +336,7 @@
 
 template <bool RES, bool POST> constexpr bool inv32_pipe() { return RES == POST; }
 
-template <bool TANH, bool RES, bool POST>
+template <bool TANH, bool RES, bool POST, bool FOLD = false>
 __global__ __launch_bounds__(1024) void fft32_inv_kernel(InvParams p) {
   extern __shared__ __attribute__((aligned(16))) float U[];
   const int tid = threadIdx.x, lane = tid & 63, half = lane >> 5, c = lane & 31;
@@ -331,60 +399,141 @@
       const int chan = g * p.cstride + cc;
       const bool cok = cc < p.cvalid && chan < p.C;
       const float* nin = p.sp + sp_item32(next < total ? next : item);
-      bool piped = false;
-      if (2 * wave < vy) {
+      if constexpr (!FOLD) {
+        bool piped = false;
+        if (2 * wave < vy) {
+          const int yy = 2 * wave + half;
+          const bool rowok = cok && yy < vy && vx > 0;
+          float X[32];
+          {
+            const float* e = U + ((yy & 15) * 32) * 32 + c;
+            const float osign = wave < 8 ? 1.f : -1.f;
+  #pragma unroll
+            for (int s0 = 0; s0 < T; s0 += 8) {
+  #pragma unroll
+              for (int s = s0; s < s0 + 8; ++s) hc_put(X, s, fma_(osign, e[EO + s * 32], e[s * 32]));
+              __builtin_amdgcn_sched_barrier(0);
+            }
+          }
+          rfft_inv<32>(X);
+          const float bias = (p.bias && cok) ? p.bias[chan] : 0.f;
+          const float sc = (p.bn_scale && cok) ? p.bn_scale[chan] : 1.f, sh = (p.bn_scale && cok) ? p.bn_shift[chan] : 0.f;
+          const int sgn = p.flip ? -1 : 1;
+          const int prow = p.flip ? p.Ho - 1 - y0 - yy : y0 + yy, pcol = p.flip ? p.Wo - 1 - x0 - subx : x0 + subx;
+          unsigned pix0 = (unsigned)(prow * p.Wo + pcol);
+          asm volatile("" : "+v"(pix0));
+          const int64_t ipix = (int64_t)n * p.Ho * p.Wo;
+          float* yimg = p.y + ipix * p.ldy;
+          float* aimg = (!POST && p.act_out) ? p.act_out + ipix * p.ld_act : nullptr;
+          const float* rimg = RES ? p.res + ipix * p.ld_res : nullptr;
+          const float* gimg = POST ? p.gact + ipix * p.ld_gact : nullptr;
+          float* y2img = (POST && p.y2) ? p.y2 + ipix * p.ld_y2 : nullptr;
+          const unsigned chv = (unsigned)chan;
+          if (INV32_PIPE) {
+            auto between = [&](int b) {
+              if constexpr (BURST == 8) {
+                if (b == 0) inv_request_slice<0, 8>(nin, wave, half, c, B); else if (b == 1) inv_request_slice<8, 8>(nin, wave, half, c, B);
+                else if (b == 2) inv_request_slice<16, 8>(nin, wave, half, c, B); else inv_request_slice<24, 8>(nin, wave, half, c, B);
+              } else {
+                if (b == 0) inv_request_slice<0, 4>(nin, wave, half, c, B); else if (b == 1) inv_request_slice<4, 4>(nin, wave, half, c, B);
+                else if (b == 2) inv_request_slice<8, 4>(nin, wave, half, c, B); else if (b == 3) inv_request_slice<12, 4>(nin, wave, half, c, B);
+                else if (b == 4) inv_request_slice<16, 4>(nin, wave, half, c, B); else if (b == 5) inv_request_slice<20, 4>(nin, wave, half, c, B);
+                else if (b == 6) inv_request_slice<24, 4>(nin, wave, half, c, B); else inv_request_slice<28, 4>(nin, wave, half, c, B);
+              }
+            };
+            if (rowok) {
+              epilogue_row<TANH, RES, POST, T, BURST, false>(p, X, 1.f / 1024.f, vx, pix0, sgn, chv, bias, sc, sh, yimg, aimg, rimg, gimg, y2img, ymax, bsum, between,
+                                                             p.pack > 1 ? T : __builtin_amdgcn_readfirstlane(min(p.Vx, p.Wo - x0)));
+            } else {
+              inv_request(nin, wave, half, c, B);
+            }
+            piped = true;
+          } else
+          if (rowok)
+            epilogue_row<TANH, RES, POST, T, BURST, false>(p, X, 1.f / 1024.f, vx, pix0, sgn, chv, bias, sc, sh, yimg, aimg, rimg, gimg, y2img, ymax, bsum, NoBetween(),
+                                                           p.pack > 1 ? T : __builtin_amdgcn_readfirstlane(min(p.Vx, p.Wo - x0)));
+        }
+        if (INV32_PIPE && !piped) inv_request(nin, wave, half, c, B);
+      } else {
+        bool piped = false;
         const int yy = 2 * wave + half;
-        const bool rowok = cok && yy < vy && vx > 0;
         float X[32];
-        {
-          const float* e = U + ((yy & 15) * 32) * 32 + c;
-          const float osign = wave < 8 ? 1.f : -1.f;
-#pragma unroll
-          for (int s0 = 0; s0 < T; s0 += 8) {
-#pragma unroll
-            for (int s = s0; s < s0 + 8; ++s) hc_put(X, s, fma_(osign, e[EO + s * 32], e[s * 32]));
-            __builtin_amdgcn_sched_barrier(0);
-          }
-        }
-        rfft_inv<32>(X);
-        const float bias = (p.bias && cok) ? p.bias[chan] : 0.f;
-        const float sc = (p.bn_scale && cok) ? p.bn_scale[chan] : 1.f, sh = (p.bn_scale && cok) ? p.bn_shift[chan] : 0.f;
-        const int sgn = p.flip ? -1 : 1;
-        const int prow = p.flip ? p.Ho - 1 - y0 - yy : y0 + yy, pcol = p.flip ? p.Wo - 1 - x0 - subx : x0 + subx;
-        unsigned pix0 = (unsigned)(prow * p.Wo + pcol);
-        asm volatile("" : "+v"(pix0));
-        const int64_t ipix = (int64_t)n * p.Ho * p.Wo;
-        float* yimg = p.y + ipix * p.ldy;
-        float* aimg = (!POST && p.act_out) ? p.act_out + ipix * p.ld_act : nullptr;
-        const float* rimg = RES ? p.res + ipix * p.ld_res : nullptr;
-        const float* gimg = POST ? p.gact + ipix * p.ld_gact : nullptr;
-        float* y2img = (POST && p.y2) ? p.y2 + ipix * p.ld_y2 : nullptr;
-        const unsigned chv = (unsigned)chan;
-        if (INV32_PIPE) {
-          auto between = [&](int b) {
-            if constexpr (BURST == 8) {
-              if (b == 0) inv_request_slice<0, 8>(nin, wave, half, c, B); else if (b == 1) inv_request_slice<8, 8>(nin, wave, half, c, B);
-              else if (b == 2) inv_request_slice<16, 8>(nin, wave, half, c, B); else inv_request_slice<24, 8>(nin, wave, half, c, B);
+        if (2 * wave < vy) {
+          {
+            const float* e = U + ((yy & 15) * 32) * 32 + c;
+            const float osign = wave < 8 ? 1.f : -1.f;
+  #pragma unroll
+            for (int s0 = 0; s0 < T; s0 += 8) {
+  #pragma unroll
+              for (int s = s0; s < s0 + 8; ++s) hc_put(X, s, fma_(osign, e[EO + s * 32], e[s * 32]));
+              __builtin_amdgcn_sched_barrier(0);
+            }
+          }
+          rfft_inv<32>(X);
+        }
+        float scale = 1.f / 1024.f;
+        FoldTile ft = {0, 0, false};
+        if constexpr (FOLD) {
+          const int fvx = __builtin_amdgcn_readfirstlane(vx);
+          ft = fold_tile(p, y0, x0, vy, fvx);
+          if (ft.edge) {
+            const bool row = 2 * wave < vy && yy < vy;
+            if (row) {
+  #pragma unroll
+              for (int x = 0; x < T; ++x) X[x] *= scale;
+            }
+            scale = 1.f;
+            lds_barrier();
+            if (row) fold_put<T, 32>(p, U, X, yy, y0, x0, fvx, c);
+            lds_barrier();
+            if (row && y0 + yy >= p.fpt && y0 + yy < p.fpt + p.fH) fold_add<T, 32>(p, U, X, yy, y0, x0, fvx, c);
+            if (2 * wave < vy) fold_shift<T>(X, __builtin_amdgcn_readfirstlane(ft.xlo));
+          }
+        }
+        if (2 * wave < vy) {
+          bool rowok = cok && yy < vy && vx > 0;
+          if constexpr (FOLD) rowok = cok && yy < vy && y0 + yy >= p.fpt && y0 + yy < p.fpt + p.fH && ft.ncol > 0;
+          const float bias = (p.bias && cok) ? p.bias[chan] : 0.f;
+          const float sc = (p.bn_scale && cok) ? p.bn_scale[chan] : 1.f, sh = (p.bn_scale && cok) ? p.bn_shift[chan] : 0.f;
+          const int sgn = (!FOLD && p.flip) ? -1 : 1;
+          const int prow = FOLD ? y0 + yy - p.fpt : (p.flip ? p.Ho - 1 - y0 - yy : y0 + yy);
+          const int pcol = FOLD ? x0 + ft.xlo - p.fpl : (p.flip ? p.Wo - 1 - x0 - subx : x0 + subx);
+          unsigned pix0 = (unsigned)(prow * (FOLD ? p.fW : p.Wo) + pcol);
+          asm volatile("" : "+v"(pix0));
+          const int64_t ipix = FOLD ? (int64_t)n * p.fH * p.fW : (int64_t)n * p.Ho * p.Wo;
+          const int evx = FOLD ? ft.ncol : vx;
+          float* yimg = p.y + ipix * p.ldy;
+          float* aimg = (!POST && p.act_out) ? p.act_out + ipix * p.ld_act : nullptr;
+          const float* rimg = RES ? p.res + ipix * p.ld_res : nullptr;
+          const float* gimg = POST ? p.gact + ipix * p.ld_gact : nullptr;
+          float* y2img = (POST && p.y2) ? p.y2 + ipix * p.ld_y2 : nullptr;
+          const unsigned chv = (unsigned)chan;
+          if (INV32_PIPE) {
+            auto between = [&](int b) {
+              if constexpr (BURST == 8) {
+                if (b == 0) inv_request_slice<0, 8>(nin, wave, half, c, B); else if (b == 1) inv_request_slice<8, 8>(nin, wave, half, c, B);
+                else if (b == 2) inv_request_slice<16, 8>(nin, wave, half, c, B); else inv_request_slice<24, 8>(nin, wave, half, c, B);
+              } else {
+                if (b == 0) inv_request_slice<0, 4>(nin, wave, half, c, B); else if (b == 1) inv_request_slice<4, 4>(nin, wave, half, c, B);
+                else if (b == 2) inv_request_slice<8, 4>(nin, wave, half, c, B); else if (b == 3) inv_request_slice<12, 4>(nin, wave, half, c, B);
+                else if (b == 4) inv_request_slice<16, 4>(nin, wave, half, c, B); else if (b == 5) inv_request_slice<20, 4>(nin, wave, half, c, B);
+                else if (b == 6) inv_request_slice<24, 4>(nin, wave, half, c, B); else inv_request_slice<28, 4>(nin, wave, half, c, B);
+              }
+            };
+            if (rowok) {
+              epilogue_row<TANH, RES, POST, T, BURST, false, FOLD>(p, X, scale, evx, pix0, sgn, chv, bias, sc, sh, yimg, aimg, rimg, gimg, y2img, ymax, bsum, between,
+                                                                   FOLD ? __builtin_amdgcn_readfirstlane(evx) : (p.pack > 1 ? T : __builtin_amdgcn_readfirstlane(min(p.Vx, p.Wo - x0))));
             } else {
-              if (b == 0) inv_request_slice<0, 4>(nin, wave, half, c, B); else if (b == 1) inv_request_slice<4, 4>(nin, wave, half, c, B);
-              else if (b == 2) inv_request_slice<8, 4>(nin, wave, half, c, B); else if (b == 3) inv_request_slice<12, 4>(nin, wave, half, c, B);
-              else if (b == 4) inv_request_slice<16, 4>(nin, wave, half, c, B); else if (b == 5) inv_request_slice<20, 4>(nin, wave, half, c, B);
-              else if (b == 6) inv_request_slice<24, 4>(nin, wave, half, c, B); else inv_request_slice<28, 4>(nin, wave, half, c, B);
+              inv_request(nin, wave, half, c, B);
             }
-          };
-          if (rowok) {
-            epilogue_row<TANH, RES, POST, T, BURST, false>(p, X, 1.f / 1024.f, vx, pix0, sgn, chv, bias, sc, sh, yimg, aimg, rimg, gimg, y2img, ymax, bsum, between,
-                                                           p.pack > 1 ? T : __builtin_amdgcn_readfirstlane(min(p.Vx, p.Wo - x0)));
-          } else {
-            inv_request(nin, wave, half, c, B);
-          }
-          piped = true;
-        } else
-        if (rowok)
-          epilogue_row<TANH, RES, POST, T, BURST, false>(p, X, 1.f / 1024.f, vx, pix0, sgn, chv, bias, sc, sh, yimg, aimg, rimg, gimg, y2img, ymax, bsum, NoBetween(),
-                                                         p.pack > 1 ? T : __builtin_amdgcn_readfirstlane(min(p.Vx, p.Wo - x0)));
-      }
-      if (INV32_PIPE && !piped) inv_request(nin, wave, half, c, B);
+            piped = true;
+          } else
+          if (rowok)
+            epilogue_row<TANH, RES, POST, T, BURST, false, FOLD>(p, X, scale, evx, pix0, sgn, chv, bias, sc, sh, yimg, aimg, rimg, gimg, y2img, ymax, bsum, NoBetween(),
+                                                                 FOLD ? __builtin_amdgcn_readfirstlane(evx) : (p.pack > 1 ? T : __builtin_amdgcn_readfirstlane(min(p.Vx, p.Wo - x0))));
+        }
+        if (INV32_PIPE && !piped) inv_request(nin, wave, half, c, B);
+      }
     }
     if (next >= total) break;
     item = __builtin_amdgcn_readfirstlane(next);
@@ -661,7 +810,7 @@
 constexpr int G_YS = 528, G_CS = 16 * G_YS + 16;
 constexpr size_t LDS64I_BYTES = (4 * G_CS + 128) * sizeof(float);
 
-template <bool TANH, bool RES, bool POST>
+template <bool TANH, bool RES, bool POST, bool FOLD = false>
 __global__ __launch_bounds__(512) void fft64_inv_kernel(InvParams p, int nvirt) {
   extern __shared__ __attribute__((aligned(16))) float G[];
   const int tid = threadIdx.x, lane = tid & 63, lg = lane >> 4, c16 = lane & 15;
@@ -787,14 +936,58 @@
       const bool cok = live && cc < p.cvalid && chan < p.C;
       const float bias = (p.bias && cok) ? p.bias[chan] : 0.f;
       const float sc = (p.bn_scale && cok) ? p.bn_scale[chan] : 1.f, sh = (p.bn_scale && cok) ? p.bn_shift[chan] : 0.f;
-      const int sgn = p.flip ? -1 : 1;
-      const int64_t ipix = (int64_t)n * p.Ho * p.Wo;
+      const int sgn = (!FOLD && p.flip) ? -1 : 1;
+      const int64_t ipix = FOLD ? (int64_t)n * p.fH * p.fW : (int64_t)n * p.Ho * p.Wo;
       float* yimg = p.y + ipix * p.ldy;
       float* aimg = (!POST && p.act_out) ? p.act_out + ipix * p.ld_act : nullptr;
       const float* rimg = RES ? p.res + ipix * p.ld_res : nullptr;
       const float* gimg = POST ? p.gact + ipix * p.ld_gact : nullptr;
       float* y2img = (POST && p.y2) ? p.y2 + ipix * p.ld_y2 : nullptr;
       const unsigned chv = (unsigned)chan;
+      if constexpr (FOLD) {
+        const FoldTile ft = fold_tile(p, y0, x0, vy, vx);
+        float scale = 1.f / 4096.f;
+#pragma unroll
+        for (int u = 0; u < 2; ++u) {
+          __builtin_amdgcn_sched_barrier(0);
+          if (4 * (2 * wave + u) < vy) rfft_inv<64>(R[u]);
+        }
+        if (ft.edge) {
+#pragma unroll
+          for (int u = 0; u < 2; ++u)
+            if (4 * (2 * wave + u) < vy) {
+#pragma unroll
+              for (int x = 0; x < T64; ++x) R[u][x] *= scale;
+            }
+          scale = 1.f;
+          lds_barrier();
+#pragma unroll
+          for (int u = 0; u < 2; ++u) {
+            const int yy = 4 * (2 * wave + u) + lg;
+            if (yy < vy) fold_put<T64, 16>(p, G, R[u], yy, y0, x0, vx, c16);
+          }
+          lds_barrier();
+#pragma unroll
+          for (int u = 0; u < 2; ++u) {
+            __builtin_amdgcn_sched_barrier(0);
+            const int yy = 4 * (2 * wave + u) + lg;
+            if (yy < vy && y0 + yy >= p.fpt && y0 + yy < p.fpt + p.fH) fold_add<T64, 16>(p, G, R[u], yy, y0, x0, vx, c16);
+            if (4 * (2 * wave + u) < vy) fold_shift<T64>(R[u], ft.xlo);
+          }
+        }
+#pragma unroll
+        for (int u = 0; u < 2; ++u) {
+          __builtin_amdgcn_sched_barrier(0);
+          const int unit = 2 * wave + u;
+          if (4 * unit >= vy) continue;
+          const int yy = 4 * unit + lg;
+          unsigned pix0 = (unsigned)((y0 + yy - p.fpt) * p.fW + x0 + ft.xlo - p.fpl);
+          asm volatile("" : "+v"(pix0));
+          if (cok && yy < vy && y0 + yy >= p.fpt && y0 + yy < p.fpt + p.fH && ft.ncol > 0)
+            epilogue_row<TANH, RES, POST, T64, BURST, true, true>(p, R[u], scale, ft.ncol, pix0, sgn, chv, bias, sc, sh, yimg, aimg, rimg, gimg, y2img, ymax, bsum, NoBetween(),
+                                                                  __builtin_amdgcn_readfirstlane(ft.ncol));
+        }
+      } else {
 #pragma unroll
       for (int u = 0; u < 2; ++u) {
         __builtin_amdgcn_sched_barrier(0);
@@ -809,6 +1002,7 @@
           epilogue_row<TANH, RES, POST, T64, BURST, true>(p, R[u], 1.f / 4096.f, vx, pix0, sgn, chv, bias, sc, sh, yimg, aimg, rimg, gimg, y2img, ymax, bsum, NoBetween(),
                                                           __builtin_amdgcn_readfirstlane(vx));
       }
+      }
     }
     if (next >= nvirt) break;
     v = __builtin_amdgcn_readfirstlane(next);
@@ -838,6 +1032,7 @@
   if (t == 0) dbias[ch] = red[0];
 }
 
+static_assert(4 * G_CS >= (14 + 14) * T64 * 16, "FOLD: the pad strips of a 15-tap layer fit the 64-point inverse's LDS image below its twiddle table");
 constexpr size_t LDS64_BYTES = LDS_BYTES + 128 * sizeof(float);
 
 void launch_fwd_fft32(pcnn_handle h, FwdParams p, int ntile) {
@@ -890,6 +1085,14 @@
   const int nvirt = 2 * ((ntg + 7) & ~7);
   const dim3 grid((unsigned)std::min((nvirt + 15) & ~15, 256));
   dispatch_epilogue(p, [&](auto TANH, auto RES, auto POST, const InvParams& q) {
+    if constexpr (!TANH.value) {
+      if (q.fold) {
+        constexpr auto fkernel = fft64_inv_kernel<false, RES.value, POST.value, true>;
+        set_lds(fkernel, LDS64I_BYTES);
+        hipLaunchKernelGGL(fkernel, grid, dim3(512), LDS64I_BYTES, h->stream, q, nvirt);
+        return;
+      }
+    }
     constexpr auto kernel = fft64_inv_kernel<TANH.value, RES.value, POST.value>;
     set_lds(kernel, LDS64I_BYTES);
     hipLaunchKernelGGL(kernel, grid, dim3(512), LDS64I_BYTES, h->stream, q, nvirt);
@@ -900,6 +1103,14 @@
   p.ntile = ntile;
   const dim3 grid((unsigned)std::min(ntile * p.groups, 256));
   dispatch_epilogue(p, [&](auto TANH, auto RES, auto POST, const InvParams& q) {
+    if constexpr (!TANH.value) {
+      if (q.fold) {
+        constexpr auto fkernel = fft32_inv_kernel<false, RES.value, POST.value, true>;
+        set_lds(fkernel, LDS_BYTES);
+        hipLaunchKernelGGL(fkernel, grid, dim3(1024), LDS_BYTES, h->stream, q);
+        return;
+      }
+    }
     constexpr auto kernel = fft32_inv_kernel<TANH.value, RES.value, POST.value>;
     set_lds(kernel, LDS_BYTES);
     hipLaunchKernelGGL(kernel, grid, dim3(1024), LDS_BYTES, h->stream, q);
diff --git a/poisson_cnn_amd/layers.py b/poisson_cnn_amd/layers.py
--- a/poisson_cnn_amd/layers.py
+++ b/poisson_cnn_amd/layers.py
@@ -305,9 +305,13 @@
             wf, wver = self._flipped(w)
             res = add_to if (self.mode == 'CONSTANT') else None
             out = ops.conv2d_bwd_fused(x, dz, w.shape, wf, pad_top=self.pads_y[0], pad_left=self.pads_x[0], pad_mode=self.mode, pad_value=self.pad_value,
-                                       dw=g[self.name + '/kernel'], residual=res, post=post, w_version=wver)
+                                       dw=g[self.name + '/kernel'], residual=res, post=post, w_version=wver, fold=self.mode != 'CONSTANT',
+                                       add_to=add_to if self.mode != 'CONSTANT' else None, before_inplace=self.ctx.before_inplace_write)
             if out is not None:
                 if self.mode == 'CONSTANT':
+                    return out
+                out, folded = out
+                if folded:
                     return out
                 if post is not None and not post.applied:
                     dzp = ops.pad_fold_bwd_post(out, (H, W), (self.pads_y, self.pads_x), self.mode, post, add_to=add_to, ws=self.ctx.ws)
diff --git a/poisson_cnn_amd/ops.py b/poisson_cnn_amd/ops.py
--- a/poisson_cnn_amd/ops.py
+++ b/poisson_cnn_amd/ops.py
@@ -267,6 +267,14 @@
 def set_post_fusion(on):
     global _post_fusion
     _post_fusion = bool(on)
+
+
+_spectral_fold = __import__('os').environ.get('PCNN_SPECTRAL_FOLD', '1') != '0'
+
+
+def set_spectral_fold(on):
+    global _spectral_fold
+    _spectral_fold = bool(on)
 
 
 _stage_fusion = __import__('os').environ.get('PCNN_STAGE_FUSION', '1') != '0'
@@ -399,7 +407,7 @@
         self.applied, self.raw = False, None
 
 
-def conv2d_bwd_fused(x, dz, w_shape, wf, *, pad_top, pad_left, pad_mode='CONSTANT', pad_value=0.0, dw, residual=None, post=None, w_version=0):
+def conv2d_bwd_fused(x, dz, w_shape, wf, *, pad_top, pad_left, pad_mode='CONSTANT', pad_value=0.0, dw, residual=None, post=None, w_version=0, fold=False, add_to=None, before_inplace=None):
     N, H, W, Cin = x.shape
     kh, kw, _, Cout = w_shape
     mode = pad_mode.upper()
@@ -414,9 +422,28 @@
     h = handle()
     if not h.lib.pcnn_conv2d_bwd_spectral_eligible(h._h, byref(d), byref(dg)):
         return None
-    out = empty((N, out_hw[0], out_hw[1], Cin), x.device)
     flops = 2.0 * N * dz.shape[1] * dz.shape[2] * kh * kw * Cin * Cout
     nbytes = 4.0 * (2 * N * H * W * Cin + N * dz.shape[1] * dz.shape[2] * Cout + 2 * kh * kw * Cin * Cout)
+    post_ok = post is None or (post.bn_scale is None and _post_fusion and Cin <= 32)
+    if fold and mode != 'CONSTANT' and _spectral_fold and post_ok and (add_to is None or (add_to.is_contiguous() and tuple(add_to.shape) == (N, H, W, Cin))):
+        dgf = conv_desc(dz.shape, _ld(dz), (kh, kw, Cout, Cin), out_hw, ldo, dpt, dpl, 'CONSTANT', 0.0, 'linear', Cin if add_to is not None else 0, 0)
+        if h.lib.pcnn_conv2d_bwd_spectral_fold_eligible(h._h, byref(d), byref(dgf)):
+            pd = None
+            if post is not None:
+                post.raw = empty((N, H, W, Cin), x.device) if post.want_raw else None
+                pd = PostDesc(post.a.data_ptr(), _ld(post.a), ACTS[post.act], LEAKY_ALPHA, post.dbias.data_ptr() if post.dbias is not None else None,
+                              post.raw.data_ptr() if post.raw is not None else None, Cin)
+            dxo = add_to if (add_to is not None and pd is None) else empty((N, H, W, Cin), x.device)
+            if dxo is add_to and before_inplace is not None:
+                before_inplace(add_to)
+            def run_fold():
+                with _FilterVersion(h, w_version):
+                    h.call('pcnn_conv2d_bwd_spectral_fold', byref(d), byref(dgf), _p(x), _p(dz), _p(wf), _p(add_to), _p(dxo), _p(dw), byref(pd) if pd is not None else None)
+            _launch('conv_bwd_fused', 2.0 * flops, run_fold, nbytes)
+            if pd is not None:
+                post.applied = True
+            return dxo, True
+    out = empty((N, out_hw[0], out_hw[1], Cin), x.device)
     if post is not None and post.bn_scale is None and mode == 'CONSTANT' and _post_fusion and h.lib.pcnn_conv2d_bwd_spectral_post_eligible(h._h, byref(d), byref(dg)):
         post.raw = empty((N, H, W, Cin), x.device) if post.want_raw else None
         pd = PostDesc(post.a.data_ptr(), _ld(post.a), ACTS[post.act], LEAKY_ALPHA, post.dbias.data_ptr() if post.dbias is not None else None,
@@ -426,12 +453,12 @@
                 h.call('pcnn_conv2d_bwd_spectral_post', byref(d), byref(dg), _p(x), _p(dz), _p(wf), _p(residual), _p(out), _p(dw), byref(pd))
         _launch('conv_bwd_fused', 2.0 * flops, run_post, nbytes)
         post.applied = True
-        return out
+        return (out, False) if fold else out
     def run():
         with _FilterVersion(h, w_version):
             h.call('pcnn_conv2d_bwd_spectral', byref(d), byref(dg), _p(x), _p(dz), _p(wf), _p(residual), _p(out), _p(dw))
     _launch('conv_bwd_fused', 2.0 * flops, run, nbytes)
-    return out
+    return (out, False) if fold else out
 
 
 def resnet3_eligible(C, act):
```

Result: no change. 43.51 grids/s, median of 6 (+0.3%).
